# youngers2006/Dreamer

Hardware: AMD Instinct MI355X
Metric: imagined latent-steps/sec (B×H) at 64×64 CarRacing, 1/2/4/8 MI355X (higher is better)
Workload: dtype f32; 1 GPU; Dreamer.train_Agent() with AC_epochs=1 (replay sample + warm start S/2 + H-step imagination + actor-critic update), B=256/GPU S=64 H=15 64x64x3, precision=fp32 (north-star batch per GPU); global_batch=256, seq_len=64, horizon=15, parallelism=dp1, precision=fp32

## Files before the change

### dreamer_amd/_lib.py

```python
import ctypes as C
import os

import torch

_HERE = os.path.dirname(os.path.abspath(__file__))
LIB_PATH = os.path.join(_HERE, "libdreamer_hip.so")
if os.environ.get("DREAMER_LIB_VARIANT"):
    LIB_PATH = os.path.join(os.path.dirname(_HERE), "tools", "variants",
                            f"libdreamer_hip_{os.environ['DREAMER_LIB_VARIANT']}.so")

fp = C.c_void_p


class dr_linear(C.Structure):
    _fields_ = [("w", fp), ("b", fp)]


class dr_mlp3(C.Structure):
    _fields_ = [("l0", dr_linear), ("n1", dr_linear), ("l3", dr_linear), ("n4", dr_linear), ("l6", dr_linear)]


class dr_dims(C.Structure):
    _fields_ = [(n, C.c_int) for n in (
        "hidden", "rows", "cols", "action", "img_h", "img_w", "enc_f1", "enc_f2", "enc_hidden",
        "prior_h1", "prior_h2", "rew_h1", "rew_h2", "cont_h1", "cont_h2",
        "actor_h1", "actor_h2", "critic_h1", "critic_h2", "buckets", "dec_f1", "dec_f2", "dec_hidden", "precision", "obs_dim", "enc_depth",
        "launch_form")] + [("fault", fp), ("fault_host", fp)]

DR_MAX_DEPTH = 5


class dr_world_model(C.Structure):
    _fields_ = [("conv", dr_linear * DR_MAX_DEPTH), ("map0", dr_linear), ("map1", dr_linear), ("map3", dr_linear),
                ("w_ih", fp), ("w_hh", fp), ("b_ih", fp), ("b_hh", fp),
                ("prior", dr_mlp3), ("reward", dr_mlp3), ("cont", dr_mlp3), ("buckets_rew", fp)]


class dr_decoder(C.Structure):
    _fields_ = [("up0", dr_linear), ("up1", dr_linear), ("up3", dr_linear), ("convt", dr_linear * DR_MAX_DEPTH)]


class dr_wm_batch(C.Structure):
    _fields_ = [("actions", fp), ("act_sb", C.c_longlong), ("act_st", C.c_longlong), ("rewards", fp),
                ("continues", fp), ("rc_sb", C.c_longlong), ("rc_st", C.c_longlong)]


class dr_wm_loss_cfg(C.Structure):
    _fields_ = [("beta_pred", C.c_float), ("beta_dyn", C.c_float), ("beta_rep", C.c_float)]


class dr_actor(C.Structure):
    _fields_ = [("l0", dr_linear), ("n1", dr_linear), ("l3", dr_linear), ("n4", dr_linear),
                ("mu", dr_linear), ("ls", dr_linear)]


class dr_critic(C.Structure):
    _fields_ = [("net", dr_mlp3), ("buckets", fp)]


class dr_noise(C.Structure):
    _fields_ = [("q", fp), ("eps", fp), ("rng", fp), ("row0", C.c_int), ("stream", C.c_int)]


class dr_frames(C.Structure):
    _fields_ = [("ring", fp), ("ring_cap", C.c_longlong), ("starts", fp), ("obs", fp),
                ("stride_b", C.c_longlong), ("stride_t", C.c_longlong), ("raw255", C.c_int), ("t0", C.c_int)]


_P = C.POINTER
_sz = C.c_size_t
_i = C.c_int
_ll = C.c_longlong
_f = C.c_float
_d = C.c_double

_SIGS = {
    "dr_last_error": (C.c_char_p, []),
    "dr_version": (_i, []),
    "dr_encoder_workspace_bytes": (_sz, [_P(dr_dims), _i]),
    "dr_encoder_features": (_i, [_P(dr_dims), _P(dr_world_model), _P(dr_frames), _i, _i, fp, fp, _sz, fp]),
    "dr_observe_workspace_bytes": (_sz, [_P(dr_dims), _i]),
    "dr_observe_scan": (_i, [_P(dr_dims), _P(dr_world_model), _i, _i, fp, fp, _ll, _ll, fp, fp, dr_noise,
                             fp, fp, fp, fp, _sz, fp]),
    "dr_observe_trace_workspace_bytes": (_sz, [_P(dr_dims), _i, _i]),
    "dr_observe_trace": (_i, [_P(dr_dims), _P(dr_world_model), _i, _i, fp, fp, _ll, _ll, fp, fp, dr_noise,
                              fp, fp, fp, fp, fp, fp, fp, _sz, fp]),
    "dr_latent_stats": (_i, [_i, _i, _i, fp, fp, fp, fp, fp, fp, fp]),
    "dr_replay_returns": (_i, [_i, _i, fp, _ll, fp, _ll, _i, fp, _f, _f, fp, fp, fp, fp]),
    "dr_value_stats": (_i, [_i, _i, _i, _i, fp, _ll, fp, fp, fp, fp, fp, fp]),
    "dr_action_logprob": (_i, [_i, _i, _i, fp, fp, fp, _ll, _ll, fp, fp, fp, fp]),
    "dr_plan_sample": (_i, [_i, _i, _i, _i, _i, fp, fp, fp, dr_noise, fp, fp]),
    "dr_plan_update": (_i, [_i, _i, _i, _i, _i, fp, fp, fp, _f, _f, _f, _f, _f, fp, fp, fp, fp, fp, fp, fp, fp]),
    "dr_imagine_tape_bytes":(_sz, [_P(dr_dims), _i, _i]),
    "dr_imagine_workspace_bytes": (_sz, [_P(dr_dims), _i, _i]),
    "dr_imagine_fwd": (_i, [_P(dr_dims), _P(dr_world_model), _P(dr_actor), _i, _i, fp, fp, dr_noise, _i,
                            fp, fp, fp, fp, fp, fp, fp, fp, fp, _sz, fp]),
    "dr_imagine_actions_workspace_bytes": (_sz, [_P(dr_dims), _i, _i]),
    "dr_imagine_actions": (_i, [_P(dr_dims), _P(dr_world_model), _i, _i, fp, fp, fp, _ll, _ll, dr_noise,
                                fp, fp, fp, fp, fp, _sz, fp]),
    "dr_imagine_bwd": (_i, [_P(dr_dims), _P(dr_world_model), _P(dr_actor), _i, _i, fp, fp, fp, fp, fp,
                            fp, fp, fp, fp, _P(dr_actor), fp, _sz, fp]),
    "dr_imagine_bwd_prep": (_i, [_P(dr_dims), _P(dr_world_model), _P(dr_actor), _i, _i, fp, fp, fp, fp, _sz, fp]),
    "dr_imagine_bwd_main": (_i, [_P(dr_dims), _P(dr_world_model), _P(dr_actor), _i, _i, fp, fp, fp, fp, fp, _i,
                                 fp, _P(dr_actor), fp, _sz, fp]),
    "dr_step_workspace_bytes": (_sz, [_P(dr_dims), _i]),
    "dr_imagine_step": (_i, [_P(dr_dims), _P(dr_world_model), _i, fp, fp, fp, dr_noise, fp, fp, fp, fp,
                             fp, _sz, fp]),
    "dr_actor_act_workspace_bytes": (_sz, [_P(dr_dims), _i]),
    "dr_actor_act": (_i, [_P(dr_dims), _P(dr_actor), _i, fp, fp, dr_noise, _i, fp, fp, fp, fp, _sz, fp]),
    "dr_act_step_workspace_bytes": (_sz, [_P(dr_dims)]),
    "dr_act_step": (_i, [_P(dr_dims), _P(dr_world_model), _P(dr_actor), fp, _i, fp, fp, fp, dr_noise, _i,
                         fp, fp, fp, fp, fp, fp, fp, fp, _sz, fp]),
    "dr_act_batch_workspace_bytes": (_sz, [_P(dr_dims), _i]),
    "dr_act_batch": (_i, [_P(dr_dims), _P(dr_world_model), _P(dr_actor), _i, fp, fp, fp, fp, fp, dr_noise, _i,
                          fp, fp, fp, fp, fp, fp, fp, fp, _sz, fp]),
    "dr_act_vec_workspace_bytes": (_sz, [_P(dr_dims), _i]),
    "dr_act_vec": (_i, [_P(dr_dims), _P(dr_world_model), _P(dr_actor), _i, fp, fp, fp, fp, fp, dr_noise, _i,
                        fp, fp, fp, fp, fp, fp, fp, fp, _sz, fp]),
    "dr_gru_cell": (_i, [_P(dr_dims), _P(dr_world_model), _i, fp, fp, fp, fp, fp, _sz, fp]),
    "dr_categorical_sample": (_i, [_i, _i, _i, fp, dr_noise, fp, fp, fp, fp]),
    "dr_mlp3_fwd": (_i, [_P(dr_mlp3), _i, _i, fp, _ll, _i, fp, _ll, _i, _i, _i, fp, _ll, fp, _sz, fp]),
    "dr_bucket_value": (_i, [_i, _i, fp, fp, fp, fp]),
    "dr_critic_tape_bytes": (_sz, [_P(dr_dims), _i]),
    "dr_critic_workspace_bytes": (_sz, [_P(dr_dims), _i, _i]),
    "dr_critic_fwd": (_i, [_P(dr_dims), _P(dr_critic), _i, fp, _ll, fp, _ll, fp, fp, fp, fp, _sz, fp]),
    "dr_lambda_returns": (_i, [_i, _i, fp, fp, fp, _f, _f, fp, fp]),
    "dr_update_S": (_i, [_i, fp, fp, fp, fp, _sz, fp]),
    "dr_actor_loss_grad": (_i, [_i, _i, _i, fp, fp, fp, fp, fp, fp, _f, _f, fp, fp, fp, fp]),
    "dr_critic_loss_bwd": (_i, [_P(dr_dims), _P(dr_critic), _i, _i, fp, fp, fp, fp, _f, fp, _P(dr_critic),
                                fp, _sz, fp]),
    "dr_sqnorm": (_i, [_ll, fp, fp, fp]),
    "dr_sqnorm_multi": (_i, [_ll, fp, fp, fp, fp]),
    "dr_clip_stats": (_i, [_ll, fp, _ll, fp, _i, fp, fp, fp, fp, fp]),
    "dr_adamw": (_i, [_ll, fp, fp, fp, fp, fp, _f, _d, _d, _d, _d, _d, fp, fp, fp, fp]),
    "dr_ema": (_i, [_ll, fp, fp, _f, _f, fp, fp]),
    "dr_ac_optimiser_step": (_i, [_ll, fp, fp, fp, fp, fp, fp, _d, _d, _d, _d, _d,
                                  _ll, fp, fp, fp, fp, fp, fp, _d, _d, _d, _d, _d,
                                  _f, fp, _f, _f, _i, fp, fp, fp, fp, fp]),
    "dr_nonfinite": (_i, [_ll, fp, fp, fp]),
    "dr_replay_gather": (_i, [_ll, _i, _i, _i, _i, fp, fp, fp, fp, fp, fp, fp, fp, fp, fp]),
    "dr_rng_advance": (_i, [fp, C.c_ulonglong, fp]),
    "dr_persistent_kernels": (_i, [_P(dr_dims), _i, _i, _i]),
    "dr_stream_create_cumask": (_i, [_i, _P(C.c_uint), _P(fp)]),
    "dr_stream_destroy": (_i, [fp]),
    "dr_device_cus": (_i, [_P(_i)]),
    "dr_host_device_ptr": (_i, [fp, _P(fp)]),
    "dr_wm_train_workspace_bytes": (_sz, [_P(dr_dims), _i, _i]),
    "dr_decoder_workspace_bytes": (_sz, [_P(dr_dims), _i]),
    "dr_decoder_fwd": (_i, [_P(dr_dims), _P(dr_decoder), _i, fp, _ll, fp, _ll, fp, fp, _sz, fp]),
    "dr_frame_metrics": (_i, [_P(dr_dims), _i, _i, fp, _P(dr_frames), fp, fp, fp, fp]),
    "dr_frame_ssim": (_i, [_P(dr_dims), _i, _i, fp, _P(dr_frames), fp, fp, fp]),
    "dr_ensemble_metrics": (_i, [_P(dr_dims), _i, _i, _i, fp, _P(dr_frames), fp, fp, fp, fp, fp, fp]),
    "dr_wm_train_phase": (_i, [_P(dr_dims), _P(dr_world_model), _P(dr_decoder), _i, _i, _P(dr_frames),
                               _P(dr_wm_batch), dr_noise, dr_wm_loss_cfg, _i, fp, _i, fp, fp, _P(dr_world_model),
                               _P(dr_decoder), fp, fp, fp, fp, _sz, fp]),
    "dr_wm_train_grads": (_i, [_P(dr_dims), _P(dr_world_model), _P(dr_decoder), _i, _i, _P(dr_frames),
                               _P(dr_wm_batch), dr_noise, dr_wm_loss_cfg, fp, fp, _P(dr_world_model),
                               _P(dr_decoder), fp, fp, fp, fp, _sz, fp]),
}

EXPORTED = sorted(_SIGS)

_lib = None
_load_error = None


def load():
    global _lib, _load_error
    if _lib is not None:
        return _lib
    if not os.path.exists(LIB_PATH):
        _load_error = f"{LIB_PATH} not built (run: python -m dreamer_amd.build)"
        raise RuntimeError("dreamer_amd: HIP library missing: " + _load_error)
    lib = C.CDLL(LIB_PATH)
    for name, (res, args) in _SIGS.items():
        fn = getattr(lib, name)
        fn.restype = res
        fn.argtypes = args
    _lib = lib
    return lib


DR_E_INVALID, DR_E_HIP, DR_E_WORKSPACE, DR_E_UNSUPPORTED = 1001, 1002, 1003, 1004
DR_ACT_MAX_ENVS = 16
DR_ACT_VEC_MAX_OBS = 1023
DR_PLAN_MAX_CANDIDATES = 2048
DR_ENSEMBLE_MAX_SAMPLES = 64
DR_PLAN_MAX_ELEMS = 1024


class HipError(RuntimeError):

    def __init__(self, name, code, msg):
        super().__init__(f"{name} failed ({code}): {msg}")
        self.code = code


def call(name, *args):
    lib = load()
    rc = getattr(lib, name)(*args)
    if rc != 0:
        msg = lib.dr_last_error().decode(errors="replace")
        raise HipError(name, rc, msg)


def query(name, *args):
    return getattr(load(), name)(*args)


def ptr(t):
    if t is None:
        return None
    if not t.is_cuda:
        raise RuntimeError("dreamer_amd: tensors must live on the GPU (this framework is MI355X-only)")
    return t.data_ptr()


def stream_ptr(device=None):
    return torch.cuda.current_stream(device).cuda_stream


def require_gpu(t):
    if not (isinstance(t, torch.Tensor) and t.is_cuda):
        raise RuntimeError("dreamer_amd: hot-path ops run only on the GPU (MI355X); "
                           "move the model and tensors to 'cuda'")
```

### dreamer_amd/csrc/conv.h

```cpp
#pragma once
#include "common.h"

int op_conv_nhwc(int n, int cin, int ih, int iw, int cout, const float* in, const float* wr, const float* bias,
                 float* out, int out_nchw, hipStream_t s);
enum { CONV_EPI_FWD = 0, CONV_EPI_DSILU = 1 };
int op_conv_nhwc_ex(int n, int cin, int ih, int iw, int cout, const float* in, const float* wr, const float* bias,
                    float* out, int out_nchw, float* pre, int epi, hipStream_t s, float* csum = nullptr);
int op_frames_nhwc4(int n, int nb, int h, int w, const dr_frames* src, float* out, hipStream_t s, float pad = 0.0f);
int op_conv1_frames(int n, int nb, int ih, int iw, int cout, const dr_frames* src, const float* wr, const float* bias,
                    float* out, hipStream_t s);
int op_conv_repack_pad(int cout, int cin, int cin_pad, const float* w, float* wr, hipStream_t s);

int op_conv_repack_split3(int cout, int cin, const float* w, void* wr, hipStream_t s);
bool op_conv_split3_supported(int n, int cin, int ih, int iw, int cout);
int op_enc12_s1_bf16(int n, int nb, int h, int w, int c1, int c2, const dr_frames* src, const float* w1,
                     const float* b1, const float* w2, const float* b2, void* wr1, void* wr2, void* out,
                     hipStream_t s, int prepacked = 0);
int op_conv_s1_bf16(int n, int cin, int ih, int iw, int cout, const void* in, const void* wr, const float* bias,
                    void* out, int out_nchw, hipStream_t s);
bool op_conv_glds_bf16_supported(int n, int cin, int ih, int iw, int cout);
int op_conv_glds_s3(int n, int cin, int ih, int iw, int cout, const float* in, const void* wr, const float* bias,
                    float* out, int out_nchw, float* pre, int epi, hipStream_t s);
size_t op_gemm_nt_glds_part_floats(int M, int N, int K);
int op_gemm_nt_glds_bf16(int M, int N, int K, const void* X, int ldx, const void* W, int ldw, const float* bias,
                         float* Y, int ldy, float* part, size_t part_floats, hipStream_t s);
int op_conv_glds_bf16(int n, int cin, int ih, int iw, int cout, const void* in, const void* wr, const float* bias,
                      void* out, int out_nchw, hipStream_t s);
int op_conv_split3(int n, int cin, int ih, int iw, int cout, const float* in, const void* wr, const float* bias,
                   float* out, int out_nchw, hipStream_t s);
int op_conv_split3_ex(int n, int cin, int ih, int iw, int cout, const float* in, const void* wr, const float* bias,
                      float* out, int out_nchw, float* pre, int epi, hipStream_t s, int terms = 3);

size_t op_nt_split3_ws_bytes(int N, int K);
int op_nt_repack_split3(int N, int K, const float* W, int ldw, void* wr, hipStream_t s);
bool op_gemm_nt_split3_supported(int M, int N, int K, const float* A, int lda, const float* A2, int lda2, int ksA,
                                 int ldy);
int op_gemm_nt_split3(int M, int N, int K, const float* A, int lda, const float* A2, int lda2, int ksA, const void* wr,
                      const float* bias, int act, float* Y, int ldy, hipStream_t s);
size_t op_gemm_nt_split3_part_floats(int M, int N);
int op_gemm_nt_split3_sk(int M, int N, int K, const float* A, int lda, const float* A2, int lda2, int ksA,
                         const void* wr, const float* bias, int act, float* Y, int ldy, float* part,
                         size_t part_floats, hipStream_t s, int splits_fixed = 0);
int op_gemm_nt_split3_ex(int M, int N, int K, const float* A, int lda, const float* A2, int lda2, int ksA,
                         const void* wr, const float* bias, int act, float* Y, int ldy, int accumulate, float* Y2,
                         int ldy2, int nsplitY, float* part, size_t part_floats, hipStream_t s, int splits_fixed = 0);

int op_conv_repack_bf16(int cout, int cin, int cin_pad, const float* w, void* wr, hipStream_t s);
int op_to_bf16_2d(int rows, int cols, const float* x, long long ld, void* y, hipStream_t s);
int op_conv1_bf16(int n, int nb, int h, int w, int cout, const dr_frames* src, const void* wr, const float* bias,
                  void* out, hipStream_t s);
bool op_enc12_split3_ok(int n, int h, int w, int c1, int c2, const dr_frames* src);
int op_enc12_split3(int n, int nb, int h, int w, int c1, int c2, const dr_frames* src, const float* w1,
                    const float* b1, const float* w2, const float* b2, void* wr1, void* wr2, float* out,
                    hipStream_t s, int prepacked = 0);
int op_enc12_split3_ex(int n, int nb, int h, int w, int c1, int c2, const dr_frames* src, const float* w1,
                       const float* b1, const float* w2, const float* b2, void* wr1, void* wr2, float* out,
                       float* pre0, float* a0, float* pre1, hipStream_t s, int terms = 3, int prepacked = 0);
enum { RJ_CONV1 = 0, RJ_CONV = 1, RJ_NT = 2, RJ_BF16 = 3 };
struct RepackJob {
  int kind, a, b, c;
  const float* w;
  void* out;
  long long ld;
  long long total;
};
#define DR_RJ_MAX 6
RepackJob rj_conv1(int cout, const float* w, void* wr);
RepackJob rj_conv(int cout, int cin, const float* w, void* wr);
RepackJob rj_nt(int N, int K, const float* W, int ldw, void* wr);
RepackJob rj_bf16(int rows, int cols, const float* x, long long ld, void* y);
int op_repack_multi(const RepackJob* jobs, int n, hipStream_t s);
int op_enc12_bf16(int n, int nb, int h, int w, int c1, int c2, const dr_frames* src, const void* wr1, const float* b1,
                  const void* wr2, const float* b2, void* out, hipStream_t s);
int op_conv_bf16(int n, int cin, int ih, int iw, int cout, const void* in, const void* wr, const float* bias,
                 void* out, int out_nchw, hipStream_t s);
int op_gemm_nt_bf16(int M, int N, int K, const void* X, int ldx, const void* W, const float* bias, float* Y, int ldy,
                    hipStream_t s);

enum { CT_EPI_BIAS = 0, CT_EPI_DSILU = 1, CT_EPI_TANH_MSE = 2 };
struct ConvTArgs {
  int n, cin, h, w, cout;
  const float* in;
  int silu_in;
  const float* wq;
  const float* bias;
  float* out;
  float* out2;
  int silu_out;
  int ldc;
  const float* pre;
  const float* target;
  int tstride;
  const float* coef;
  float* part;
  float* bpart;
};
int op_convT_repack(int cin, int cout, const float* wt, float* wq, hipStream_t s);
int op_convT_nhwc(int epi, const ConvTArgs& a, hipStream_t s);
int op_convT_mse_parts(int h, int w);
int op_convT_out3_repack(int cin, const float* wt, float* wq, hipStream_t s);
int op_convT_out3(const ConvTArgs& a, hipStream_t s);
int op_convT_repack_split3(int cin, int cout, const float* wt, void* wr, hipStream_t s);
bool op_convT_split3_supported(int n, int cin, int h, int w, int cout, int terms = 3);
bool op_convT_cls_supported(int n, int cin, int h, int w, int cout);
int op_convT_split3(int epi, const ConvTArgs& a, const void* wr, hipStream_t s, int terms = 3);
bool op_convT_glds_s3_supported(const ConvTArgs& a, int epi);
int op_convT_glds_s3(int epi, const ConvTArgs& a, const void* wr, hipStream_t s);

size_t op_conv_wgrad_ws_floats(int n, int h, int w, int ca, int cb);
int op_wgrad_reduce(int ca, int cb, int cbo, int nsplit, const float* part, float* dw, float scale, int accumulate,
                    hipStream_t s);
bool op_wgrad_split3_supported(int n, int h, int w, int ca, int cb, int terms = 3);
size_t op_wgrad_split3_ws_floats(int n, int h, int w, int ca, int cb);
int op_wgrad_split3(int n, int h, int w, int ca, int cb, const float* lo, int lda, const float* hi, int ldb,
                    float* dw, int cbo, float scale, int accumulate, float* ws, size_t ws_floats, hipStream_t s,
                    int terms = 3);
int op_conv_wgrad(int n, int h, int w, int ca, int cb, const float* lo, int lda, int lo_silu, const float* hi, int ldb,
                  float* dw, int cbo, float scale, int accumulate, float* ws, size_t ws_floats, hipStream_t s,
                  float* bias_out = nullptr);
size_t op_chan_sum_ws_floats(long long rows, int C);
int op_chan_sum(long long rows, int C, const float* X, int ldx, float* out, int accumulate, float* ws, size_t ws_floats,
                hipStream_t s);
int op_chan_sum_final(int nb, int C, const float* part, float* out, int accumulate, hipStream_t s);

size_t op_gemm_tn_split3_ws_bytes(int M, int N, int K);
bool op_gemm_tn_split3_supported(int M, int N, int K);
int op_gemm_tn_split3(int M, int N, int K, const float* G, long long ldg, const float* X, long long ldx,
                      const float* X2, long long ldx2, int nsplitB, float* Y, long long ldy, int accumulate, void* ws,
                      size_t ws_bytes, hipStream_t s, int terms = 3);
struct TnProblem {
  int M, N, K;
  const float* G;
  long long ldg;
  const float* X;
  long long ldx;
  const float* X2;
  long long ldx2;
  int nsplitB;
  float* Y;
  long long ldy;
  int accumulate;
};
size_t op_gemm_tn_split3_multi_ws_bytes(const TnProblem* p, int n);
int op_gemm_tn_split3_multi(const TnProblem* p, int n, void* ws, size_t ws_bytes, hipStream_t s, int terms);
```

### dreamer_amd/csrc/conv_split.hip

```cpp
#include "conv.h"

#include <algorithm>
#include <climits>
#include <type_traits>

namespace {
typedef unsigned short u16;
typedef __bf16 bf16x8 __attribute__((ext_vector_type(8)));
typedef unsigned u32x4 __attribute__((ext_vector_type(4)));
typedef unsigned u32x2 __attribute__((ext_vector_type(2)));

__device__ __forceinline__ f32x4 mfma_b16(u32x4 a, u32x4 b, f32x4 c) {
  return __builtin_amdgcn_mfma_f32_16x16x32_bf16(__builtin_bit_cast(bf16x8, a), __builtin_bit_cast(bf16x8, b), c, 0, 0,
                                                  0);
}
__device__ __forceinline__ unsigned b16bits(__bf16 v) { return (unsigned)__builtin_bit_cast(u16, v); }
__device__ __forceinline__ void split3(float x, unsigned& h, unsigned& m, unsigned& l) {
  const __bf16 bh = (__bf16)x;
  const float r1 = x - (float)bh;
  const __bf16 bm = (__bf16)r1;
  const float r2 = r1 - (float)bm;
  h = b16bits(bh);
  m = b16bits(bm);
  l = b16bits((__bf16)r2);
// ... 1665 lines not shown
  for (int i = 0; i < APT; ++i) {
    const int m = min(m0 + prow + (NT / 8) * i, M - 1);
    oa[i] = (unsigned)(m * g.lda);
    oa2[i] = (unsigned)(m * g.lda2);
  }
  f32x4 ra0[APT], ra1[APT];
  u32x4 rb0[BPT], rb1[BPT];
  bool kv0 = true, kv1 = true;
  auto load = [&](int c, auto slot) __attribute__((always_inline)) {
    f32x4* ra = decltype(slot)::value == 0 ? ra0 : ra1;
    u32x4* rb = decltype(slot)::value == 0 ? rb0 : rb1;
    bool& kv = decltype(slot)::value == 0 ? kv0 : kv1;
    const int k = 32 * c + 4 * quad;
    kv = k < K;
    const int kk = kv ? k : 0;
    const bool s1 = kk < ksA;
    const float* base = s1 ? g.A : g.A2;
#pragma unroll
    for (int i = 0; i < APT; ++i) {
      const unsigned e = s1 ? oa[i] + (unsigned)kk : oa2[i] + (unsigned)(kk - ksA);
      ra[i] = *reinterpret_cast<const f32x4*>(base + e);
    }
#pragma unroll
    for (int j = 0; j < BPT; ++j) {
      const int e = tid + NT * j;
      if (BU % NT == 0 || e < BU) {
        const int pl = e / (BN * 4), rm = e - pl * BN * 4, row = rm >> 2, u = rm & 3;
        rb[j] = *reinterpret_cast<const u32x4*>(g.wr + (((long long)c * 3 + pl) * Np + n0 + row) * 32 + 8 * u);
      }
    }
  };
  auto store = [&](auto slot, int buf) __attribute__((always_inline)) {
    const f32x4* ra = decltype(slot)::value == 0 ? ra0 : ra1;
    const u32x4* rb = decltype(slot)::value == 0 ? rb0 : rb1;
    const bool kv = decltype(slot)::value == 0 ? kv0 : kv1;
#pragma unroll
    for (int i = 0; i < APT; ++i) {
      const int row = prow + (NT / 8) * i;
      const f32x4 v = kv ? ra[i] : (f32x4){0.f, 0.f, 0.f, 0.f};
      unsigned h0, m0_, l0, h1, m1, l1;
      split3_pair(v[0], v[1], h0, m0_, l0);
      split3_pair(v[2], v[3], h1, m1, l1);
      const int unit = (quad >> 1) ^ swz(row), half = quad & 1;
      reinterpret_cast<u32x2*>(&As[buf][0][row][unit])[half] = (u32x2){h0, h1};
      reinterpret_cast<u32x2*>(&As[buf][1][row][unit])[half] = (u32x2){m0_, m1};
      reinterpret_cast<u32x2*>(&As[buf][2][row][unit])[half] = (u32x2){l0, l1};
    }
#pragma unroll
    for (int j = 0; j < BPT; ++j) {
      const int e = tid + NT * j;
      if (BU % NT == 0 || e < BU) {
        const int pl = e / (BN * 4), rm = e - pl * BN * 4, row = rm >> 2, u = rm & 3;
        Bs[buf][pl][row][u ^ swz(row)] = rb[j];
      }
    }
  };
  const int wm0 = (wave >> 1) * 64, wn0 = (wave & 1) * WTN;
  const int fu = q ^ swz(r);
  f32x4 acc[FM][FN];
#pragma unroll
  for (int i = 0; i < FM; ++i)
#pragma unroll
    for (int j = 0; j < FN; ++j) acc[i][j] = (f32x4){0.f, 0.f, 0.f, 0.f};
  using S0 = std::integral_constant<int, 0>;
  using S1 = std::integral_constant<int, 1>;
  if (cb < NCH) {
  load(cb, S0{});
  load(min(cb + 1, NCH - 1), S1{});
  store(S0{}, 0);
  __syncthreads();
  auto step = [&](int c, auto slot) __attribute__((always_inline)) {
    constexpr int SL = decltype(slot)::value;
    using Next = std::integral_constant<int, 1 - SL>;
    const int buf = (c - cb) & 1;
    load(min(c + 2, NCH - 1), slot);
    u32x4 av[3][FM], bv[3][FN];
#pragma unroll
    for (int pl = 0; pl < 3; ++pl) {
#pragma unroll
      for (int i = 0; i < FM; ++i) av[pl][i] = As[buf][pl][wm0 + 16 * i + r][fu];
#pragma unroll
      for (int j = 0; j < FN; ++j) bv[pl][j] = Bs[buf][pl][wn0 + 16 * j + r][fu];
    }
#define DR_G3(PA, PB)                                                                                   \
  _Pragma("unroll") for (int i = 0; i < FM; ++i) _Pragma("unroll") for (int j = 0; j < FN; ++j) acc[i][j] = \
      mfma_b16(bv[PB][j], av[PA][i], acc[i][j]);
    DR_G3(2, 0)
    DR_G3(1, 1)
    DR_G3(0, 2)
    DR_G3(1, 0)
    DR_G3(0, 1)
    DR_G3(0, 0)
#undef DR_G3
    if (c + 1 < NCH) store(Next{}, buf ^ 1);
    dr_lds_barrier();
  };
  int c = cb;
  for (; c + 1 < NCH; c += 2) {
    step(c, S0{});
    step(c + 1, S1{});
  }
  if (c < NCH) step(c, S0{});
  }
#pragma unroll
  for (int i = 0; i < FM; ++i) {
    const int m = m0 + wm0 + 16 * i + r;
    if (m >= M) continue;
#pragma unroll
    for (int j = 0; j < FN; ++j) {
      const int n = n0 + wn0 + 16 * j + 4 * q;
      if (n >= N) continue;
      f32x4 v = acc[i][j];
      if (g.splits > 1) {
        *reinterpret_cast<f32x4*>(g.part + ((long long)blockIdx.y * M + m) * N + n) = v;
        continue;
      }
      if (g.bias) v += *reinterpret_cast<const f32x4*>(g.bias + n);
      if (g.act == 1) {
#pragma unroll
        for (int e = 0; e < 4; ++e) v[e] = v[e] / (1.0f + expf(-v[e]));
      }
      s3_store(g, m, n, v);
    }
  }
}

__global__ void k_s3_finish(GemmS3 g) {
  const long long i4 = (long long)blockIdx.x * 256 + threadIdx.x;
  const int N4 = g.N / 4;
  if (i4 >= (long long)g.M * N4) return;
  const int m = (int)(i4 / N4), n = 4 * (int)(i4 - (long long)m * N4);
  f32x4 v = (f32x4){0.f, 0.f, 0.f, 0.f};
  for (int sp = 0; sp < g.splits; ++sp) v += *reinterpret_cast<const f32x4*>(g.part + ((long long)sp * g.M + m) * g.N + n);
  if (g.bias) v += *reinterpret_cast<const f32x4*>(g.bias + n);
  if (g.act == 1) {
#pragma unroll
    for (int e = 0; e < 4; ++e) v[e] = v[e] / (1.0f + expf(-v[e]));
  }
  s3_store(g, m, n, v);
}

__device__ __forceinline__ void nt_repack_split3_elem(long long i, int N, int K, int Np, const float* __restrict__ W,
                                                      long long ldw, u16* __restrict__ wr) {
  const int KC = (K + 31) / 32;
  const int n = (int)(i / (KC * 32)), k = (int)(i - (long long)n * KC * 32);
  unsigned hh = 0, mm = 0, ll = 0;
  if (n < N && k < K) split3(W[(long long)n * ldw + k], hh, mm, ll);
  const long long plane = (long long)Np * 32;
  const long long base = ((long long)(k >> 5) * 3 * Np + n) * 32 + (k & 31);
  wr[base] = (u16)hh;
  wr[base + plane] = (u16)mm;
  wr[base + 2 * plane] = (u16)ll;
}
__global__ void k_nt_repack_split3(int N, int K, int Np, const float* __restrict__ W, int ldw, u16* __restrict__ wr) {
  const long long i = (long long)blockIdx.x * blockDim.x + threadIdx.x;
  if (i >= (long long)((K + 31) / 32) * 32 * Np) return;
  nt_repack_split3_elem(i, N, K, Np, W, ldw, wr);
}

struct RepackBatch {
  RepackJob j[DR_RJ_MAX];
  int blk0[DR_RJ_MAX + 1];
  int n;
};
__global__ __launch_bounds__(256) void k_repack_multi(RepackBatch b) {
  __shared__ __attribute__((aligned(16))) RepackJob J;
  int z = 0;
#pragma unroll
  for (int i = 1; i < DR_RJ_MAX; ++i)
    if ((int)blockIdx.x >= b.blk0[i]) z = i;
  dr_stage_args(b.j[z], J, threadIdx.x);
  const long long i = (long long)(blockIdx.x - b.blk0[z]) * 256 + threadIdx.x;
  if (i >= J.total) return;
  u16* out = static_cast<u16*>(J.out);
  switch (J.kind) {
    case RJ_CONV1: conv1_repack_split3_elem((int)i, J.a, J.w, out); break;
    case RJ_CONV: conv_repack_split3_elem((int)i, J.a, J.b, J.w, out); break;
    case RJ_NT: nt_repack_split3_elem(i, J.a, J.b, J.c, J.w, J.ld, out); break;
    default: {
      const int rr = (int)(i / J.b), cc = (int)(i - (long long)rr * J.b);
      out[i] = __builtin_bit_cast(u16, (__bf16)J.w[(long long)rr * J.ld + cc]);
    }
  }
}

RepackJob rj_conv1(int cout, const float* w, void* wr) { return {RJ_CONV1, cout, 0, 0, w, wr, 0, (long long)cout * 64}; }
RepackJob rj_conv(int cout, int cin, const float* w, void* wr) {
  return {RJ_CONV, cout, cin, 0, w, wr, 0, (long long)cout * 16 * cin};
}
RepackJob rj_nt(int N, int K, const float* W, int ldw, void* wr) {
  const int Np = (N + 127) / 128 * 128;
  return {RJ_NT, N, K, Np, W, wr, ldw, (long long)((K + 31) / 32) * 32 * Np};
}
RepackJob rj_bf16(int rows, int cols, const float* x, long long ld, void* y) {
  return {RJ_BF16, rows, cols, 0, x, y, ld, (long long)rows * cols};
}

int op_repack_multi(const RepackJob* jobs, int n, hipStream_t s) {
  if (n < 0 || n > DR_RJ_MAX) {
    dr_set_error("repack_multi: %d jobs (at most %d)", n, DR_RJ_MAX);
    return DR_E_INVALID;
  }
  if (n == 0) return DR_OK;
  RepackBatch b = {};
  int tot = 0;
  for (int i = 0; i < DR_RJ_MAX; ++i) {
    b.blk0[i] = tot;
    if (i < n) {
      b.j[i] = jobs[i];
      tot += (int)((jobs[i].total + 255) / 256);
    }
  }
  b.blk0[DR_RJ_MAX] = tot;
  b.n = n;
  hipLaunchKernelGGL(k_repack_multi, dim3((unsigned)tot), dim3(256), 0, s, b);
  return dr_check_launch("repack_multi");
}

static int s3_np(int N) { return (N + 127) / 128 * 128; }
size_t op_nt_split3_ws_bytes(int N, int K) {
  return (size_t)((K + 31) / 32) * 32 * 3 * s3_np(N) * sizeof(u16);
}
int op_nt_repack_split3(int N, int K, const float* W, int ldw, void* wr, hipStream_t s) {
  const int Np = s3_np(N);
  const long long total = (long long)((K + 31) / 32) * 32 * Np;
  hipLaunchKernelGGL(k_nt_repack_split3, dim3((unsigned)((total + 255) / 256)), dim3(256), 0, s, N, K, Np, W, ldw,
                     (u16*)wr);
  return dr_check_launch("nt_repack_split3");
}
bool op_gemm_nt_split3_supported(int M, int N, int K, const float* A, int lda, const float* A2, int lda2, int ksA,
                                 int ldy) {
  const bool seg = ksA < K;
  return M > 0 && N > 0 && N % 4 == 0 && ldy % 4 == 0 && K % 4 == 0 && lda % 4 == 0 && !((uintptr_t)A & 15) &&
         (!seg || (ksA % 4 == 0 && lda2 % 4 == 0 && A2 && !((uintptr_t)A2 & 15))) &&
         (long long)M * lda < (1LL << 31) && (!seg || (long long)M * lda2 < (1LL << 31));
}
size_t op_gemm_nt_split3_part_floats(int M, int N) { return (size_t)DR_S3_SPLITS * M * N; }

int op_gemm_nt_split3(int M, int N, int K, const float* A, int lda, const float* A2, int lda2, int ksA, const void* wr,
                      const float* bias, int act, float* Y, int ldy, hipStream_t s) {
  return op_gemm_nt_split3_sk(M, N, K, A, lda, A2, lda2, ksA, wr, bias, act, Y, ldy, nullptr, 0, s);
}

int op_gemm_nt_split3_sk(int M, int N, int K, const float* A, int lda, const float* A2, int lda2, int ksA,
                         const void* wr, const float* bias, int act, float* Y, int ldy, float* part,
                         size_t part_floats, hipStream_t s, int splits_fixed) {
  return op_gemm_nt_split3_ex(M, N, K, A, lda, A2, lda2, ksA, wr, bias, act, Y, ldy, 0, nullptr, 0, INT_MAX, part,
                              part_floats, s, splits_fixed);
}

int op_gemm_nt_split3_ex(int M, int N, int K, const float* A, int lda, const float* A2, int lda2, int ksA,
                         const void* wr, const float* bias, int act, float* Y, int ldy, int accumulate, float* Y2,
                         int ldy2, int nsplitY, float* part, size_t part_floats, hipStream_t s, int splits_fixed) {
  const bool y2 = nsplitY < N;
  if (!op_gemm_nt_split3_supported(M, N, K, A, lda, A2, lda2, ksA, ldy) || ((uintptr_t)Y & 15) ||
      (bias && ((uintptr_t)bias & 15)) || ((uintptr_t)part & 15) || splits_fixed < 0 ||
      splits_fixed > DR_S3_SPLITS || (splits_fixed > 1 && (!part || (size_t)splits_fixed * M * N > part_floats)) ||
      (y2 && (!Y2 || ((uintptr_t)Y2 & 15) || ldy2 % 4 || nsplitY % 4 || nsplitY < 0))) {
    dr_set_error("gemm_nt_split3: unsupported problem (M=%d N=%d K=%d)", M, N, K);
    return DR_E_INVALID;
  }
  GemmS3 g = {M, N, K, ksA < K ? ksA : K, lda, lda2, ldy, act, s3_np(N), A, A2, (const u16*)wr, bias, Y, 1, part,
              accumulate ? 1 : 0, ldy2, y2 ? nsplitY : INT_MAX, 0, Y2};
  auto tl = [&](int bm, int bn) { return ((M + bm - 1) / bm) * ((N + bn - 1) / bn); };
  auto waves = [&](int bm, int bn) { return (long long)tl(bm, bn) * (bm / 32); };
  const int nch = (K + 31) / 32;
  auto splits_for = [&](int bm, int bn) {
    if (splits_fixed > 0) return splits_fixed;
    int sp = 1;
    while (part && sp < DR_S3_SPLITS && waves(bm, bn) * sp < 2048 && nch / (2 * sp) >= 8 &&
           (size_t)(2 * sp) * M * N <= part_floats)
      sp *= 2;
    return sp;
  };
  const int shapes[5][2] = {{256, 128}, {256, 64}, {128, 128}, {128, 64}, {64, 64}};
  int pick = 4;
  for (int c = 0; c < 5; ++c) {
    if (waves(shapes[c][0], shapes[c][1]) * splits_for(shapes[c][0], shapes[c][1]) >= 2048) {
      pick = c;
      break;
    }
  }
  g.splits = splits_for(shapes[pick][0], shapes[pick][1]);
  const unsigned gy = (unsigned)g.splits;
  switch (pick) {
    case 0: hipLaunchKernelGGL((k_gemm_split3<256, 128>), dim3(dr_xcd_grid(tl(256, 128)), gy), dim3(512), 0, s, g); break;
    case 1: hipLaunchKernelGGL((k_gemm_split3<256, 64>), dim3(dr_xcd_grid(tl(256, 64)), gy), dim3(512), 0, s, g); break;
    case 2: hipLaunchKernelGGL((k_gemm_split3<128, 128>), dim3(dr_xcd_grid(tl(128, 128)), gy), dim3(256), 0, s, g); break;
    case 3: hipLaunchKernelGGL((k_gemm_split3<128, 64>), dim3(dr_xcd_grid(tl(128, 64)), gy), dim3(256), 0, s, g); break;
    default: hipLaunchKernelGGL((k_gemm_split3<64, 64>), dim3(dr_xcd_grid(tl(64, 64)), gy), dim3(128), 0, s, g); break;
  }
  DR_TRY(dr_check_launch("gemm_nt_split3"));
  if (g.splits > 1) {
    hipLaunchKernelGGL(k_s3_finish, dim3((unsigned)(((long long)M * (N / 4) + 255) / 256)), dim3(256), 0, s, g);
    DR_TRY(dr_check_launch("s3_finish"));
  }
  return DR_OK;
}

static int s3_pad(int n) { return (n + 127) / 128 * 128; }

struct KnRepack {
  int K, N, P, nsplit;
  const float* X;
  const float* X2;
  long long ldx, ldx2;
  u16* wr;
  long long pad_;
};

template <int TERMS>
__device__ __forceinline__ void kn_repack_body(int K, int N, int P, const float* __restrict__ X, long long ldx,
                                               const float* __restrict__ X2, long long ldx2, int nsplit,
                                               u16* __restrict__ wr) {
  const int n = blockIdx.x * 256 + threadIdx.x, kc = blockIdx.y;
  if (n >= P) return;
  const bool seg2 = n >= nsplit;
  const float* src = seg2 ? X2 : X;
  const long long ld = seg2 ? ldx2 : ldx;
  const int nn = seg2 ? n - nsplit : n;
  float v[32];
  const bool nok = n < N;
  const float* col = src + (nok ? nn : 0);
#pragma unroll
  for (int k = 0; k < 32; ++k) {
    const int kk = 32 * kc + k;
    const bool ok = nok && kk < K;
    const float t = col[ok ? (long long)kk * ld : 0LL];
    v[k] = ok ? t : 0.f;
  }
  u32x4* o = reinterpret_cast<u32x4*>(wr + (((long long)kc * 3) * P + n) * 32);
  if constexpr (TERMS == 1) {
#pragma unroll
    for (int u = 0; u < 4; ++u) {
      u32x4 h;
#pragma unroll
      for (int e = 0; e < 4; ++e) h[e] = pack_bf16x2(v[8 * u + 2 * e], v[8 * u + 2 * e + 1]);
      o[u] = h;
    }
    return;
  }
  u32x4 h[4], m[4], l[4];
#pragma unroll
  for (int u = 0; u < 4; ++u)
#pragma unroll
    for (int e = 0; e < 4; ++e) {
      unsigned hh, mm, ll;
      split3_pair(v[8 * u + 2 * e], v[8 * u + 2 * e + 1], hh, mm, ll);
      h[u][e] = hh;
      m[u][e] = mm;
      l[u][e] = ll;
    }
  const long long pl = (long long)P * 32 / 8;
#pragma unroll
  for (int u = 0; u < 4; ++u) {
    o[u] = h[u];
    o[pl + u] = m[u];
    o[2 * pl + u] = l[u];
  }
}

struct GemmPP {
  int M, N, K, Mp, Np, splits, accumulate, tiles;
  long long ldy;
  const u16* wa;
  const u16* wb;
  float* Y;
// ... 294 lines not shown
```

### dreamer_amd/csrc/engine.hip

```cpp
#include "engine_util.h"
#include "scan.h"
#include "dream.h"
#include "bptt.h"


static bool s3_first_layer(const dr_dims* d, int M, int N, const float* h, long long ldh, const float* z,
                           long long ldz) {
  return d->precision != DR_PREC_BF16 && M >= 1024 && ldh < INT_MAX && ldz < INT_MAX &&
         op_gemm_nt_split3_supported(M, N, d->hidden + latent(d), h, (int)ldh, z, (int)ldz, d->hidden, N);
}

struct EncWs {
  float *x0, *a[DR_MAX_DEPTH], *wr[DR_MAX_DEPTH], *sk;
  long long sk_n;
  void* wproj;
  void* s3proj;
  float* s3part;
  size_t s3part_n;
};

static void enc_carve(Carve& c, const dr_dims* d, int n, EncWs& w) {
  memset(&w, 0, sizeof(w));
  if (d->obs_dim > 0) {
    const int F = enc_feat_dim(d);
    w.x0 = c.f((long long)n * d->obs_dim);
    w.a[0] = c.f((long long)n * F);
    w.a[1] = c.f((long long)n * F);
    w.sk_n = splitk_floats(n, d->enc_hidden);
    w.sk = c.f(w.sk_n);
    return;
  }
  const bool bf = d->precision == DR_PREC_BF16;
  int e[DR_MAX_DEPTH + 1];
  const int N = enc_chans(d, e);
  const long long p0 = (long long)d->img_h * d->img_w;
  auto act = [&](long long elems) { return bf ? (float*)c.raw(elems * 2) : c.f(elems); };
  w.sk_n = bf ? 0 : splitk_floats(n, d->enc_hidden);
  w.sk = bf ? nullptr : c.f(w.sk_n);
  w.x0 = bf ? nullptr : c.f((long long)n * p0 * 4);
  for (int k = 0; k < N; ++k) w.a[k] = act((long long)n * (p0 >> (2 * (k + 1))) * e[k + 1]);
  w.wr[0] = (float*)c.raw((size_t)e[1] * 64 * 6);
  for (int k = 1; k < N; ++k) w.wr[k] = (float*)c.raw((long long)e[k + 1] * e[k] * 16 * 6);
  w.wproj = bf ? c.raw((size_t)d->enc_hidden * enc_feat_dim(d) * 2) : nullptr;
  w.s3proj = bf ? nullptr : c.raw(op_nt_split3_ws_bytes(d->enc_hidden, enc_feat_dim(d)));
  w.s3part_n = bf ? op_gemm_nt_glds_part_floats(n, d->enc_hidden, enc_feat_dim(d))
                  : op_gemm_nt_split3_part_floats(n, d->enc_hidden);
  w.s3part = w.s3part_n ? c.f((long long)w.s3part_n) : nullptr;
}

extern "C" size_t dr_encoder_workspace_bytes(const dr_dims* d, int n_frames) {
  Carve c(nullptr);
  EncWs w;
  enc_carve(c, d, n_frames, w);
  return c.off;
}

static int encoder_bf16(const dr_dims* d, const dr_world_model* wm, const dr_frames* src, int B, int n, float* feat,
                        const EncWs& w, hipStream_t s) {
  int e[DR_MAX_DEPTH + 1];
  const int N = enc_chans(d, e);
  const int h0 = d->img_h, w0 = d->img_w;
  const int F = enc_feat_dim(d);
  const bool e12 = N >= 2 && op_enc12_split3_ok(n, h0, w0, e[1], e[2], src) && !((uintptr_t)w.a[1] & 15);
  RepackJob rj[DR_RJ_MAX];
  int nj = 0;
  if (e12) {
    rj[nj++] = rj_conv1(e[1], wm->conv[0].w, w.wr[0]);
    rj[nj++] = rj_conv(e[2], e[1], wm->conv[1].w, w.wr[1]);
  }
  bool s3[DR_MAX_DEPTH + 1] = {};
  for (int k = 2; k < N; ++k) {
    s3[k] = op_conv_split3_supported(n, e[k], h0 >> k, w0 >> k, e[k + 1]) && nj < DR_RJ_MAX - 1;
    if (s3[k]) rj[nj++] = rj_conv(e[k + 1], e[k], wm->conv[k].w, w.wr[k]);
    else DR_TRY(op_conv_repack_bf16(e[k + 1], e[k], e[k], wm->conv[k].w, w.wr[k], s));
  }
  rj[nj++] = rj_bf16(d->enc_hidden, F, wm->map0.w, F + d->hidden, w.wproj);
  DR_TRY(op_repack_multi(rj, nj, s));
  const int rc_s1 = e12 ? op_enc12_s1_bf16(n, B, h0, w0, e[1], e[2], src, wm->conv[0].w, wm->conv[0].b, wm->conv[1].w,
                                           wm->conv[1].b, w.wr[0], w.wr[1], w.a[1], s, 1)
                        : DR_E_INVALID;
  if (rc_s1 != DR_OK) {
    if (rc_s1 != DR_E_INVALID) return rc_s1;
    DR_TRY(op_conv_repack_bf16(e[1], 3, 4, wm->conv[0].w, w.wr[0], s));
    DR_TRY(op_conv_repack_bf16(e[2], e[1], e[1], wm->conv[1].w, w.wr[1], s));
    const int rc_b = op_enc12_bf16(n, B, h0, w0, e[1], e[2], src, w.wr[0], wm->conv[0].b, w.wr[1], wm->conv[1].b,
                                   w.a[1], s);
    if (rc_b != DR_OK) {
      if (rc_b != DR_E_INVALID) return rc_b;
      DR_TRY(op_conv1_bf16(n, B, h0, w0, e[1], src, w.wr[0], wm->conv[0].b, w.a[0], s));
      DR_TRY(op_conv_bf16(n, e[1], h0 / 2, w0 / 2, e[2], w.a[0], w.wr[1], wm->conv[1].b, w.a[1], 0, s));
    }
  }
  for (int k = 2; k < N; ++k) {
    if (s3[k]) {
      DR_TRY(op_conv_s1_bf16(n, e[k], h0 >> k, w0 >> k, e[k + 1], w.a[k - 1], w.wr[k], wm->conv[k].b, w.a[k],
                             k == N - 1 ? 1 : 0, s));
    } else {
      DR_TRY(op_conv_bf16(n, e[k], h0 >> k, w0 >> k, e[k + 1], w.a[k - 1], w.wr[k], wm->conv[k].b, w.a[k],
                          k == N - 1 ? 1 : 0, s));
    }
  }
  const int rcp = op_gemm_nt_glds_bf16(n, d->enc_hidden, F, w.a[N - 1], F, w.wproj, F, wm->map0.b, feat, d->enc_hidden,
                                       w.s3part, w.s3part_n, s);
  if (rcp != DR_E_INVALID) return rcp;
  return op_gemm_nt_bf16(n, d->enc_hidden, F, w.a[N - 1], F, w.wproj, wm->map0.b, feat, d->enc_hidden, s);
}

extern "C" int dr_encoder_features(const dr_dims* d, const dr_world_model* wm, const dr_frames* src, int B, int T,
                                   float* feat, void* ws, size_t ws_bytes, hipStream_t s) {
  DR_REQUIRE(d && wm && src && feat && B > 0 && T > 0, "null argument or empty batch");
  DR_REQUIRE(vae_depth_ok(d), "enc_depth must be 0, 4 or 5");
  if (d->obs_dim > 0) {
    DR_REQUIRE(d->enc_f2 > 0 && d->obs_dim % 4 == 0, "vector observations: obs_dim % 4 == 0 required");
    const int n = B * T, F = enc_feat_dim(d), D = d->obs_dim;
    Carve c(ws);
    EncWs w;
    enc_carve(c, d, n, w);
    WS_CHECK(c, ws_bytes);
    DR_TRY(op_vec_gather(n, B, D, src, w.x0, s));
    GemmArgs g1 = lin(n, F, D, w.x0, D, wm->conv[0].w, D, wm->conv[0].b, w.a[0], F);
    g1.act = 1;
    DR_TRY(run(G_NT, AM_PLAIN, g1, s));
    GemmArgs g2 = lin(n, F, F, w.a[0], F, wm->conv[1].w, F, wm->conv[1].b, w.a[1], F);
    g2.act = 1;
    DR_TRY(run(G_NT, AM_PLAIN, g2, s));
    GemmArgs gp = lin(n, d->enc_hidden, F, w.a[1], F, wm->map0.w, F + d->hidden, wm->map0.b, feat, d->enc_hidden);
    float* sk = w.sk;
    long long skn = w.sk_n;
    give_splitk(gp, sk, skn);
    return run(G_NT, AM_PLAIN, gp, s);
  }
  int e[DR_MAX_DEPTH + 1];
  const int N = enc_chans(d, e);
  DR_REQUIRE(d->img_h % (1 << N) == 0 && d->img_w % (1 << N) == 0,
             "image size must be a multiple of 2^depth (16, or 32 for the 5-layer encoder)");
  DR_REQUIRE(d->enc_f1 % 4 == 0 && d->enc_f2 % 4 == 0, "encoder filter counts must be multiples of 4");
  DR_REQUIRE(d->precision == DR_PREC_FP32 || d->precision == DR_PREC_BF16, "precision must be DR_PREC_FP32/BF16");
  const int n = B * T;
  Carve c(ws);
  EncWs w;
  enc_carve(c, d, n, w);
  WS_CHECK(c, ws_bytes);
  if (d->precision == DR_PREC_BF16) return encoder_bf16(d, wm, src, B, n, feat, w, s);
  const int h0 = d->img_h, w0 = d->img_w;
  const int F = enc_feat_dim(d);
  const bool e12 = N >= 2 && op_enc12_split3_ok(n, h0, w0, e[1], e[2], src);
  const bool s3p = w.s3proj && n >= 1024 &&
                   op_gemm_nt_split3_supported(n, d->enc_hidden, F, w.a[N - 1], F, nullptr, 0, F, d->enc_hidden);
  RepackJob rj[DR_RJ_MAX];
  int nj = 0;
  if (e12) {
    rj[nj++] = rj_conv1(e[1], wm->conv[0].w, w.wr[0]);
    rj[nj++] = rj_conv(e[2], e[1], wm->conv[1].w, w.wr[1]);
  }
  bool s3[DR_MAX_DEPTH + 1] = {};
  for (int k = e12 ? 2 : 1; k < N; ++k) {
    s3[k] = op_conv_split3_supported(n, e[k], h0 >> k, w0 >> k, e[k + 1]) && nj < DR_RJ_MAX - 1;
    if (!s3[k]) continue;
    DR_TRY(conv_bias_aligned(__func__, "conv", k, wm->conv[k].b));
    rj[nj++] = rj_conv(e[k + 1], e[k], wm->conv[k].w, w.wr[k]);
  }
  if (s3p) rj[nj++] = rj_nt(d->enc_hidden, F, wm->map0.w, F + d->hidden, w.s3proj);
  DR_TRY(op_repack_multi(rj, nj, s));
  int k0 = 1;
  const int rc12 = e12 ? op_enc12_split3(n, B, h0, w0, e[1], e[2], src, wm->conv[0].w, wm->conv[0].b, wm->conv[1].w,
                                         wm->conv[1].b, w.wr[0], w.wr[1], w.a[1], s, 1)
                       : DR_E_INVALID;
  if (rc12 == DR_OK) {
    k0 = 2;
  } else {
    if (rc12 != DR_E_INVALID) return rc12;
    DR_TRY(op_conv_repack_pad(e[1], 3, 4, wm->conv[0].w, w.wr[0], s));
    if (op_conv1_frames(n, B, h0, w0, e[1], src, w.wr[0], wm->conv[0].b, w.a[0], s) != DR_OK) {
      DR_TRY(op_frames_nhwc4(n, B, h0, w0, src, w.x0, s));
      DR_TRY(op_conv_nhwc(n, 4, h0, w0, e[1], w.x0, w.wr[0], wm->conv[0].b, w.a[0], 0, s));
    }
  }
  for (int k = k0; k < N; ++k) {
    const int cin = e[k], cout = e[k + 1], hin = h0 >> k, win = w0 >> k, last = k == N - 1;
    const float* cw = wm->conv[k].w;
    const float* cb = wm->conv[k].b;
    if (s3[k]) {
      DR_TRY(op_conv_split3(n, cin, hin, win, cout, w.a[k - 1], w.wr[k], cb, w.a[k], last, s));
    } else {
      DR_TRY(op_conv_repack_pad(cout, cin, cin, cw, w.wr[k], s));
      DR_TRY(op_conv_nhwc(n, cin, hin, win, cout, w.a[k - 1], w.wr[k], cb, w.a[k], last, s));
    }
  }
  if (s3p) {
    const int ksplits = std::max(1, std::min(8, (F + 1023) / 1024));
    return op_gemm_nt_split3_sk(n, d->enc_hidden, F, w.a[N - 1], F, nullptr, 0, F, w.s3proj, wm->map0.b, 0, feat,
                                d->enc_hidden, w.s3part, w.s3part_n, s, ksplits);
  }
  GemmArgs gp = lin(n, d->enc_hidden, F, w.a[N - 1], F, wm->map0.w, F + d->hidden, wm->map0.b, feat, d->enc_hidden);
  float* sk = w.sk;
  long long skn = w.sk_n;
  give_splitk(gp, sk, skn);
  return run(G_NT, AM_PLAIN, gp, s);
}

struct ObsWs {
  float *gi, *gh, *pre1, *logits, *wt, *hb[2];
  unsigned short* hb16[2];
  int* idx;
  void *s3m0, *s3whh;
  void* ring;
};
static void obs_carve(Carve& c, const dr_dims* d, int B, ObsWs& w) {
  w.ring = c.raw(op_pscan_ring_bytes(B));
  w.s3m0 = c.raw(op_nt_split3_ws_bytes(d->enc_hidden, d->hidden));
  w.s3whh = c.raw(op_nt_split3_ws_bytes(3 * d->hidden, d->hidden));
  w.gi = c.f((long long)B * 3 * d->hidden);
  w.gh = c.f((long long)B * 3 * d->hidden);
  w.pre1 = c.f((long long)B * d->enc_hidden);
  w.logits = c.f((long long)B * latent(d));
  w.wt = c.f((long long)(latent(d) + d->action) * 3 * d->hidden);
  w.hb[0] = c.f((long long)B * d->hidden);
  w.hb[1] = c.f((long long)B * d->hidden);
  w.hb16[0] = (unsigned short*)c.raw(sizeof(unsigned short) * B * d->hidden);
  w.hb16[1] = (unsigned short*)c.raw(sizeof(unsigned short) * B * d->hidden);
  w.idx = c.i(2LL * B * d->rows);
}

extern "C" size_t dr_observe_workspace_bytes(const dr_dims* d, int B) {
  Carve c(nullptr);
  ObsWs w;
  obs_carve(c, d, B, w);
  return c.off;
}

struct ObsTrace {
  float *latents, *hiddens, *post_logits;
  float* z_last;
  int* idx_last;
};

static int observe_steps(const dr_dims* d, const dr_world_model* wm, int B, int T, const float* feat,
                         const float* actions, long long act_sb, long long act_st, const float* h_init,
                         const float* z_init, const dr_noise& noise, float* z_out, float* h_out, float* logits_out,
                         ObsWs& w, const ObsTrace* tr, hipStream_t s);

extern "C" int dr_observe_scan(const dr_dims* d, const dr_world_model* wm, int B, int T, const float* feat,
                               const float* actions, long long act_sb, long long act_st, const float* h_init,
                               const float* z_init, dr_noise noise, float* z_out, float* h_out, float* logits_out,
                               void* ws, size_t ws_bytes, hipStream_t s) {
  DR_REQUIRE(d && wm && feat && z_out && h_out && B > 0 && T > 0, "null argument or empty batch");
  GemmBf16Scope bf16_scope(d->precision == DR_PREC_BF16);
  DR_REQUIRE(T == 1 || (z_init == nullptr ? T > 1 : true), "bad T");
  DR_REQUIRE(actions || (z_init == nullptr && T == 1), "actions required");
  Carve c(ws);
  ObsWs w;
  obs_carve(c, d, B, w);
  WS_CHECK(c, ws_bytes);
  const int L = latent(d), Hd = d->hidden, eh = d->enc_hidden;
  const int F = enc_feat_dim(d);
  const bool any_gru = (z_init != nullptr) || T > 1;
  if (any_gru) {
    DR_REQUIRE(wm->w_ih && wm->w_hh && wm->b_ih && wm->b_hh, "GRU weights required");
    DR_TRY(op_transpose(3 * Hd, L + d->action, wm->w_ih, w.wt, s));
  }
  if (z_init == nullptr && h_init == nullptr && op_pscan_supported(d, B, T, d->action)) {
    const int rc = op_pscan(d, wm, B, T, d->action, feat, actions, act_sb, act_st, w.wt, wm->map0.w + F, F + Hd,
                            noise, 0, z_out, h_out, logits_out, w.ring, s);
    if (rc != DR_E_UNSUPPORTED) return rc;
  }
  return observe_steps(d, wm, B, T, feat, actions, act_sb, act_st, h_init, z_init, noise, z_out, h_out, logits_out, w,
                       nullptr, s);
}

static int observe_steps(const dr_dims* d, const dr_world_model* wm, int B, int T, const float* feat,
                         const float* actions, long long act_sb, long long act_st, const float* h_init,
                         const float* z_init, const dr_noise& noise, float* z_out, float* h_out, float* logits_out,
                         ObsWs& w, const ObsTrace* tr, hipStream_t s) {
  const int L = latent(d), Hd = d->hidden, eh = d->enc_hidden;
  const int F = enc_feat_dim(d);
  const long long ldL = (long long)T * L, ldH = (long long)T * Hd;
  const bool planes = B >= 128 && T > 1 && Hd % 8 == 0;
  if (planes) {
    DR_TRY(split_planes(eh, Hd, wm->map0.w + F, F + Hd, w.s3m0, s));
    DR_TRY(split_planes(3 * Hd, Hd, wm->w_hh, Hd, w.s3whh, s));
  }
  const float* h = h_init;
  const unsigned short* h16 = nullptr;
  const bool a16 = planes && d->precision == DR_PREC_BF16;
  int hb = 0;
  const bool split_gru = B >= 128;
  bool gh_pre = false;
  if (z_init) {
    if (z_init != z_out) DR_TRY(copy2d(z_out, L, z_init, L, L, B, s));
    DR_TRY(op_onehot_index(B, d->rows, d->cols, z_out, L, w.idx, onehot_vals(w.idx, B, d->rows), s));
    if (split_gru && planes && h_init) {
      GemmArgs gh = lin(B, 3 * Hd, Hd, h_init, Hd, wm->w_hh, Hd, wm->b_hh, w.gh, 3 * Hd);
      wplanes(gh, w.s3whh);
      DR_TRY(gemm_launch(G_NT, AM_PLAIN, &gh, 1, s));
      gh_pre = true;
    }
  }
  for (int t = 0; t < T; ++t) {
    const bool do_gru = (z_init != nullptr) || t > 0;
    if (do_gru) {
      const int ai = t - (z_init == nullptr ? 1 : 0);
      float* hn = w.hb[hb];
      unsigned short* hn16 = a16 ? w.hb16[hb] : nullptr;
      hb ^= 1;
      DR_TRY(gru_onehot(d, wm, B, w.idx, actions + ai * act_st, act_sb, h, Hd, hn, Hd, w.wt, nullptr,
                        nullptr, nullptr, nullptr, s, z_out, L, w.gh, gh_pre, hn16));
      h = hn;
      h16 = hn16;
    }
    GemmArgs g[2];
    g[0] = lin(B, eh, h ? Hd : 0, h, Hd, wm->map0.w + F, F + Hd, nullptr, w.pre1, eh);
    g[0].addend = feat + (long long)t * B * eh;
    g[0].ld_add = eh;
    const GemmArgs g_last = g[0];
    gh_pre = split_gru && h && t + 1 < T;
    if (gh_pre) {
      g[1] = lin(B, 3 * Hd, Hd, h, Hd, wm->w_hh, Hd, wm->b_hh, w.gh, 3 * Hd);
      if (planes) {
        wplanes(g[0], w.s3m0);
        wplanes(g[1], w.s3whh);
        g[0].A16 = g[1].A16 = h16;
      } else {
        g[0].bf16 = g[1].bf16 = 0;
      }
    }
    DR_TRY(gemm_launch(G_NT, AM_PLAIN, g, gh_pre ? 2 : 1, s));
    float* lg = (t == T - 1 && logits_out) ? logits_out : nullptr;
    long long ld_lg = L;
    const bool dual = tr && gh_pre && (planes || d->precision == DR_PREC_BF16);
    if (tr && tr->post_logits) {
      lg = tr->post_logits + (long long)t * L;
      ld_lg = ldL;
    }
    GemmArgs gp = lin_ln(B, L, eh, w.pre1, eh, wm->map1, wm->map3.w, wm->map3.b, dual ? nullptr : lg, ld_lg);
    with_sampler(gp, d, noise, t, z_out, L, w.idx, nullptr, 0);
    DR_TRY(run(G_NT, AM_LNSILU, gp, s));
    const float* zs = z_out;
    if (dual) {
      DR_TRY(gemm_launch(G_NT, AM_PLAIN, &g_last, 1, s));
      GemmArgs gq = lin_ln(B, L, eh, w.pre1, eh, wm->map1, wm->map3.w, wm->map3.b, lg, ld_lg);
      with_sampler(gq, d, noise, t, tr->z_last, L, tr->idx_last, nullptr, 0);
      DR_TRY(run(G_NT, AM_LNSILU, gq, s));
      zs = tr->z_last;
    }
    if (tr) {
      const float* hs = h;
      if (!hs) {
        DR_TRY(zero(w.hb[0], (long long)B * Hd, s));
        hs = w.hb[0];
      }
      const Copy2dJob cj[2] = {{tr->latents + (long long)t * L, ldL, zs, L, L, B},
                               {tr->hiddens + (long long)t * Hd, ldH, hs, Hd, Hd, B}};
      DR_TRY(op_copy2d_multi(cj, 2, s));
    }
  }
  if (!h_out) return DR_OK;
  if (h) DR_TRY(copy2d(h_out, Hd, h, Hd, Hd, B, s));
  else DR_TRY(zero(h_out, (long long)B * Hd, s));
  return DR_OK;
}

struct Tape {
  float *eps, *ls_raw;
  float *pre1a, *x1a, *pre2a, *x2a;
  float *r, *u, *n, *ghn;
  float *pre1p, *pre2p, *soft;
};
static void tape_carve(Carve& c, const dr_dims* d, int B, int H, Tape& t) {
  const long long BH = (long long)B * H;
  t.eps = c.f(BH * d->action);
  t.ls_raw = c.f(BH * d->action);
  t.pre1a = c.f(BH * d->actor_h1);
  t.x1a = c.f(BH * d->actor_h1);
  t.pre2a = c.f(BH * d->actor_h2);
  t.x2a = c.f(BH * d->actor_h2);
  t.r = c.f(BH * d->hidden);
  t.u = c.f(BH * d->hidden);
  t.n = c.f(BH * d->hidden);
  t.ghn = c.f(BH * d->hidden);
  t.pre1p = c.f(BH * d->prior_h1);
  t.pre2p = c.f(BH * d->prior_h2);
  t.soft = c.f(BH * latent(d));
}

extern "C" size_t dr_imagine_tape_bytes(const dr_dims* d, int B, int H) {
  Carve c(nullptr);
  Tape t;
  tape_carve(c, d, B, H, t);
  return c.off;
}

struct ImWs {
  float *gi, *gh, *plog, *p1r, *p1c, *p2r, *p2c, *rlog, *clog, *rval, *wt, *wst, *bst;
  unsigned short* hid16;
  float *tl0f, *hpart;
  void *s3r, *s3c;
  void *s3p0, *s3a0, *s3whh, *s3wt, *s3twhh, *s3tl0a;
  float* s3part;
  size_t s3part_n;
  int* idx[2];
  float *gH, *gZ, *gA, *glog, *gx2, *gp2, *gx1, *gp1, *ggi, *ggh, *gheads, *gx2a, *gpre2a, *gy2a, *xh2a, *gx1a,
      *gpre1a, *gy1a, *xh1a, *hcat, *zcat, *sk;
  unsigned short *ggi16, *ggh16, *gpre1a16;
  long long sk_n;
  float *tl6p, *tl3p, *tl0p, *twhh, *thead, *tl3a, *tl0a;
  void* tn;
  size_t tn_bytes;
  void* pd;
  void* pb;
};
static void imws_carve(Carve& c, const dr_dims* d, int B, int H, ImWs& w) {
  const long long Bl = B, BH = (long long)B * H, B1 = (long long)B * (H + 1);
  const int L = latent(d), Hd = d->hidden, A = d->action;
  w.gi = c.f(Bl * 3 * Hd);
  w.gh = c.f(Bl * 3 * Hd);
  w.plog = c.f(Bl * L);
  w.p1r = c.f(B1 * d->rew_h1);
  w.p1c = c.f(B1 * d->cont_h1);
  w.p2r = c.f(B1 * d->rew_h2);
  w.p2c = c.f(B1 * d->cont_h2);
  w.rlog = c.f(B1 * d->buckets);
  w.clog = c.f(B1);
  w.rval = c.f(B1);
  w.s3p0 = c.raw(op_nt_split3_ws_bytes(d->prior_h1, Hd));
  w.s3a0 = c.raw(op_nt_split3_ws_bytes(d->actor_h1, Hd));
  w.s3whh = c.raw(op_nt_split3_ws_bytes(3 * Hd, Hd));
  w.s3wt = c.raw(op_nt_split3_ws_bytes(L + A, 3 * Hd));
  w.s3twhh = c.raw(op_nt_split3_ws_bytes(Hd, 3 * Hd));
  w.s3tl0a = c.raw(op_nt_split3_ws_bytes(Hd + L, d->actor_h1));
  w.s3r = c.raw(op_nt_split3_ws_bytes(d->rew_h1, d->hidden + L));
  w.s3c = c.raw(op_nt_split3_ws_bytes(d->cont_h1, d->hidden + L));
  w.s3part_n = op_gemm_nt_split3_part_floats((int)B1, std::max(d->rew_h1, d->cont_h1));
  w.s3part = c.f((long long)w.s3part_n);
  w.wt = c.f((long long)(L + A) * 3 * Hd);
  w.hid16 = (unsigned short*)c.raw(sizeof(unsigned short) * Bl * (H + 1) * Hd);
  w.tl0f = c.f((long long)(Hd + L) * d->actor_h1);
  w.hpart = c.f(Bl * d->actor_h1);
  w.wst = c.f((long long)2 * A * d->actor_h2);
  w.bst = c.f((long long)2 * A);
  w.idx[0] = c.i(2 * Bl * d->rows);
  w.idx[1] = c.i(2 * Bl * d->rows);
  w.tl6p = c.f((long long)L * d->prior_h2);
  w.tl3p = c.f((long long)d->prior_h2 * d->prior_h1);
  w.tl0p = c.f((long long)d->prior_h1 * Hd);
  w.twhh = c.f((long long)3 * Hd * Hd);
  w.thead = c.f((long long)2 * A * d->actor_h2);
  w.tl3a = c.f((long long)d->actor_h2 * d->actor_h1);
  w.tl0a = c.f((long long)d->actor_h1 * (Hd + L));
  w.gH = c.f(B1 * Hd);
  w.gZ = c.f(B1 * L);
  w.gA = c.f(BH * A);
  w.glog = c.f(Bl * L);
  w.gx2 = c.f(Bl * d->prior_h2);
  w.gp2 = c.f(Bl * d->prior_h2);
  w.gx1 = c.f(Bl * d->prior_h1);
  w.gp1 = c.f(Bl * d->prior_h1);
  w.ggi = c.f(Bl * 3 * Hd);
  w.ggh = c.f(Bl * 3 * Hd);
  w.ggi16 = (unsigned short*)c.raw(sizeof(unsigned short) * Bl * 3 * Hd);
  w.ggh16 = (unsigned short*)c.raw(sizeof(unsigned short) * Bl * 3 * Hd);
  w.gheads = c.f(BH * 2 * A);
  w.gx2a = c.f(Bl * d->actor_h2);
  w.gpre2a = c.f(BH * d->actor_h2);
  w.gy2a = c.f(BH * d->actor_h2);
  w.xh2a = c.f(BH * d->actor_h2);
  w.gx1a = c.f(Bl * d->actor_h1);
  w.gpre1a = c.f(BH * d->actor_h1);
  w.gpre1a16 = (unsigned short*)c.raw(sizeof(unsigned short) * BH * d->actor_h1);
  w.gy1a = c.f(BH * d->actor_h1);
  w.xh1a = c.f(BH * d->actor_h1);
  w.hcat = c.f(BH * Hd);
  w.zcat = c.f(BH * L);
  w.sk_n = splitk_floats(d->actor_h1, Hd + L) + splitk_floats(d->actor_h2, d->actor_h1) +
           2 * splitk_floats(A, d->actor_h2);
  w.sk = c.f(w.sk_n);
  const int BHi = (int)BH;
  w.tn_bytes = op_gemm_tn_split3_ws_bytes(d->actor_h1, Hd + L, BHi) +
               op_gemm_tn_split3_ws_bytes(d->actor_h2, d->actor_h1, BHi) +
               2 * op_gemm_tn_split3_ws_bytes(A, d->actor_h2, BHi);
  w.tn = c.raw(w.tn_bytes);
  w.pd = c.raw(op_pdream_ws_bytes(d, B, H));
  w.pb = c.raw(op_pbptt_ws_bytes(d, B, H));
}

extern "C" size_t dr_imagine_workspace_bytes(const dr_dims* d, int B, int H) {
  Carve c(nullptr);
  ImWs w;
  imws_carve(c, d, B, H, w);
  return c.off;
}

static int imagine_heads(const dr_dims* d, const dr_world_model* wm, int B, int H, const float* latents,
                         const float* hiddens, float* rewards, float* continues, ImWs& w, hipStream_t s,
                         bool keep0 = false);

static int imagine_launch_form(const dr_dims* d, const dr_world_model* wm, const dr_actor* ac, int B, int H,
                               const dr_noise& noise, const dr_noise& nq, int deterministic, float* latents,
                               float* hiddens, float* actions, float* mus, float* sigmas, const Tape& tp, ImWs& w,
                               bool split_gru, bool zg, hipStream_t s) {
  const int L = latent(d), Hd = d->hidden, A = d->action, a1 = d->actor_h1, a2 = d->actor_h2;
  const long long ldH = (long long)(H + 1) * Hd, ldL = (long long)(H + 1) * L, ldA = (long long)H * A;
  const long long lda1 = (long long)H * a1, lda2 = (long long)H * a2;
  const bool planes = split_gru && H > 1 && Hd % 8 == 0;
  const bool a16 = planes && d->precision == DR_PREC_BF16;
  if (planes) {
    DR_TRY(split_planes(d->prior_h1, Hd, wm->prior.l0.w, Hd, w.s3p0, s));
    if (zg) DR_TRY(split_planes(a1, Hd, ac->l0.w, Hd + L, w.s3a0, s));
    DR_TRY(split_planes(3 * Hd, Hd, wm->w_hh, Hd, w.s3whh, s));
  }

  {
    DR_TRY(run(G_NT, AM_PLAIN, lin2(B, a1, hiddens, ldH, Hd, latents, ldL, L, ac->l0.w, ac->l0.b, tp.pre1a, lda1), s));
    GemmArgs g = lin_ln(B, a2, a1, tp.pre1a, lda1, ac->n1, ac->l3.w, ac->l3.b, tp.pre2a, lda2);
    g.a_out = tp.x1a; g.ld_aout = lda1;
    DR_TRY(run(G_NT, AM_LNSILU, g, s));
  }
  DR_TRY(stack_heads(ac, A, a2, w.wst, w.bst, s));
  {
    GemmArgs h = lin_ln(B, 2 * A, a2, tp.pre2a, lda2, ac->n4, w.wst, w.bst, nullptr, 0);
    h.a_out = tp.x2a; h.ld_aout = lda2;
    with_actor_head(h, A, noise, 0, deterministic, actions, ldA, mus, ldA, sigmas, ldA, tp.eps, tp.ls_raw, ldA);
    DR_TRY(run(G_NT, AM_LNSILU, h, s));
  }
  for (int t = 0; t < H; ++t) {
    const long long hb = (long long)Hd * B * t;
    float* h_t = hiddens + (long long)t * Hd;
    float* h_n = hiddens + (long long)(t + 1) * Hd;
    float* z_t = latents + (long long)t * L;
    float* z_n = latents + (long long)(t + 1) * L;
    unsigned short* h_n16 = a16 ? w.hid16 + (long long)(t + 1) * Hd : nullptr;
    DR_TRY(gru_onehot(d, wm, B, w.idx[t & 1], actions + (long long)t * A, ldA, h_t, ldH, h_n, ldH, w.wt,
                      tp.r + hb, tp.u + hb, tp.n + hb, tp.ghn + hb, s, z_t, ldL, w.gh, split_gru && t > 0, h_n16));
    float* p1 = tp.pre1p + (long long)t * B * d->prior_h1;
    float* p2 = tp.pre2p + (long long)t * B * d->prior_h2;
    {
      const bool more = t + 1 < H;
      GemmArgs p[3];
      int np = 0;
      p[np] = lin(B, d->prior_h1, Hd, h_n, ldH, wm->prior.l0.w, Hd, wm->prior.l0.b, p1, d->prior_h1);
      if (planes) wplanes(p[np], w.s3p0);
      ++np;
      if (more && zg) {
        p[np] = lin(B, a1, Hd, h_n, ldH, ac->l0.w, Hd + L, ac->l0.b, w.hpart, a1);
        if (planes) wplanes(p[np], w.s3a0);
        ++np;
      }
      if (more && split_gru) {
        p[np] = lin(B, 3 * Hd, Hd, h_n, ldH, wm->w_hh, Hd, wm->b_hh, w.gh, 3 * Hd);
        if (planes) wplanes(p[np], w.s3whh);
        ++np;
      }
      for (int i = 0; i < np; ++i) {
        if (!planes) p[i].bf16 = 0;
        p[i].A16 = h_n16;
      }
      DR_TRY(gemm_launch(G_NT, AM_PLAIN, p, np, s));
    }
    DR_TRY(run(G_NT, AM_LNSILU, lin_ln(B, d->prior_h2, d->prior_h1, p1, d->prior_h1, wm->prior.n1, wm->prior.l3.w,
                                       wm->prior.l3.b, p2, d->prior_h2), s));
    GemmArgs g = lin_ln(B, L, d->prior_h2, p2, d->prior_h2, wm->prior.n4, wm->prior.l6.w, wm->prior.l6.b, nullptr, 0);
    with_sampler(g, d, nq, t, z_n, ldL, w.idx[(t + 1) & 1], tp.soft + (long long)t * B * L, L);
    DR_TRY(run(G_NT, AM_LNSILU, g, s));
    if (t + 1 < H) {
      const long long o1 = (long long)(t + 1) * a1, o2 = (long long)(t + 1) * a2, o = (long long)(t + 1) * A;
      if (zg) {
        int* ix = w.idx[(t + 1) & 1];
        DR_TRY(op_zgather_add(B, a1, d->rows, d->cols, ix, onehot_vals(ix, B, d->rows), z_n, ldL,
                              w.tl0f + (long long)Hd * a1, a1, w.hpart, a1, tp.pre1a + o1, lda1, s));
      } else {
        DR_TRY(run(G_NT, AM_PLAIN, lin2(B, a1, h_n, ldH, Hd, z_n, ldL, L, ac->l0.w, ac->l0.b, tp.pre1a + o1, lda1), s));
      }
      GemmArgs g3 = lin_ln(B, a2, a1, tp.pre1a + o1, lda1, ac->n1, ac->l3.w, ac->l3.b, tp.pre2a + o2, lda2);
      g3.a_out = tp.x1a + o1;
      g3.ld_aout = lda1;
      DR_TRY(run(G_NT, AM_LNSILU, g3, s));
      GemmArgs hd = lin_ln(B, 2 * A, a2, tp.pre2a + o2, lda2, ac->n4, w.wst, w.bst, nullptr, 0);
      hd.a_out = tp.x2a + o2;
      hd.ld_aout = lda2;
      with_actor_head(hd, A, noise, t + 1, deterministic, actions + o, ldA, mus + o, ldA, sigmas + o, ldA,
                      tp.eps + (long long)(t + 1) * B * A, tp.ls_raw + o, ldA);
      DR_TRY(run(G_NT, AM_LNSILU, hd, s));
    }
  }
  return DR_OK;
}

extern "C" int dr_imagine_fwd(const dr_dims* d, const dr_world_model* wm, const dr_actor* ac, int B, int H,
                              const float* z0, const float* h0, dr_noise noise, int deterministic, float* latents,
                              float* hiddens, float* actions, float* rewards, float* continues, float* mus,
                              float* sigmas, void* tape, void* ws, size_t ws_bytes, hipStream_t s) {
  DR_REQUIRE(d && wm && ac && z0 && h0 && latents && hiddens && actions && rewards && continues && mus && sigmas &&
                 tape && B > 0 && H > 0,
             "null argument or empty batch");
  GemmBf16Scope bf16_scope(d->precision == DR_PREC_BF16);
  Carve c(ws);
  ImWs w;
  imws_carve(c, d, B, H, w);
  WS_CHECK(c, ws_bytes);
  Carve ct(tape);
  Tape tp;
  tape_carve(ct, d, B, H, tp);
  const int L = latent(d), Hd = d->hidden, A = d->action, a1 = d->actor_h1, a2 = d->actor_h2;
  const long long ldH = (long long)(H + 1) * Hd, ldL = (long long)(H + 1) * L, ldA = (long long)H * A;
  const long long lda1 = (long long)H * a1, lda2 = (long long)H * a2;
  {
    const Copy2dJob cj[2] = {{latents, ldL, z0, L, L, B}, {hiddens, ldH, h0, Hd, Hd, B}};
    DR_TRY(op_copy2d_multi(cj, 2, s));
  }
  dr_noise nq = noise;
  nq.stream += 65536;
  const bool split_gru = B >= 128;
  const bool zg = d->rows <= 32 && a1 % 4 == 0;
  {
    TransposeJob tj[2] = {{3 * Hd, L + A, 3 * Hd, wm->w_ih, w.wt}, {a1, Hd + L, a1, ac->l0.w, w.tl0f}};
    DR_TRY(op_transpose_multi(tj, zg ? 2 : 1, s));
  }
  DR_TRY(op_onehot_index(B, d->rows, d->cols, latents, ldL, w.idx[0], onehot_vals(w.idx[0], B, d->rows), s));

  bool unrolled = false;
  if (zg && op_pdream_supported(d, B, H, A)) {
    const PDreamTape pt = {tp.eps, tp.ls_raw, tp.pre1a, tp.x1a, tp.pre2a, tp.x2a, tp.r, tp.u, tp.n, tp.ghn,
                           tp.pre1p, tp.pre2p, tp.soft};
    const int rc = op_pdream(d, wm, ac, B, H, w.wt, w.tl0f + (long long)Hd * a1, w.idx[0], noise, nq, deterministic,
                             latents, hiddens, actions, mus, sigmas, pt, w.pd, s);
    if (rc != DR_E_UNSUPPORTED && rc != DR_OK) return rc;
    unrolled = rc == DR_OK;
  }
  if (!unrolled) DR_TRY(imagine_launch_form(d, wm, ac, B, H, noise, nq, deterministic, latents, hiddens, actions, mus,
                                            sigmas, tp, w, split_gru, zg, s));
  return imagine_heads(d, wm, B, H, latents, hiddens, rewards, continues, w, s);
}

static int imagine_heads(const dr_dims* d, const dr_world_model* wm, int B, int H, const float* latents,
                         const float* hiddens, float* rewards, float* continues, ImWs& w, hipStream_t s, bool keep0) {
  const int L = latent(d), Hd = d->hidden;
  {
    const int M1 = B * (H + 1);
    GemmArgs p[2];
    if (s3_first_layer(d, M1, d->rew_h1, hiddens, Hd, latents, L) &&
        s3_first_layer(d, M1, d->cont_h1, hiddens, Hd, latents, L)) {
      DR_TRY(op_nt_repack_split3(d->rew_h1, Hd + L, wm->reward.l0.w, Hd + L, w.s3r, s));
      DR_TRY(op_nt_repack_split3(d->cont_h1, Hd + L, wm->cont.l0.w, Hd + L, w.s3c, s));
      DR_TRY(op_gemm_nt_split3_sk(M1, d->rew_h1, Hd + L, hiddens, Hd, latents, L, Hd, w.s3r, wm->reward.l0.b, 0,
                                  w.p1r, d->rew_h1, w.s3part, w.s3part_n, s));
      DR_TRY(op_gemm_nt_split3_sk(M1, d->cont_h1, Hd + L, hiddens, Hd, latents, L, Hd, w.s3c, wm->cont.l0.b, 0,
                                  w.p1c, d->cont_h1, w.s3part, w.s3part_n, s));
    } else {
      p[0] = lin2(M1, d->rew_h1, hiddens, Hd, Hd, latents, L, L, wm->reward.l0.w, wm->reward.l0.b, w.p1r, d->rew_h1);
      p[1] = lin2(M1, d->cont_h1, hiddens, Hd, Hd, latents, L, L, wm->cont.l0.w, wm->cont.l0.b, w.p1c, d->cont_h1);
      DR_TRY(gemm_launch(G_NT, AM_PLAIN, p, 2, s));
    }
    p[0] = lin_ln(M1, d->buckets, d->rew_h2, w.p2r, d->rew_h2, wm->reward.n4, wm->reward.l6.w, wm->reward.l6.b, w.rlog,
                  d->buckets);
    p[1] = lin_ln(M1, 1, d->cont_h2, w.p2c, d->cont_h2, wm->cont.n4, wm->cont.l6.w, wm->cont.l6.b, w.clog, 1);
    p[1].act = 2;
    if (std::max(std::max(d->rew_h1, d->rew_h2), std::max(d->cont_h1, d->cont_h2)) <= 208) {
      Mlp2Args m2[2];
      const float* x1[2] = {w.p1r, w.p1c};
      const dr_mlp3* hm[2] = {&wm->reward, &wm->cont};
      const int k1[2] = {d->rew_h1, d->cont_h1}, k2[2] = {d->rew_h2, d->cont_h2};
      for (int i = 0; i < 2; ++i) {
        memset(&m2[i], 0, sizeof(Mlp2Args));
        m2[i].M = M1; m2[i].K1 = k1[i]; m2[i].K2 = k2[i];
        m2[i].X = x1[i]; m2[i].ldx = k1[i];
        m2[i].ln1_g = hm[i]->n1.w; m2[i].ln1_b = hm[i]->n1.b;
        m2[i].W3 = hm[i]->l3.w; m2[i].b3 = hm[i]->l3.b;
        m2[i].ln4_g = hm[i]->n4.w; m2[i].ln4_b = hm[i]->n4.b;
        m2[i].e = p[i];
        m2[i].e.A = nullptr;
      }
      DR_TRY(mlp2_launch(m2, 2, s));
    } else {
      GemmArgs q[2];
      q[0] = lin_ln(M1, d->rew_h2, d->rew_h1, w.p1r, d->rew_h1, wm->reward.n1, wm->reward.l3.w, wm->reward.l3.b, w.p2r,
                    d->rew_h2);
      q[1] = lin_ln(M1, d->cont_h2, d->cont_h1, w.p1c, d->cont_h1, wm->cont.n1, wm->cont.l3.w, wm->cont.l3.b, w.p2c,
                    d->cont_h2);
      DR_TRY(gemm_launch(G_NT, AM_LNSILU, q, 2, s));
      DR_TRY(gemm_launch(G_NT, AM_LNSILU, p, 2, s));
    }
    DR_TRY(op_bucket_value(M1, d->buckets, w.rlog, d->buckets, wm->buckets_rew, w.rval, 1, s));
    const int k0 = keep0 ? 0 : 1, Ho = H + 1 - k0;
    const Copy2dJob cj[2] = {{rewards, Ho, w.rval + k0, H + 1, Ho, B}, {continues, Ho, w.clog + k0, H + 1, Ho, B}};
    DR_TRY(op_copy2d_multi(cj, 2, s));
  }
  return DR_OK;
}

struct ImActWs {
  ImWs w;
  float *p1, *p2;
};
static void imact_carve(Carve& c, const dr_dims* d, int B, int H, ImActWs& a) {
  const long long Bl = B, B1 = (long long)B * (H + 1);
  const int L = latent(d), Hd = d->hidden, A = d->action;
  ImWs& w = a.w;
  memset(&w, 0, sizeof(w));
  w.gh = c.f(Bl * 3 * Hd);
  w.wt = c.f((long long)(L + A) * 3 * Hd);
  w.hid16 = (unsigned short*)c.raw(sizeof(unsigned short) * B1 * Hd);
  w.s3p0 = c.raw(op_nt_split3_ws_bytes(d->prior_h1, Hd));
  w.s3whh = c.raw(op_nt_split3_ws_bytes(3 * Hd, Hd));
  w.idx[0] = c.i(2 * Bl * d->rows);
  w.idx[1] = c.i(2 * Bl * d->rows);
  a.p1 = c.f(Bl * d->prior_h1);
  a.p2 = c.f(Bl * d->prior_h2);
  w.p1r = c.f(B1 * d->rew_h1);
  w.p1c = c.f(B1 * d->cont_h1);
  w.p2r = c.f(B1 * d->rew_h2);
  w.p2c = c.f(B1 * d->cont_h2);
  w.rlog = c.f(B1 * d->buckets);
  w.clog = c.f(B1);
  w.rval = c.f(B1);
  w.s3r = c.raw(op_nt_split3_ws_bytes(d->rew_h1, Hd + L));
  w.s3c = c.raw(op_nt_split3_ws_bytes(d->cont_h1, Hd + L));
  w.s3part_n = op_gemm_nt_split3_part_floats((int)B1, std::max(d->rew_h1, d->cont_h1));
  w.s3part = c.f((long long)w.s3part_n);
}

extern "C" size_t dr_imagine_actions_workspace_bytes(const dr_dims* d, int B, int H) {
  if (!d || B <= 0 || H <= 0) return 0;
  Carve c(nullptr);
  ImActWs a;
  imact_carve(c, d, B, H, a);
  return c.off;
}

extern "C" int dr_imagine_actions(const dr_dims* d, const dr_world_model* wm, int B, int H, const float* z0,
                                  const float* h0, const float* actions, long long act_sb, long long act_st,
                                  dr_noise noise, float* latents, float* hiddens, float* rewards, float* continues,
                                  void* ws, size_t ws_bytes, hipStream_t s) {
  DR_REQUIRE(d && wm && z0 && h0 && actions && latents && hiddens && rewards && continues && ws && B > 0 && H > 0,
             "null argument or empty batch");
  DR_REQUIRE(wm->w_ih && wm->w_hh && wm->b_ih && wm->b_hh, "GRU weights required");
  GemmBf16Scope bf16_scope(d->precision == DR_PREC_BF16);
  Carve c(ws);
  ImActWs a;
  imact_carve(c, d, B, H, a);
  WS_CHECK(c, ws_bytes);
  ImWs& w = a.w;
  const int L = latent(d), Hd = d->hidden, A = d->action;
  const long long ldH = (long long)(H + 1) * Hd, ldL = (long long)(H + 1) * L;
  {
    const Copy2dJob cj[2] = {{latents, ldL, z0, L, L, B}, {hiddens, ldH, h0, Hd, Hd, B}};
    DR_TRY(op_copy2d_multi(cj, 2, s));
  }
  const bool split_gru = B >= 128;
  const bool planes = split_gru && H > 1 && Hd % 8 == 0;
  const bool a16 = planes && d->precision == DR_PREC_BF16;
  DR_TRY(op_transpose(3 * Hd, L + A, wm->w_ih, w.wt, s));
  DR_TRY(op_onehot_index(B, d->rows, d->cols, latents, ldL, w.idx[0], onehot_vals(w.idx[0], B, d->rows), s));
  if (planes) {
    DR_TRY(split_planes(d->prior_h1, Hd, wm->prior.l0.w, Hd, w.s3p0, s));
    DR_TRY(split_planes(3 * Hd, Hd, wm->w_hh, Hd, w.s3whh, s));
  }
  for (int t = 0; t < H; ++t) {
    float* h_t = hiddens + (long long)t * Hd;
    float* h_n = hiddens + (long long)(t + 1) * Hd;
    float* z_t = latents + (long long)t * L;
    float* z_n = latents + (long long)(t + 1) * L;
    unsigned short* h_n16 = a16 ? w.hid16 + (long long)(t + 1) * Hd : nullptr;
    DR_TRY(gru_onehot(d, wm, B, w.idx[t & 1], actions + (long long)t * act_st, act_sb, h_t, ldH, h_n, ldH, w.wt,
                      nullptr, nullptr, nullptr, nullptr, s, z_t, ldL, w.gh, split_gru && t > 0, h_n16));
    {
      GemmArgs p[2];
      int np = 0;
      p[np] = lin(B, d->prior_h1, Hd, h_n, ldH, wm->prior.l0.w, Hd, wm->prior.l0.b, a.p1, d->prior_h1);
      if (planes) wplanes(p[np], w.s3p0);
      ++np;
      if (t + 1 < H && split_gru) {
        p[np] = lin(B, 3 * Hd, Hd, h_n, ldH, wm->w_hh, Hd, wm->b_hh, w.gh, 3 * Hd);
        if (planes) wplanes(p[np], w.s3whh);
        ++np;
      }
      for (int i = 0; i < np; ++i) {
        if (!planes) p[i].bf16 = 0;
        p[i].A16 = h_n16;
      }
      DR_TRY(gemm_launch(G_NT, AM_PLAIN, p, np, s));
    }
    DR_TRY(run(G_NT, AM_LNSILU, lin_ln(B, d->prior_h2, d->prior_h1, a.p1, d->prior_h1, wm->prior.n1, wm->prior.l3.w,
                                       wm->prior.l3.b, a.p2, d->prior_h2), s));
    GemmArgs g = lin_ln(B, L, d->prior_h2, a.p2, d->prior_h2, wm->prior.n4, wm->prior.l6.w, wm->prior.l6.b, nullptr, 0);
    with_sampler(g, d, noise, t, z_n, ldL, w.idx[(t + 1) & 1], nullptr, 0);
    DR_TRY(run(G_NT, AM_LNSILU, g, s));
  }
  return imagine_heads(d, wm, B, H, latents, hiddens, rewards, continues, w, s);
}

static int imagine_bwd_impl(const dr_dims* d, const dr_world_model* wm, const dr_actor* ac, int B, int H,
                            const float* latents, const float* hiddens, const float* actions,
                            const float* g_mus, const float* g_sigmas,
                            const float* g_actions, const float* g_latents, const float* g_hiddens,
                            const void* tape, const dr_actor* gr, void* ws, size_t ws_bytes, hipStream_t s,
                            bool do_prep, bool do_main);

extern "C" int dr_imagine_bwd(const dr_dims* d, const dr_world_model* wm, const dr_actor* ac, int B, int H,
                              const float* latents, const float* hiddens, const float* actions,
                              const float* g_mus, const float* g_sigmas,
                              const float* g_actions, const float* g_latents, const float* g_hiddens,
                              const void* tape, const dr_actor* gr, void* ws, size_t ws_bytes, hipStream_t s) {
  return imagine_bwd_impl(d, wm, ac, B, H, latents, hiddens, actions, g_mus, g_sigmas, g_actions, g_latents,
                          g_hiddens, tape, gr, ws, ws_bytes, s, true, true);
}

extern "C" int dr_imagine_bwd_prep(const dr_dims* d, const dr_world_model* wm, const dr_actor* ac, int B, int H,
                                   const float* g_actions, const float* g_latents, const float* g_hiddens, void* ws,
                                   size_t ws_bytes, hipStream_t s) {
  DR_REQUIRE(d && wm && ac && B > 0 && H > 0, "null argument or empty batch");
  return imagine_bwd_impl(d, wm, ac, B, H, nullptr, nullptr, nullptr, nullptr, nullptr, g_actions, g_latents,
                          g_hiddens, nullptr, nullptr, ws, ws_bytes, s, true, false);
}

extern "C" int dr_imagine_bwd_main(const dr_dims* d, const dr_world_model* wm, const dr_actor* ac, int B, int H,
                                   const float* latents, const float* hiddens, const float* actions,
                                   const float* g_mus, const float* g_sigmas, int upstream_state, const void* tape,
                                   const dr_actor* gr, void* ws, size_t ws_bytes, hipStream_t s) {
  const float* flag = upstream_state ? reinterpret_cast<const float*>(ws) : nullptr;
  return imagine_bwd_impl(d, wm, ac, B, H, latents, hiddens, actions, g_mus, g_sigmas, nullptr, flag, nullptr, tape,
                          gr, ws, ws_bytes, s, false, true);
}

static int imagine_bwd_impl(const dr_dims* d, const dr_world_model* wm, const dr_actor* ac, int B, int H,
                            const float* latents, const float* hiddens, const float* actions,
                            const float* g_mus, const float* g_sigmas,
                            const float* g_actions, const float* g_latents, const float* g_hiddens,
                            const void* tape, const dr_actor* gr, void* ws, size_t ws_bytes, hipStream_t s,
                            bool do_prep, bool do_main) {
  DR_REQUIRE(d && wm && ac && B > 0 && H > 0, "null argument or empty batch");
  GemmBf16Scope bf16_scope(d->precision == DR_PREC_BF16);
  DR_REQUIRE(!do_main || (latents && hiddens && actions && tape && gr), "null argument");
  Carve c(ws);
  ImWs w;
  imws_carve(c, d, B, H, w);
  WS_CHECK(c, ws_bytes);
  Carve ct((void*)tape);
  Tape tp;
  if (do_main) tape_carve(ct, d, B, H, tp);
  const int L = latent(d), Hd = d->hidden, A = d->action, a1 = d->actor_h1, a2 = d->actor_h2;
  const long long ldH = (long long)(H + 1) * Hd, ldL = (long long)(H + 1) * L, ldA = (long long)H * A;
  const long long lda1 = (long long)H * a1, lda2 = (long long)H * a2;
  const int BH = B * H;
  const bool upstream_state = g_latents || g_hiddens;
  if (do_prep) {
  if (!g_hiddens && !g_latents && !g_actions) {
    DR_TRY(zero(w.gH, (long long)((w.gA + (long long)BH * A) - w.gH), s));
  } else {
    if (g_hiddens) DR_TRY(copy2d(w.gH, Hd, g_hiddens, Hd, Hd, (long long)B * (H + 1), s));
    else DR_TRY(zero(w.gH, (long long)B * (H + 1) * Hd, s));
    if (g_latents) DR_TRY(copy2d(w.gZ, L, g_latents, L, L, (long long)B * (H + 1), s));
    else DR_TRY(zero(w.gZ, (long long)B * (H + 1) * L, s));
    if (g_actions) DR_TRY(copy2d(w.gA, A, g_actions, A, A, (long long)BH, s));
    else DR_TRY(zero(w.gA, (long long)BH * A, s));
  }
  {
    const int h1 = d->prior_h1, h2 = d->prior_h2;
    TransposeJob tj[9] = {
        {L, h2, L, wm->prior.l6.w, w.tl6p},
        {h2, h1, h2, wm->prior.l3.w, w.tl3p},
        {h1, Hd, h1, wm->prior.l0.w, w.tl0p},
        {3 * Hd, L + A, 3 * Hd, wm->w_ih, w.wt},
        {3 * Hd, Hd, 3 * Hd, wm->w_hh, w.twhh},
        {A, a2, 2 * A, ac->mu.w, w.thead},
        {A, a2, 2 * A, ac->ls.w, w.thead + A},
        {a2, a1, a2, ac->l3.w, w.tl3a},
        {a1, Hd + L, a1, ac->l0.w, w.tl0a},
    };
    DR_TRY(op_transpose_multi(tj, 9, s));
    if (B >= 128 && (3 * Hd) % 8 == 0) {
      DR_TRY(split_planes(L + A, 3 * Hd, w.wt, 3 * Hd, w.s3wt, s));
      DR_TRY(split_planes(Hd, 3 * Hd, w.twhh, 3 * Hd, w.s3twhh, s));
      if (d->actor_h1 % 8 == 0) DR_TRY(split_planes(Hd + L, d->actor_h1, w.tl0a, d->actor_h1, w.s3tl0a, s));
    }
  }
  }
  const bool planes = B >= 128 && (3 * Hd) % 8 == 0;
  if (!do_main) return DR_OK;

  bool looped = false;
  if (op_pbptt_supported(d, B, H, A)) {
    const PBpttIO io = {w.tl6p, w.tl3p, w.tl0p, w.wt, w.twhh, w.thead, w.tl3a, w.tl0a,
                        tp.soft, tp.pre2p, tp.pre1p, tp.r, tp.u, tp.n, tp.ghn, tp.pre2a, tp.pre1a, tp.ls_raw, tp.eps,
                        hiddens, actions, g_mus, g_sigmas, w.gH, w.gZ, w.gA,
                        w.gheads, w.gpre2a, w.gy2a, w.xh2a, w.gpre1a, w.gy1a, w.xh1a};
    const int rc = op_pbptt(d, wm, ac, B, H, io, w.pb, s);
    if (rc != DR_E_UNSUPPORTED && rc != DR_OK) return rc;
    looped = rc == DR_OK;
  }
  for (int t = H - 1; t >= 0 && !looped; --t) {
    const long long hb = (long long)Hd * B * t;
    float* gH_t = w.gH + (long long)t * Hd;
    float* gH_n = w.gH + (long long)(t + 1) * Hd;
    float* gZ_t = w.gZ + (long long)t * L;
    float* gZ_n = w.gZ + (long long)(t + 1) * L;
    const bool state_grad = upstream_state || t < H - 1;
    if (state_grad) {
      const int h1 = d->prior_h1, h2 = d->prior_h2;
      const int gl = d->cols / 4;
      GemmArgs gs = bwd_nt(B, h2, L, gZ_n, ldL, w.tl6p, w.gx2, h2, 0);
      if (L <= 1024 && d->cols % 4 == 0 && gl <= 64 && (gl & (gl - 1)) == 0 && gemm_bwd_rows16(&gs, 1)) {
        GemmArgs g = bwd_nt(B, h2, L, gZ_n, ldL, w.tl6p, w.gx2, h2, 0);
        g.pre = tp.soft + (long long)t * B * L;
        g.ld_pre = L;
        g.C = d->cols;
        DR_TRY(run(G_NT, AM_STEBWD, g, s));
      } else {
        DR_TRY(op_softmax_ste_bwd(B, d->rows, d->cols, gZ_n, ldL, tp.soft + (long long)t * B * L, L, w.glog, s));
        DR_TRY(run(G_NT, AM_PLAIN, bwd_nt(B, h2, L, w.glog, L, w.tl6p, w.gx2, h2, 0), s));
      }
      DR_TRY(lnbwd_nt(B, h1, h2, w.gx2, h2, tp.pre2p + (long long)t * B * h2, h2, wm->prior.n4, w.tl3p, w.gx1, h1, 0,
                      w.gp2, h2, nullptr, nullptr, nullptr, 0, INT_MAX, s));
      GruBwdEpi ge;
      memset(&ge, 0, sizeof(ge));
      ge.h = hiddens + (long long)t * Hd; ge.ldh = ldH;
      ge.r = tp.r + hb; ge.u = tp.u + hb; ge.n = tp.n + hb; ge.ghn = tp.ghn + hb;
      ge.gi = w.ggi; ge.gh = w.ggh; ge.ho = gH_t; ge.ldo = ldH; ge.Hd = Hd;
      const bool a16 = planes && d->precision == DR_PREC_BF16;
      if (a16) {
        ge.gi16 = w.ggi16;
        ge.gh16 = w.ggh16;
      }
      DR_TRY(lnbwd_nt(B, Hd, h1, w.gx1, h1, tp.pre1p + (long long)t * B * h1, h1, wm->prior.n1, w.tl0p, gH_n, ldH, 1,
                      w.gp1, h1, nullptr, nullptr, nullptr, 0, INT_MAX, s, &ge));
      if (t > 0) {
        GemmArgs p[2];
        p[0] = bwd_nt(B, L + A, 3 * Hd, w.ggi, 3 * Hd, w.wt, gZ_t, ldL, 1);
        p[0].Y2 = w.gA + (long long)t * A; p[0].ldy2 = ldA; p[0].nsplitY = L;
        p[1] = bwd_nt(B, Hd, 3 * Hd, w.ggh, 3 * Hd, w.twhh, gH_t, ldH, 1);
        if (planes) {
          wplanes(p[0], w.s3wt);
          wplanes(p[1], w.s3twhh);
        }
        if (a16) {
          p[0].A16 = w.ggi16;
          p[1].A16 = w.ggh16;
        }
        DR_TRY(gemm_launch(G_NT, AM_PLAIN, p, 2, s));
      } else {
        DR_TRY(run(G_NT, AM_PLAIN, bwd_nt(B, A, 3 * Hd, w.ggi, 3 * Hd, w.wt + (long long)L * 3 * Hd, w.gA, ldA, 1), s));
      }
    }
    const long long ot = (long long)t * A;
    float* gh_t = w.gheads + (long long)t * 2 * A;
    const long long o2 = (long long)t * a2, o1 = (long long)t * a1;
    DR_TRY(op_actor_head_bwd_x(B, A, a2, w.gA + ot, ldA, g_mus ? g_mus + ot : nullptr,
                               g_sigmas ? g_sigmas + ot : nullptr, ldA, actions + ot, ldA, tp.ls_raw + ot, ldA,
                               tp.eps + (long long)t * B * A, gh_t, (long long)H * 2 * A, w.thead, w.gx2a, a2, s));
    DR_TRY(lnbwd_nt(B, a1, a2, w.gx2a, a2, tp.pre2a + o2, lda2, ac->n4, w.tl3a, w.gx1a, a1, 0, w.gpre2a + o2, lda2,
                    w.gy2a + o2, w.xh2a + o2, nullptr, 0, INT_MAX, s));
    if (t > 0 && planes && a1 % 8 == 0) {
      const bool a16 = d->precision == DR_PREC_BF16 && lda1 % 8 == 0;
      DR_TRY(op_ln_silu_bwd(B, a1, w.gx1a, a1, tp.pre1a + o1, lda1, ac->n1.w, ac->n1.b, w.gpre1a + o1, lda1,
                            w.gy1a + o1, w.xh1a + o1, s, a16 ? w.gpre1a16 + o1 : nullptr));
      GemmArgs g = bwd_nt(B, Hd + L, a1, w.gpre1a + o1, lda1, w.tl0a, gH_t, ldH, 1);
      if (a16) g.A16 = w.gpre1a16 + o1;
      g.Y2 = gZ_t; g.ldy2 = ldL; g.nsplitY = Hd;
      wplanes(g, w.s3tl0a);
      DR_TRY(run(G_NT, AM_PLAIN, g, s));
    } else if (t > 0) {
      DR_TRY(lnbwd_nt(B, Hd + L, a1, w.gx1a, a1, tp.pre1a + o1, lda1, ac->n1, w.tl0a, gH_t, ldH, 1, w.gpre1a + o1,
                      lda1, w.gy1a + o1, w.xh1a + o1, gZ_t, ldL, Hd, s));
    } else {
      DR_TRY(op_ln_silu_bwd(B, a1, w.gx1a, a1, tp.pre1a + o1, lda1, ac->n1.w, ac->n1.b, w.gpre1a + o1, lda1,
                            w.gy1a + o1, w.xh1a + o1, s));
    }
  }
  {
    const Copy2dJob cj[2] = {{w.hcat, (long long)H * Hd, hiddens, ldH, (long long)H * Hd, B},
                             {w.zcat, (long long)H * L, latents, ldL, (long long)H * L, B}};
    DR_TRY(op_copy2d_multi(cj, 2, s));
  }
  {
    GemmArgs p[4];
    p[0] = bwd_w(a1, Hd + L, BH, w.gpre1a, a1, w.hcat, Hd, gr->l0.w);
    p[0].W2 = w.zcat; p[0].ldb2 = L; p[0].nsplitB = Hd;
    p[1] = bwd_w(a2, a1, BH, w.gpre2a, a2, tp.x1a, a1, gr->l3.w);
    p[2] = bwd_w(A, a2, BH, w.gheads, 2 * A, tp.x2a, a2, gr->mu.w);
    p[3] = bwd_w(A, a2, BH, w.gheads + A, 2 * A, tp.x2a, a2, gr->ls.w);
    float* sk = w.sk;
    long long skn = w.sk_n;
    for (int i = 0; i < 4; ++i) give_splitk(p[i], sk, skn);
    DR_TRY(tn_launch(p, 4, w.tn, w.tn_bytes, s, d->precision == DR_PREC_BF16 ? 1 : 3));
  }
  {
    ColsumJob cj[8] = {
        {a1, w.gpre1a, a1, nullptr, 0, gr->l0.b}, {a1, w.gy1a, a1, w.xh1a, a1, gr->n1.w},
        {a1, w.gy1a, a1, nullptr, 0, gr->n1.b},   {a2, w.gpre2a, a2, nullptr, 0, gr->l3.b},
        {a2, w.gy2a, a2, w.xh2a, a2, gr->n4.w},   {a2, w.gy2a, a2, nullptr, 0, gr->n4.b},
        {A, w.gheads, 2 * A, nullptr, 0, gr->mu.b}, {A, w.gheads + A, 2 * A, nullptr, 0, gr->ls.b},
    };
    DR_TRY(op_colsum_multi(BH, cj, 8, s));
  }
  return DR_OK;
}

struct CTape {
  float *pre1, *x1, *pre2, *x2, *logits;
};
static void ctape_carve(Carve& c, const dr_dims* d, int M, CTape& t) {
  t.pre1 = c.f((long long)M * d->critic_h1);
  t.x1 = c.f((long long)M * d->critic_h1);
  t.pre2 = c.f((long long)M * d->critic_h2);
  t.x2 = c.f((long long)M * d->critic_h2);
  t.logits = c.f((long long)M * d->buckets);
}

extern "C" size_t dr_critic_tape_bytes(const dr_dims* d, int M) {
  Carve c(nullptr);
  CTape t;
  ctape_carve(c, d, M, t);
  return c.off;
}

static size_t critic_ws_bytes(const dr_dims* d, int M) {
  Carve c(nullptr);
  CTape t;
  ctape_carve(c, d, M, t);
  c.f(splitk_floats(M, d->critic_h1));
  c.raw(op_nt_split3_ws_bytes(d->critic_h1, d->hidden + latent(d)));
  c.f((long long)op_gemm_nt_split3_part_floats(M, d->critic_h1));
  return c.off + 256;
}


extern "C" int dr_critic_fwd(const dr_dims* d, const dr_critic* cr, int M, const float* h, long long ldh,
                             const float* z, long long ldz, float* logits, float* values, void* tape, void* ws,
                             size_t ws_bytes, hipStream_t s) {
  DR_REQUIRE(d && cr && h && z && M > 0, "null argument or empty batch");
  GemmBf16Scope bf16_scope(d->precision == DR_PREC_BF16);
  CTape t;
  float* sk = nullptr;
  long long skn = 0;
  void* s3w = nullptr;
  float* s3part = nullptr;
  size_t s3part_n = 0;
  if (tape) {
    Carve c(tape);
    ctape_carve(c, d, M, t);
  }
  if (ws) {
    Carve c(ws);
    CTape tw;
    ctape_carve(c, d, M, tw);
    if (!tape) {
      t = tw;
      WS_CHECK(c, ws_bytes);
    }
    const long long want = splitk_floats(M, d->critic_h1);
    if (c.off + (size_t)want * sizeof(float) + 256 <= ws_bytes) {
      skn = want;
      sk = c.f(skn);
      const size_t pb = op_nt_split3_ws_bytes(d->critic_h1, d->hidden + latent(d));
      if (c.off + pb + 256 <= ws_bytes) s3w = c.raw(pb);
      const size_t pn = op_gemm_nt_split3_part_floats(M, d->critic_h1);
      if (s3w && c.off + pn * sizeof(float) + 256 <= ws_bytes) {
        s3part = c.f((long long)pn);
        s3part_n = pn;
      }
    }
  }
  DR_REQUIRE(tape || ws, "dr_critic_fwd needs a tape or a workspace");
  const int L = latent(d), Hd = d->hidden, c1 = d->critic_h1, c2 = d->critic_h2, nb = d->buckets;
  if (s3w && s3_first_layer(d, M, c1, h, ldh, z, ldz)) {
    DR_TRY(op_nt_repack_split3(c1, Hd + L, cr->net.l0.w, Hd + L, s3w, s));
    DR_TRY(op_gemm_nt_split3_sk(M, c1, Hd + L, h, (int)ldh, z, (int)ldz, Hd, s3w, cr->net.l0.b, 0, t.pre1, c1,
                                s3part, s3part_n, s));
  } else {
    GemmArgs g1 = lin2(M, c1, h, ldh, Hd, z, ldz, L, cr->net.l0.w, cr->net.l0.b, t.pre1, c1);
    give_splitk(g1, sk, skn);
    DR_TRY(run(G_NT, AM_PLAIN, g1, s));
  }
  GemmArgs g2 = lin_ln(M, c2, c1, t.pre1, c1, cr->net.n1, cr->net.l3.w, cr->net.l3.b, t.pre2, c2);
  g2.a_out = t.x1; g2.ld_aout = c1;
  DR_TRY(run(G_NT, AM_LNSILU, g2, s));
  float* lg = logits ? logits : t.logits;
  GemmArgs g3 = lin_ln(M, nb, c2, t.pre2, c2, cr->net.n4, cr->net.l6.w, cr->net.l6.b, lg, nb);
  g3.a_out = t.x2; g3.ld_aout = c2;
  DR_TRY(run(G_NT, AM_LNSILU, g3, s));
  if (tape && logits && logits != t.logits) DR_TRY(copy2d(t.logits, nb, logits, nb, nb, M, s));
  if (values) DR_TRY(op_bucket_value(M, nb, lg, nb, cr->buckets, values, 1, s));
  return DR_OK;
}

struct CBws {
  float *row_loss, *glog, *gx2, *gp2, *gy2, *xh2, *gx1, *gp1, *gy1, *xh1;
  float *tl6, *tl3;
  float* sk;
  long long sk_n;
  void* tn;
  size_t tn_bytes;
};
static void cbws_carve(Carve& c, const dr_dims* d, int B, int H, CBws& w) {
  const long long M = (long long)B * (H + 1);
  w.tn_bytes = op_gemm_tn_split3_ws_bytes(d->buckets, d->critic_h2, (int)M) +
               op_gemm_tn_split3_ws_bytes(d->critic_h2, d->critic_h1, (int)M) +
               op_gemm_tn_split3_ws_bytes(d->critic_h1, d->hidden + latent(d), (int)M);
  w.tn = c.raw(w.tn_bytes);
  w.row_loss = c.f((long long)B * H);
  w.sk_n = splitk_floats(d->buckets, d->critic_h2) + splitk_floats(d->critic_h2, d->critic_h1) +
           splitk_floats(d->critic_h1, d->hidden + latent(d));
  w.sk = c.f(w.sk_n);
  w.tl6 = c.f((long long)d->buckets * d->critic_h2);
  w.tl3 = c.f((long long)d->critic_h2 * d->critic_h1);
  w.glog = c.f(M * d->buckets);
  w.gx2 = c.f(M * d->critic_h2);
  w.gp2 = c.f(M * d->critic_h2);
  w.gy2 = c.f(M * d->critic_h2);
  w.xh2 = c.f(M * d->critic_h2);
  w.gx1 = c.f(M * d->critic_h1);
  w.gp1 = c.f(M * d->critic_h1);
  w.gy1 = c.f(M * d->critic_h1);
  w.xh1 = c.f(M * d->critic_h1);
}

extern "C" size_t dr_critic_workspace_bytes(const dr_dims* d, int B, int H) {
  Carve c(nullptr);
  CBws w;
  cbws_carve(c, d, B, H, w);
  const size_t a = c.off, b = critic_ws_bytes(d, B * (H + 1));
  return a > b ? a : b;
}

extern "C" int dr_critic_loss_bwd(const dr_dims* d, const dr_critic* cr, int B, int H, const float* hiddens,
                                  const float* latents, const float* R, const void* tape, float scale,
                                  float* loss_out, const dr_critic* gr, void* ws, size_t ws_bytes, hipStream_t s) {
  DR_REQUIRE(d && cr && hiddens && latents && R && tape && loss_out && gr && B > 0 && H > 0, "null argument");
  GemmBf16Scope bf16_scope(d->precision == DR_PREC_BF16);
  Carve c(ws);
  CBws w;
  cbws_carve(c, d, B, H, w);
  WS_CHECK(c, ws_bytes);
  const int M = B * (H + 1);
  Carve ct((void*)tape);
  CTape t;
  ctape_carve(ct, d, M, t);
  const int L = latent(d), Hd = d->hidden, c1 = d->critic_h1, c2 = d->critic_h2, nb = d->buckets;
  DR_TRY(op_critic_ce(B, H, nb, t.logits, R, cr->buckets, scale, w.row_loss, w.glog, s));
  DR_TRY(op_mean(B * H, w.row_loss, loss_out, s));
  {
    TransposeJob tj[2] = {{nb, c2, nb, cr->net.l6.w, w.tl6}, {c2, c1, c2, cr->net.l3.w, w.tl3}};
    DR_TRY(op_transpose_multi(tj, 2, s));
  }
  DR_TRY(run(G_NT, AM_PLAIN, bwd_nt(M, c2, nb, w.glog, nb, w.tl6, w.gx2, c2, 0), s));
  DR_TRY(lnbwd_nt(M, c1, c2, w.gx2, c2, t.pre2, c2, cr->net.n4, w.tl3, w.gx1, c1, 0, w.gp2, c2, w.gy2, w.xh2, nullptr,
                  0, INT_MAX, s));
  DR_TRY(op_ln_silu_bwd(M, c1, w.gx1, c1, t.pre1, c1, cr->net.n1.w, cr->net.n1.b, w.gp1, c1, w.gy1, w.xh1, s));
  {
    GemmArgs p[3];
    p[0] = bwd_w(nb, c2, M, w.glog, nb, t.x2, c2, gr->net.l6.w);
    p[1] = bwd_w(c2, c1, M, w.gp2, c2, t.x1, c1, gr->net.l3.w);
    p[2] = bwd_w(c1, Hd + L, M, w.gp1, c1, hiddens, Hd, gr->net.l0.w);
    p[2].W2 = latents; p[2].ldb2 = L; p[2].nsplitB = Hd;
    float* sk = w.sk;
    long long skn = w.sk_n;
    for (int i = 0; i < 3; ++i) give_splitk(p[i], sk, skn);
    DR_TRY(tn_launch(p, 3, w.tn, w.tn_bytes, s, d->precision == DR_PREC_BF16 ? 1 : 3));
  }
  {
    ColsumJob cj[7] = {
        {nb, w.glog, nb, nullptr, 0, gr->net.l6.b}, {c2, w.gp2, c2, nullptr, 0, gr->net.l3.b},
        {c2, w.gy2, c2, w.xh2, c2, gr->net.n4.w},   {c2, w.gy2, c2, nullptr, 0, gr->net.n4.b},
        {c1, w.gp1, c1, nullptr, 0, gr->net.l0.b},  {c1, w.gy1, c1, w.xh1, c1, gr->net.n1.w},
        {c1, w.gy1, c1, nullptr, 0, gr->net.n1.b},
    };
    DR_TRY(op_colsum_multi(M, cj, 7, s));
  }
  return DR_OK;
}

static size_t step_ws(const dr_dims* d, int B) {
  Carve c(nullptr);
  c.f((long long)B * 3 * d->hidden);
  c.f((long long)B * 3 * d->hidden);
  c.f((long long)B * latent(d));
  const int mx = d->prior_h1 > d->rew_h1 ? d->prior_h1 : d->rew_h1;
  c.f((long long)B * (mx > d->actor_h1 ? mx : d->actor_h1) * 2);
  c.f((long long)B * (d->buckets + 8) * 2);
  return c.off;
}

extern "C" size_t dr_step_workspace_bytes(const dr_dims* d, int B) { return step_ws(d, B) + 4096; }

static int mlp3(const dr_mlp3& m, int M, int in_h, const float* h, long long ldh, int in_z, const float* z,
                long long ldz, int h1, int h2, int n_out, float* out, long long ldo, float* p1, float* p2,
                hipStream_t s) {
  GemmArgs g = in_z ? lin2(M, h1, h, ldh, in_h, z, ldz, in_z, m.l0.w, m.l0.b, p1, h1)
                    : lin(M, h1, in_h, h, ldh, m.l0.w, in_h, m.l0.b, p1, h1);
  DR_TRY(run(G_NT, AM_PLAIN, g, s));
  DR_TRY(run(G_NT, AM_LNSILU, lin_ln(M, h2, h1, p1, h1, m.n1, m.l3.w, m.l3.b, p2, h2), s));
  return run(G_NT, AM_LNSILU, lin_ln(M, n_out, h2, p2, h2, m.n4, m.l6.w, m.l6.b, out, ldo), s);
}

extern "C" int dr_mlp3_fwd(const dr_mlp3* m, int M, int in_h, const float* h, long long ldh, int in_z,
                           const float* z, long long ldz, int h1, int h2, int n_out, float* out, long long ldo,
                           void* ws, size_t ws_bytes, hipStream_t s) {
  DR_REQUIRE(m && h && out && M > 0 && h1 > 0 && h2 > 0 && n_out > 0, "null argument or bad widths");
  Carve c(ws);
  float* p1 = c.f((long long)M * h1);
  float* p2 = c.f((long long)M * h2);
  WS_CHECK(c, ws_bytes);
  return mlp3(*m, M, in_h, h, ldh, in_z, z, ldz, h1, h2, n_out, out, ldo, p1, p2, s);
}

struct TraceWs {
  ObsWs o;
  float *zc, *zl;
  int* idxl;
  float *p1, *p2;
  ImWs w;
};
static void trace_carve(Carve& c, const dr_dims* d, int B, int T, TraceWs& a) {
  const long long BT = (long long)B * T;
  const int L = latent(d), Hd = d->hidden;
  obs_carve(c, d, B, a.o);
  a.zc = c.f((long long)B * L);
  a.zl = c.f((long long)B * L);
  a.idxl = c.i(2LL * B * d->rows);
  a.p1 = c.f(BT * d->prior_h1);
  a.p2 = c.f(BT * d->prior_h2);
  ImWs& w = a.w;
  memset(&w, 0, sizeof(w));
  w.p1r = c.f(BT * d->rew_h1);
  w.p1c = c.f(BT * d->cont_h1);
  w.p2r = c.f(BT * d->rew_h2);
  w.p2c = c.f(BT * d->cont_h2);
  w.rlog = c.f(BT * d->buckets);
  w.clog = c.f(BT);
  w.rval = c.f(BT);
  w.s3r = c.raw(op_nt_split3_ws_bytes(d->rew_h1, Hd + L));
  w.s3c = c.raw(op_nt_split3_ws_bytes(d->cont_h1, Hd + L));
  w.s3part_n = op_gemm_nt_split3_part_floats((int)BT, std::max(d->rew_h1, d->cont_h1));
  w.s3part = c.f((long long)w.s3part_n);
}

extern "C" size_t dr_observe_trace_workspace_bytes(const dr_dims* d, int B, int T) {
  if (!d || B <= 0 || T <= 0 || (long long)B * T > 0x7fffffffLL) return 0;
  Carve c(nullptr);
  TraceWs a;
  trace_carve(c, d, B, T, a);
  return c.off;
}

extern "C" int dr_observe_trace(const dr_dims* d, const dr_world_model* wm, int B, int T, const float* feat,
                                const float* actions, long long act_sb, long long act_st, const float* h_init,
                                const float* z_init, dr_noise noise, float* latents, float* hiddens,
                                float* post_logits, float* prior_logits, float* rewards, float* continues, void* ws,
                                size_t ws_bytes, hipStream_t s) {
  DR_REQUIRE(d && wm && feat && latents && hiddens && ws && B > 0 && T > 0, "null argument or empty batch");
  DR_REQUIRE((long long)B * T <= 0x7fffffffLL, "too many states");
  DR_REQUIRE((rewards == nullptr) == (continues == nullptr), "rewards and continues: both or neither");
  DR_REQUIRE(actions || (z_init == nullptr && T == 1), "actions required");
  GemmBf16Scope bf16_scope(d->precision == DR_PREC_BF16);
  Carve c(ws);
  TraceWs a;
  trace_carve(c, d, B, T, a);
  WS_CHECK(c, ws_bytes);
  const int L = latent(d), Hd = d->hidden;
  if (z_init != nullptr || T > 1) {
    DR_REQUIRE(wm->w_ih && wm->w_hh && wm->b_ih && wm->b_hh, "GRU weights required");
    DR_TRY(op_transpose(3 * Hd, L + d->action, wm->w_ih, a.o.wt, s));
  }
  const ObsTrace tr = {latents, hiddens, post_logits, a.zl, a.idxl};
  DR_TRY(observe_steps(d, wm, B, T, feat, actions, act_sb, act_st, h_init, z_init, noise, a.zc, nullptr, nullptr, a.o,
                       &tr, s));
  const int M = B * T;
  if (prior_logits)
    DR_TRY(mlp3(wm->prior, M, Hd, hiddens, Hd, 0, nullptr, 0, d->prior_h1, d->prior_h2, L, prior_logits, L, a.p1, a.p2,
                s));
  if (rewards) DR_TRY(imagine_heads(d, wm, B, T - 1, latents, hiddens, rewards, continues, a.w, s, true));
  return DR_OK;
}

extern "C" int dr_gru_cell(const dr_dims* d, const dr_world_model* wm, int B, const float* z, const float* h,
                           const float* a, float* h_out, void* ws, size_t ws_bytes, hipStream_t s) {
  DR_REQUIRE(d && wm && z && a && h_out && B > 0, "null argument");
  Carve c(ws);
  float* gi = c.f((long long)B * 3 * d->hidden);
  float* gh = c.f((long long)B * 3 * d->hidden);
  WS_CHECK(c, ws_bytes);
  return gru_step(d, wm, B, z, latent(d), a, d->action, h, d->hidden, h_out, d->hidden, gi, gh, nullptr, nullptr,
                  nullptr, nullptr, s);
}

extern "C" int dr_imagine_step(const dr_dims* d, const dr_world_model* wm, int B, const float* h, const float* z,
                               const float* a, dr_noise noise, float* h_out, float* z_out, float* r_out,
                               float* c_out, void* ws, size_t ws_bytes, hipStream_t s) {
  DR_REQUIRE(d && wm && z && a && h_out && z_out && B > 0, "null argument");
  const int L = latent(d), Hd = d->hidden;
  Carve c(ws);
  float* gi = c.f((long long)B * 3 * Hd);
  float* gh = c.f((long long)B * 3 * Hd);
  float* lg = c.f((long long)B * L);
// ... 65 lines not shown
```

### dreamer_amd/engine.py

```python
import contextlib
import gc

import numpy as np

import torch

from . import _lib as L
from . import hip

WARM_STREAM = 1 << 24
DREAM_STREAM = 2 << 24
_CU_STREAMS = {}


@contextlib.contextmanager
def _no_gc():
    enabled = gc.isenabled()
    gc.collect()
    gc.disable()
    try:
        yield
    finally:
        if enabled:
            gc.enable()


def cu_mask_words(n_cus, fraction):
    keep = max(1, min(n_cus, int(round(n_cus * fraction))))
    words = [0] * ((n_cus + 31) // 32)
    for i in range(keep):
        words[i // 32] |= 1 << (i % 32)
    return words


class ImaginationEngine:
    def __init__(self, dreamer, B=None, world=None, use_graph=True):
        self.dr = dreamer
        self.dev = dreamer.device
        self.B = int(B or dreamer.batch_size)
        self.S = int(dreamer.sequence_length)
        self.H = int(dreamer.horizon)
        self.T = self.S // 2
        self.world = world
        self.rank = world[0] if world else 0
        self.wsize = world[1] if world else 1
        self.dp = world is not None
        self.use_graph = use_graph
        self.graph = None
        self.graph_key = None
        self.side = torch.cuda.Stream(self.dev)
        self.chunks = [(0, self.T)]
        self._alloc()
    @staticmethod
    def warm_chunks(T, size=8):
        return [(t0, min(T, t0 + size)) for t0 in range(0, T, size)]

    def dims(self):
        return self.dr.world_model.dims(self.dr.agent)

    def _alloc(self):
        d = self.dims()
        self.d = d
        B, H, T = self.B, self.H, self.T
        L_ = d.rows * d.cols
        dev = self.dev
        f = lambda *s: torch.zeros(*s, device=dev)
        self.starts = torch.zeros(B, dtype=torch.int64, device=dev)
        self.starts_host = [torch.zeros(B, dtype=torch.int64).pin_memory() for _ in range(2)]
        self.copy_ev = [None, None]
        self.epochs = 0
        self.act_win = f(B, self.S, d.action)
        self.feat = f(T * B, d.enc_hidden)
        self.z0, self.h0 = f(B, L_), f(B, d.hidden)
        self.latents, self.hiddens = f(B, H + 1, L_), f(B, H + 1, d.hidden)
        self.actions, self.mus, self.sigmas = f(B, H, d.action), f(B, H, d.action), f(B, H, d.action)
        self.rewards, self.continues = f(B, H), f(B, H)
        self.V_t, self.V_c = f(B, H + 1), f(B, H + 1)
        self.R = f(B, H)
        self.R_all = f(self.wsize * B, H) if self.dp else self.R
        self.norm = f(1)
        self.loss_a = f(1 + B * H)
        self.g_mu, self.g_sig = f(B, H, d.action), f(B, H, d.action)
        self.sq = f(2)
        self.skip = torch.zeros(1, dtype=torch.int32, device=dev)
        M = B * (H + 1)
        self.ws_enc = hip.workspace(dev).get("e_enc", L.query("dr_encoder_workspace_bytes", d, T * B))
        self.ws_obs = hip.workspace(dev).get("e_obs", L.query("dr_observe_workspace_bytes", d, B))
        self.tape = torch.zeros(L.query("dr_imagine_tape_bytes", d, B, H), dtype=torch.uint8, device=dev)
        self.ws_im = hip.workspace(dev).get("e_im", L.query("dr_imagine_workspace_bytes", d, B, H))
        self.ctape = torch.zeros(L.query("dr_critic_tape_bytes", d, M), dtype=torch.uint8, device=dev)
        self.ws_cr = hip.workspace(dev).get("e_cr", L.query("dr_critic_workspace_bytes", d, B, H))
        self.ws_cr2 = hip.workspace(dev).get("e_cr2", L.query("dr_critic_workspace_bytes", d, B, H))
        self.rng = hip.rng(dev)

    def encode_and_warm(self, frames, noise_q=None):
        d, st = self.d, hip.stream()
        wm = self.dr.world_model.packed()
        L.call("dr_encoder_features", d, wm, frames, self.B, self.T, L.ptr(self.feat), L.ptr(self.ws_enc),
               self.ws_enc.numel(), st)
        if noise_q is not None:
            nz = hip.explicit_noise(q=noise_q, device=self.dev)
        else:
            nz = L.dr_noise(None, None, self.rng.state.data_ptr(), self.rank * self.B, WARM_STREAM)
        A = d.action
        L.call("dr_observe_scan", d, wm, self.B, self.T, L.ptr(self.feat), L.ptr(self.act_win), self.S * A, A, None,
               None, nz, L.ptr(self.z0), L.ptr(self.h0), None, L.ptr(self.ws_obs), self.ws_obs.numel(), st)

    def imagine(self, eps=None, q=None, deterministic=False, z0=None, h0=None, d=None):
        d = self.d if d is None else d
        z0 = self.z0 if z0 is None else z0
        h0 = self.h0 if h0 is None else h0
        if eps is not None or q is not None:
            nz = hip.explicit_noise(q=q, eps=eps, device=self.dev)
        else:
            nz = L.dr_noise(None, None, self.rng.state.data_ptr(), self.rank * self.B, DREAM_STREAM)
        L.call("dr_imagine_fwd", d, self.dr.world_model.packed(), self.dr.agent.actor_struct(), self.B, self.H,
               L.ptr(z0), L.ptr(h0), nz, int(deterministic), L.ptr(self.latents), L.ptr(self.hiddens),
               L.ptr(self.actions), L.ptr(self.rewards), L.ptr(self.continues), L.ptr(self.mus),
               L.ptr(self.sigmas), L.ptr(self.tape), L.ptr(self.ws_im), self.ws_im.numel(), hip.stream())

    def returns(self):
        ag, d, st = self.dr.agent, self.d, hip.stream()
        M = self.B * (self.H + 1)
        L_ = d.rows * d.cols
        L.call("dr_critic_fwd", d, ag.critic_struct(target=True), M, L.ptr(self.hiddens), d.hidden,
               L.ptr(self.latents), L_, None, L.ptr(self.V_t), None, L.ptr(self.ws_cr), self.ws_cr.numel(), st)
        L.call("dr_lambda_returns", self.B, self.H, L.ptr(self.rewards), L.ptr(self.continues), L.ptr(self.V_t),
               ag.gamma, ag.lambda_, L.ptr(self.R), st)

    def losses_and_grads(self, fork=True):
        ag, d = self.dr.agent, self.d
        main = torch.cuda.current_stream(self.dev)
        st = main.cuda_stream
        B, H = self.B, self.H
        M = B * (H + 1)
        L_ = d.rows * d.cols
        scale = 1.0 / float(B * self.wsize * H)
        L.call("dr_critic_fwd", d, ag.critic_struct(), M, L.ptr(self.hiddens), d.hidden, L.ptr(self.latents), L_,
               None, L.ptr(self.V_c), L.ptr(self.ctape), L.ptr(self.ws_cr), self.ws_cr.numel(), st)
        critic_args = (d, ag.critic_struct(), B, H, L.ptr(self.hiddens), L.ptr(self.latents), L.ptr(self.R),
                       L.ptr(self.ctape), scale, L.ptr(ag.loss_slot(1)), ag.critic_struct(grad=True),
                       L.ptr(self.ws_cr), self.ws_cr.numel())
        if fork:
            self.side.wait_stream(main)
            L.call("dr_critic_loss_bwd", *critic_args, self.side.cuda_stream)
        L.call("dr_update_S", self.R_all.numel(), L.ptr(self.R_all), L.ptr(ag.S_dev), L.ptr(self.norm), None, 0, st)
        L.call("dr_actor_loss_grad", B, H, d.action, L.ptr(self.mus), L.ptr(self.sigmas), L.ptr(self.actions),
               L.ptr(self.R), L.ptr(self.V_c), L.ptr(self.norm), ag.nu, scale, L.ptr(self.loss_a), L.ptr(self.g_mu),
               L.ptr(self.g_sig), st)
        if not fork:
            L.call("dr_critic_loss_bwd", *critic_args, st)
        L.call("dr_imagine_bwd", d, self.dr.world_model.packed(), ag.actor_struct(), B, H, L.ptr(self.latents),
               L.ptr(self.hiddens), L.ptr(self.actions), L.ptr(self.g_mu), L.ptr(self.g_sig), None, None, None,
               L.ptr(self.tape), ag.actor_struct(grad=True), L.ptr(self.ws_im), self.ws_im.numel(), st)
        ag.loss_slot(0).copy_(self.loss_a[0:1])
        if fork:
            main.wait_stream(self.side)

    def _x_critic_fwd_and_prep(self):
        ag, d, st = self.dr.agent, self.d, hip.stream()
        M = self.B * (self.H + 1)
        L.call("dr_critic_fwd", d, ag.critic_struct(), M, L.ptr(self.hiddens), d.hidden, L.ptr(self.latents),
               d.rows * d.cols, None, L.ptr(self.V_c), L.ptr(self.ctape), L.ptr(self.ws_cr2), self.ws_cr2.numel(),
               st)
        L.call("dr_imagine_bwd_prep", d, self.dr.world_model.packed(), ag.actor_struct(), self.B, self.H, None,
               None, None, L.ptr(self.ws_im), self.ws_im.numel(), st)

    def _actor_loss(self):
        ag, d, st = self.dr.agent, self.d, hip.stream()
        B, H = self.B, self.H
        scale = 1.0 / float(B * self.wsize * H)
        L.call("dr_update_S", self.R_all.numel(), L.ptr(self.R_all), L.ptr(ag.S_dev), L.ptr(self.norm), None, 0, st)
        L.call("dr_actor_loss_grad", B, H, d.action, L.ptr(self.mus), L.ptr(self.sigmas), L.ptr(self.actions),
               L.ptr(self.R), L.ptr(self.V_c), L.ptr(self.norm), ag.nu, scale, L.ptr(self.loss_a), L.ptr(self.g_mu),
               L.ptr(self.g_sig), st)

    def _x_critic_bwd(self):
        ag, d = self.dr.agent, self.d
        B, H = self.B, self.H
        scale = 1.0 / float(B * self.wsize * H)
        L.call("dr_critic_loss_bwd", d, ag.critic_struct(), B, H, L.ptr(self.hiddens), L.ptr(self.latents),
               L.ptr(self.R), L.ptr(self.ctape), scale, L.ptr(ag.loss_slot(1)), ag.critic_struct(grad=True),
               L.ptr(self.ws_cr2), self.ws_cr2.numel(), hip.stream())

    def _bptt(self, d=None):
        ag, d = self.dr.agent, (self.d if d is None else d)
        L.call("dr_imagine_bwd_main", d, self.dr.world_model.packed(), ag.actor_struct(), self.B, self.H,
               L.ptr(self.latents), L.ptr(self.hiddens), L.ptr(self.actions), L.ptr(self.g_mu), L.ptr(self.g_sig),
               0, L.ptr(self.tape), ag.actor_struct(grad=True), L.ptr(self.ws_im), self.ws_im.numel(), hip.stream())
        ag.loss_slot(0).copy_(self.loss_a[0:1])

    def optimise(self):
        self.dr.agent.fused_optimiser_step(self.sq, self.skip)

    def _encode_chunk(self, t0, t1, stream_ptr):
        d = self.d
        fr = self.dr.buffer.frames_struct(self.starts)
        fr.t0 = t0
        off = t0 * self.B * d.enc_hidden * 4
        L.call("dr_encoder_features", d, self.dr.world_model.packed(), fr, self.B, t1 - t0,
               L.ptr(self.feat) + off, L.ptr(self.ws_enc), self.ws_enc.numel(), stream_ptr)

    def _scan_chunk(self, t0, t1, stream_ptr):
        d, A = self.d, self.d.action
        nz = L.dr_noise(None, None, self.rng.state.data_ptr(), self.rank * self.B, WARM_STREAM + t0)
        feat = L.ptr(self.feat) + t0 * self.B * d.enc_hidden * 4
        if t0 == 0:
            acts, zi, hi = L.ptr(self.act_win), None, None
        else:
            acts, zi, hi = L.ptr(self.act_win) + (t0 - 1) * A * 4, L.ptr(self.z0), L.ptr(self.h0)
        L.call("dr_observe_scan", d, self.dr.world_model.packed(), self.B, t1 - t0, feat, acts, self.S * A, A,
               hi, zi, nz, L.ptr(self.z0), L.ptr(self.h0), None, L.ptr(self.ws_obs), self.ws_obs.numel(),
               stream_ptr)

    def _ph_encwarm(self):
        main = torch.cuda.current_stream(self.dev)
        self.dr.buffer.gather_actions(self.starts, self.act_win)
        self.side.wait_stream(main)
        done = []
        with torch.cuda.stream(self.side):
            for t0, t1 in self.chunks:
                self._encode_chunk(t0, t1, self.side.cuda_stream)
                ev = torch.cuda.Event()
                ev.record(self.side)
                done.append(ev)
        for (t0, t1), ev in zip(self.chunks, done):
            main.wait_event(ev)
            self._scan_chunk(t0, t1, main.cuda_stream)

    def time_encoder(self, reps=5):
        st = torch.cuda.current_stream(self.dev)
        for t0, t1 in self.chunks:
            self._encode_chunk(t0, t1, st.cuda_stream)
        a, b = torch.cuda.Event(enable_timing=True), torch.cuda.Event(enable_timing=True)
        a.record(st)
        for _ in range(reps):
            for t0, t1 in self.chunks:
                self._encode_chunk(t0, t1, st.cuda_stream)
        b.record(st)
        b.synchronize()
        return a.elapsed_time(b) / reps

    def _ph_update(self):
        self.losses_and_grads(fork=False)

    def _ph_optim(self):
        self.optimise()
        L.call("dr_rng_advance", self.rng.state.data_ptr(), 1, hip.stream())

    def phases(self):
        ph = [("encwarm", self._ph_encwarm, None), ("imagine", self.imagine, None),
              ("returns", self.returns, self._allgather_R if self.dp else None),
              ("update", self._ph_update, self._allreduce_grads if self.dp else None),
              ("optim", self._ph_optim, None)]
        if self.dp and not self.persistent_bptt():
            ph[3:4] = [("critic", self._ph_critic, self._allreduce_critic_async),
                       ("actor", self._ph_actor, self._allreduce_actor)]
        return ph

    def persistent_chain(self):
        return bool(L.query("dr_persistent_kernels", self.d, self.B, self.T, self.H) & 2)

    def persistent_bptt(self):
        return bool(L.query("dr_persistent_kernels", self.d, self.B, self.T, self.H) & 4)

    def check_faults(self, wait=True):
        h, _ = self.dr.agent.fault_host()
        if wait:
            torch.cuda.current_stream(self.dev).synchronize()
        if int(h[0]) != 0:
            self._on_fault()

    def _on_fault(self):
        ag = self.dr.agent
        torch.cuda.synchronize(self.dev)
        ag.fault_slot().zero_()
        ag.fault_host()[0][0] = 0
        ag.persistent_ok = False
        self.d = self.dims()
        self.graph, self.graph_key, self._pipe = None, None, None
        raise RuntimeError("dreamer_amd: a persistent kernel (posterior scan / imagination unroll / BPTT) timed out "
                           "waiting on another workgroup (not every workgroup was resident, e.g. other work held "
                           "CUs); its outputs were NaN and that epoch's actor-critic update was skipped. Every "
                           "later epoch runs the launch form.")

    def _ph_critic(self):
        ag, d, st = self.dr.agent, self.d, hip.stream()
        B, H = self.B, self.H
        M = B * (H + 1)
        scale = 1.0 / float(B * self.wsize * H)
        L.call("dr_critic_fwd", d, ag.critic_struct(), M, L.ptr(self.hiddens), d.hidden, L.ptr(self.latents),
               d.rows * d.cols, None, L.ptr(self.V_c), L.ptr(self.ctape), L.ptr(self.ws_cr), self.ws_cr.numel(), st)
        self._actor_loss()
        L.call("dr_critic_loss_bwd", d, ag.critic_struct(), B, H, L.ptr(self.hiddens), L.ptr(self.latents),
               L.ptr(self.R), L.ptr(self.ctape), scale, L.ptr(ag.loss_slot(1)), ag.critic_struct(grad=True),
               L.ptr(self.ws_cr), self.ws_cr.numel(), st)
        ag.loss_slot(0).copy_(self.loss_a[0:1])

    def _ph_actor(self):
        ag, d = self.dr.agent, self.d
        L.call("dr_imagine_bwd", d, self.dr.world_model.packed(), ag.actor_struct(), self.B, self.H,
               L.ptr(self.latents), L.ptr(self.hiddens), L.ptr(self.actions), L.ptr(self.g_mu), L.ptr(self.g_sig),
               None, None, None, L.ptr(self.tape), ag.actor_struct(grad=True), L.ptr(self.ws_im), self.ws_im.numel(),
               hip.stream())

    def epoch_body(self):
        for _, body, coll in self.phases():
            body()
            if coll is not None:
                coll()

    def _allgather_R(self):
        import torch.distributed as dist
        parts = list(self.R_all.view(self.wsize, self.B, self.H).unbind(0))
        dist.all_gather(parts, self.R, group=self.world[2])

    def _allreduce_grads(self):
        import torch.distributed as dist
        ag = self.dr.agent
        dist.all_reduce(ag.grad_buffer, op=dist.ReduceOp.SUM, group=self.world[2])
        ag.loss_buffer.div_(self.wsize)

    def _allreduce_critic_async(self):
        import torch.distributed as dist
        ag = self.dr.agent
        na = ag.fa.grad.numel()
        self._critic_work = dist.all_reduce(ag.grad_buffer[na:], op=dist.ReduceOp.SUM, group=self.world[2],
                                            async_op=True)

    def _allreduce_actor(self):
        import torch.distributed as dist
        ag = self.dr.agent
        na = ag.fa.grad.numel()
        dist.all_reduce(ag.grad_buffer[:na], op=dist.ReduceOp.SUM, group=self.world[2])
        self._critic_work.wait()
        self._critic_work = None
        ag.loss_buffer.div_(self.wsize)

    def run(self, starts_np, timing=False):
        self.check_faults(wait=False)
        i = self.epochs & 1
        if self.copy_ev[i] is not None:
            self.copy_ev[i].synchronize()
        self.starts_host[i].copy_(torch.from_numpy(np.asarray(starts_np, dtype=np.int64)))
        self.starts.copy_(self.starts_host[i], non_blocking=True)
        self.copy_ev[i] = torch.cuda.Event()
        self.copy_ev[i].record()
        self.epochs += 1
        ag = self.dr.agent
        key = (ag.params_key(), self.dr.world_model.params_key(), self.dr.buffer.device_key())
        if self.use_graph and (self.graph is None or self.graph_key != key):
            self._capture(key)
        evs = [torch.cuda.Event(enable_timing=True)] if timing else None
        if evs:
            evs[0].record()
        for k, (name, body, coll) in enumerate(self.phases()):
            if self.use_graph:
                self.graph[k].replay()
            else:
                body()
            if coll is not None:
                coll()
            if evs:
                e = torch.cuda.Event(enable_timing=True)
                e.record()
                evs.append(e)
        self.last_events = evs
        return ag.loss_slot(0), ag.loss_slot(1)

    def phase_ms(self):
        names = [p[0] for p in self.phases()]
        ev = self.last_events
        return {n: ev[k].elapsed_time(ev[k + 1]) for k, n in enumerate(names)}

    def warm_stream(self, cu_fraction=None):
        import ctypes
        import os
        if cu_fraction is None:
            cu_fraction = float(os.environ.get("DREAMER_WARM_CUS", "0.875"))
        if not 0.0 < cu_fraction < 1.0:
            return torch.cuda.Stream(self.dev)
        n = ctypes.c_int(0)
        with torch.cuda.device(self.dev):
            L.call("dr_device_cus", ctypes.byref(n))
            words = cu_mask_words(n.value, cu_fraction)
            ck = (torch.device(self.dev).index, tuple(words))
            h = _CU_STREAMS.get(ck)
            if h is None:
                mask = (ctypes.c_uint * len(words))(*words)
                h = ctypes.c_void_p()
                L.call("dr_stream_create_cumask", len(words), mask, ctypes.byref(h))
                _CU_STREAMS[ck] = h
        return torch.cuda.ExternalStream(h.value, device=self.dev)

    def _pipe_capture(self, key):
        dev, B, H = self.dev, self.B, self.H
        if getattr(self, "_pipe", None) is None:
            self._pipe = dict(
                stream=self.warm_stream(), side=torch.cuda.Stream(dev),
                rng=torch.zeros(2, dtype=torch.int64, device=dev),
                z0=[self.z0, torch.zeros_like(self.z0)],
                h0=[self.h0, torch.zeros_like(self.h0)],
                key=None)
        P = self._pipe
        if P["key"] == key:
            return P
        d, A = self.d, self.d.action
        dw = L.dr_dims.from_buffer_copy(d)
        dw.launch_form = 1

        def warm(s):
            st = torch.cuda.current_stream(dev).cuda_stream
            self.dr.buffer.gather_actions(self.starts, self.act_win)
            self._encode_chunk(0, self.T, st)
            nz = L.dr_noise(None, None, P["rng"].data_ptr(), self.rank * B, WARM_STREAM)
            L.call("dr_observe_scan", dw, self.dr.world_model.packed(), B, self.T, L.ptr(self.feat),
                   L.ptr(self.act_win), self.S * A, A, None, None, nz, L.ptr(P["z0"][s]), L.ptr(P["h0"][s]), None,
                   L.ptr(self.ws_obs), self.ws_obs.numel(), st)
            L.call("dr_rng_advance", P["rng"].data_ptr(), 1, st)

        cs = torch.cuda.Stream(dev)
        cs.wait_stream(torch.cuda.current_stream(dev))
        graphs = {}
        with _no_gc(), torch.cuda.stream(cs):
            for s in (0, 1):
                for name, body in (("warm", lambda s=s: warm(s)),
                                   ("imagine", lambda s=s: self.imagine(z0=P["z0"][s], h0=P["h0"][s], d=dw))):
                    g = torch.cuda.CUDAGraph()
                    with torch.cuda.graph(g, stream=cs):
                        body()
                    graphs[(name, s)] = g
            for name, body in (("returns", self.returns), ("xfwd", self._x_critic_fwd_and_prep),
                               ("actor_loss", self._actor_loss), ("xbwd", self._x_critic_bwd),
                               ("bptt", lambda: self._bptt(d=dw)), ("optim", self._ph_optim)):
                g = torch.cuda.CUDAGraph()
                with torch.cuda.graph(g, stream=cs):
                    body()
                graphs[name] = g
        torch.cuda.current_stream(dev).wait_stream(cs)
        P["graphs"], P["key"] = graphs, key
        return P

    def run_many(self, starts_list):
        self.check_faults(wait=False)
        ag = self.dr.agent
        key = (ag.params_key(), self.dr.world_model.params_key(), self.dr.buffer.device_key())
        P = self._pipe_capture(key)
        G = P["graphs"]
        outer = torch.cuda.current_stream(self.dev)
        import os
        fenced = 0.0 < float(os.environ.get("DREAMER_WARM_CUS", "0.875")) < 1.0
        prio = int(os.environ.get("DREAMER_CHAIN_PRIORITY", "-1" if fenced else "0"))
        if prio != 0:
            if P.get("chain") is None or P.get("chain_prio") != prio:
                P["chain"], P["chain_prio"] = torch.cuda.Stream(self.dev, priority=prio), prio
            P["chain"].wait_stream(outer)
            with torch.cuda.stream(P["chain"]):
                losses = self._run_many(P, G, starts_list, P["chain"])
            outer.wait_stream(P["chain"])
        else:
            losses = self._run_many(P, G, starts_list, outer)
        return losses

    def _run_many(self, P, G, starts_list, main):
        import os
        K = len(starts_list)
        ag = self.dr.agent
        ws = P["stream"]
        host = torch.from_numpy(np.stack([np.asarray(x, dtype=np.int64) for x in starts_list])).pin_memory()
        losses = torch.empty(K, 2, device=self.dev)
        ws.wait_stream(main)
        with torch.cuda.stream(ws):
            dst = host.to(self.dev, non_blocking=True)
            P["rng"].copy_(self.rng.state)
        ev_w, ev_i = [None] * K, [None] * K
        warm0_main = os.environ.get("DREAMER_WARM0_MAIN", "1") == "1"

        def issue_warm(e):
            s = main if (e == 0 and warm0_main) else ws
            if s is main:
                main.wait_stream(ws)
            elif e == 1 and warm0_main:
                ws.wait_event(ev_w[0])
            with torch.cuda.stream(s):
                if e >= 2:
                    s.wait_event(ev_i[e - 2])
                self.starts.copy_(dst[e])
                G[("warm", e & 1)].replay()
                ev_w[e] = torch.cuda.Event()
                ev_w[e].record(s)

        xs = P["side"]
        import os
        side = os.environ.get("DREAMER_SIDE", "none")

        def record(stream):
            ev = torch.cuda.Event()
            ev.record(stream)
            return ev

        issue_warm(0)
        for e in range(K):
            if e + 1 < K:
                issue_warm(e + 1)
            main.wait_event(ev_w[e])
            G[("imagine", e & 1)].replay()
            ev_i[e] = record(main)
            s1 = xs if side in ("both", "fwd") else main
            s2 = xs if side in ("both", "bwd") else main
            if s1 is xs:
                xs.wait_event(ev_i[e])
            with torch.cuda.stream(s1):
                G["xfwd"].replay()
            ev_x1 = record(s1)
            G["returns"].replay()
            if self.dp:
                self._allgather_R()
            ev_r = record(main)
            main.wait_event(ev_x1)
            G["actor_loss"].replay()
            if s2 is xs:
                xs.wait_event(record(main) if s1 is main else ev_r)
            with torch.cuda.stream(s2):
                G["xbwd"].replay()
            ev_x2 = record(s2)
            G["bptt"].replay()
            main.wait_event(ev_x2)
            if self.dp:
                self._allreduce_grads()
            G["optim"].replay()
            losses[e].copy_(ag.loss_buffer[0:2])
        main.wait_stream(ws)
        main.wait_stream(xs)
        self.epochs += K
        self._pipe_host = host
        return losses

    def _capture(self, key):
        s = torch.cuda.Stream(self.dev)
        s.wait_stream(torch.cuda.current_stream(self.dev))
        graphs = []
        with _no_gc(), torch.cuda.stream(s):
            for _, body, _ in self.phases():
                g = torch.cuda.CUDAGraph()
                with torch.cuda.graph(g, stream=s):
                    body()
                graphs.append(g)
        torch.cuda.current_stream(self.dev).wait_stream(s)
        self.graph, self.graph_key = graphs, key
```

### include/dreamer_hip.h

```cpp
#ifndef DREAMER_HIP_H
#define DREAMER_HIP_H

#include <hip/hip_runtime.h>
#include <stddef.h>

#ifdef __cplusplus
extern "C" {
#endif

#define DR_OK 0
#define DR_E_INVALID 1001
#define DR_E_HIP 1002
#define DR_E_WORKSPACE 1003
#define DR_E_UNSUPPORTED 1004

typedef struct { float* w; float* b; } dr_linear;

typedef struct { dr_linear l0, n1, l3, n4, l6; } dr_mlp3;

typedef struct {
  int hidden;
  int rows, cols;
  int action;
  int img_h, img_w;
  int enc_f1, enc_f2;
  int enc_hidden;
  int prior_h1, prior_h2, rew_h1, rew_h2, cont_h1, cont_h2;
  int actor_h1, actor_h2, critic_h1, critic_h2;
  int buckets;
  int dec_f1, dec_f2;
  int dec_hidden;
  int precision;
  int obs_dim;
  int enc_depth;
  int launch_form;
  float* fault;
  unsigned* fault_host;
} dr_dims;
#define DR_MAX_DEPTH 5
#define DR_PREC_FP32 0
#define DR_PREC_BF16 1

typedef struct {
  dr_linear conv[DR_MAX_DEPTH];
  dr_linear map0, map1, map3;
  float *w_ih, *w_hh, *b_ih, *b_hh;
  dr_mlp3 prior;
  dr_mlp3 reward;
  dr_mlp3 cont;
  float* buckets_rew;
} dr_world_model;

typedef struct {
  dr_linear up0, up1, up3;
  dr_linear convt[DR_MAX_DEPTH];
} dr_decoder;

typedef struct { dr_linear l0, n1, l3, n4, mu, ls; } dr_actor;

typedef struct { dr_mlp3 net; float* buckets; } dr_critic;

typedef struct {
  const float* q;
  const float* eps;
  const unsigned long long* rng;
  int row0;
  int stream;
} dr_noise;

typedef struct {
  const unsigned char* ring;
  long long ring_cap;
  const long long* starts;
  const float* obs;
  long long stride_b, stride_t;
  int raw255;
  int t0;
} dr_frames;

const char* dr_last_error(void);
int dr_version(void);

int dr_stream_create_cumask(int n_words, const unsigned* mask, hipStream_t* out);
int dr_stream_destroy(hipStream_t s);
int dr_device_cus(int* out);
int dr_host_device_ptr(void* host, void** dev);

size_t dr_encoder_workspace_bytes(const dr_dims* d, int n_frames);
int dr_encoder_features(const dr_dims* d, const dr_world_model* wm, const dr_frames* src, int B, int T,
                        float* feat, void* ws, size_t ws_bytes, hipStream_t stream);

size_t dr_observe_workspace_bytes(const dr_dims* d, int B);
int dr_observe_scan(const dr_dims* d, const dr_world_model* wm, int B, int T, const float* feat,
                    const float* actions, long long act_sb, long long act_st, const float* h_init,
                    const float* z_init, dr_noise noise, float* z_out, float* h_out, float* logits_out,
                    void* ws, size_t ws_bytes, hipStream_t stream);

size_t dr_observe_trace_workspace_bytes(const dr_dims* d, int B, int T);
int dr_observe_trace(const dr_dims* d, const dr_world_model* wm, int B, int T, const float* feat,
                     const float* actions, long long act_sb, long long act_st, const float* h_init,
                     const float* z_init, dr_noise noise, float* latents, float* hiddens, float* post_logits,
                     float* prior_logits, float* rewards, float* continues, void* ws, size_t ws_bytes,
                     hipStream_t stream);

size_t dr_imagine_tape_bytes(const dr_dims* d, int B, int H);
size_t dr_imagine_workspace_bytes(const dr_dims* d, int B, int H);
int dr_imagine_fwd(const dr_dims* d, const dr_world_model* wm, const dr_actor* actor, int B, int H,
                   const float* z0, const float* h0, dr_noise noise, int deterministic, float* latents,
                   float* hiddens, float* actions, float* rewards, float* continues, float* mus,
                   float* sigmas, void* tape, void* ws, size_t ws_bytes, hipStream_t stream);

size_t dr_imagine_actions_workspace_bytes(const dr_dims* d, int B, int H);
int dr_imagine_actions(const dr_dims* d, const dr_world_model* wm, int B, int H, const float* z0, const float* h0,
                       const float* actions, long long act_sb, long long act_st, dr_noise noise, float* latents,
                       float* hiddens, float* rewards, float* continues, void* ws, size_t ws_bytes,
                       hipStream_t stream);

int dr_imagine_bwd(const dr_dims* d, const dr_world_model* wm, const dr_actor* actor, int B, int H,
                   const float* latents, const float* hiddens, const float* actions, const float* g_mus,
                   const float* g_sigmas,
                   const float* g_actions, const float* g_latents, const float* g_hiddens,
                   const void* tape, const dr_actor* grad, void* ws, size_t ws_bytes, hipStream_t stream);
int dr_imagine_bwd_prep(const dr_dims* d, const dr_world_model* wm, const dr_actor* actor, int B, int H,
                        const float* g_actions, const float* g_latents, const float* g_hiddens, void* ws,
                        size_t ws_bytes, hipStream_t stream);
int dr_imagine_bwd_main(const dr_dims* d, const dr_world_model* wm, const dr_actor* actor, int B, int H,
                        const float* latents, const float* hiddens, const float* actions, const float* g_mus,
                        const float* g_sigmas, int upstream_state, const void* tape, const dr_actor* grad, void* ws,
                        size_t ws_bytes, hipStream_t stream);

int dr_imagine_step(const dr_dims* d, const dr_world_model* wm, int B, const float* h, const float* z,
                    const float* a, dr_noise noise, float* h_out, float* z_out, float* r_out, float* c_out,
                    void* ws, size_t ws_bytes, hipStream_t stream);
size_t dr_actor_act_workspace_bytes(const dr_dims* d, int B);
int dr_actor_act(const dr_dims* d, const dr_actor* actor, int B, const float* h, const float* z,
                 dr_noise noise, int deterministic, float* a_out, float* mu_out, float* sigma_out, void* ws,
                 size_t ws_bytes, hipStream_t stream);
size_t dr_act_step_workspace_bytes(const dr_dims* d);
int dr_act_step(const dr_dims* d, const dr_world_model* wm, const dr_actor* actor, const unsigned char* frame,
                int has_prev, const float* z_prev, const float* h, const float* a_prev, dr_noise noise,
                int deterministic, float* z_out, float* h_out, float* a_out, float* mu_out, float* sigma_out,
                float* logits_out, int* status, void* ws, size_t ws_bytes, hipStream_t stream);
#define DR_ACT_MAX_ENVS 16
size_t dr_act_batch_workspace_bytes(const dr_dims* d, int n_env);
int dr_act_batch(const dr_dims* d, const dr_world_model* wm, const dr_actor* actor, int n_env,
                 const unsigned char* frames, const unsigned char* first, const float* z_prev, const float* h,
                 const float* a_prev, dr_noise noise, int deterministic, float* z_out, float* h_out, float* a_out,
                 float* mu_out, float* sigma_out, float* logits_out, int* status, void* ws, size_t ws_bytes,
                 hipStream_t stream);
#define DR_ACT_VEC_MAX_OBS 1023
size_t dr_act_vec_workspace_bytes(const dr_dims* d, int n_env);
int dr_act_vec(const dr_dims* d, const dr_world_model* wm, const dr_actor* actor, int n_env, const float* obs,
               const unsigned char* first, const float* z_prev, const float* h, const float* a_prev, dr_noise noise,
               int deterministic, float* z_out, float* h_out, float* a_out, float* mu_out, float* sigma_out,
               float* logits_out, int* status, void* ws, size_t ws_bytes, hipStream_t stream);

int dr_gru_cell(const dr_dims* d, const dr_world_model* wm, int B, const float* z, const float* h,
                const float* a, float* h_out, void* ws, size_t ws_bytes, hipStream_t stream);
int dr_categorical_sample(int M, int R, int C, const float* logits, dr_noise noise, float* z_out,
                          int* idx_out, float* soft_out, hipStream_t stream);
int dr_mlp3_fwd(const dr_mlp3* m, int M, int in_h, const float* h, long long ldh, int in_z, const float* z,
                long long ldz, int h1, int h2, int n_out, float* out, long long ldo, void* ws, size_t ws_bytes,
                hipStream_t stream);
size_t dr_step_workspace_bytes(const dr_dims* d, int B);
int dr_bucket_value(int M, int nb, const float* logits, const float* buckets, float* out, hipStream_t stream);

size_t dr_critic_tape_bytes(const dr_dims* d, int M);
size_t dr_critic_workspace_bytes(const dr_dims* d, int B, int H);
int dr_critic_fwd(const dr_dims* d, const dr_critic* c, int M, const float* h, long long ldh, const float* z,
                  long long ldz, float* logits, float* values, void* tape, void* ws, size_t ws_bytes,
                  hipStream_t stream);
int dr_lambda_returns(int B, int H, const float* r, const float* c, const float* V, float gamma, float lam,
                      float* R, hipStream_t stream);
int dr_update_S(int n, const float* R, float* S, float* norm_out, void* ws, size_t ws_bytes,
                hipStream_t stream);
int dr_actor_loss_grad(int B, int H, int A, const float* mus, const float* sigmas, const float* actions,
                       const float* R, const float* V, const float* norm, float nu, float scale,
                       float* loss_out, float* g_mus, float* g_sigmas, hipStream_t stream);
int dr_critic_loss_bwd(const dr_dims* d, const dr_critic* c, int B, int H, const float* hiddens,
                       const float* latents, const float* R, const void* tape, float scale, float* loss_out,
                       const dr_critic* grad, void* ws, size_t ws_bytes, hipStream_t stream);

int dr_sqnorm(long long n, const float* g, float* acc, hipStream_t stream);
int dr_sqnorm_multi(long long n, const float* g, float* acc, float* scratch, hipStream_t stream);
#define DR_CLIP_SCRATCH_FLOATS 1024
int dr_clip_stats(long long na, const float* ga, long long nb, const float* gb, int nloss, const float* loss,
                  float* sq, int* skip, void* scratch, hipStream_t stream);
int dr_adamw(long long n, float* p, float* g, float* m, float* v, const float* sqnorm, float max_norm,
             double lr, double b1, double b2, double eps, double wd, int* step, float* hyper, const int* skip,
             hipStream_t stream);
int dr_ema(long long n, float* target, const float* src, float keep, float tau, const int* skip,
           hipStream_t stream);
int dr_ac_optimiser_step(long long na, float* pa, float* ga, float* ma, float* va, int* step_a, float* hyper_a,
                         double lr_a, double b1_a, double b2_a, double eps_a, double wd_a, long long nc, float* pc,
                         float* gc, float* mc, float* vc, int* step_c, float* hyper_c, double lr_c, double b1_c,
                         double b2_c, double eps_c, double wd_c, float max_norm, float* target, float ema_keep,
                         float tau, int nloss, const float* loss, float* sq, int* skip, void* scratch,
                         hipStream_t stream);
int dr_nonfinite(long long n, const float* x, int* flag, hipStream_t stream);

typedef struct {
  const float* actions; long long act_sb, act_st;
  const float* rewards; const float* continues; long long rc_sb, rc_st;
} dr_wm_batch;
typedef struct { float beta_pred, beta_dyn, beta_rep; } dr_wm_loss_cfg;
size_t dr_wm_train_workspace_bytes(const dr_dims* d, int B, int T);
#define DR_WM_PREP 1
#define DR_WM_FWD 2
#define DR_WM_BWD 4
#define DR_WM_BWD_HEADS 8
#define DR_WM_BWD_SCAN 16
#define DR_WM_BWD_ENC 32
int dr_wm_train_phase(const dr_dims* d, const dr_world_model* wm, const dr_decoder* dec, int B, int T,
                      const dr_frames* src, const dr_wm_batch* batch, dr_noise noise, dr_wm_loss_cfg cfg, int phases,
                      float* stats, int rows_global, float* losses, int* skip, const dr_world_model* g_wm,
                      const dr_decoder* g_dec, float* hiddens_out, float* latents_out, float* post_logits_out,
                      void* ws, size_t ws_bytes, hipStream_t stream);
int dr_wm_train_grads(const dr_dims* d, const dr_world_model* wm, const dr_decoder* dec, int B, int T,
                      const dr_frames* src, const dr_wm_batch* batch, dr_noise noise, dr_wm_loss_cfg cfg,
                      float* losses, int* skip, const dr_world_model* g_wm, const dr_decoder* g_dec,
                      float* hiddens_out, float* latents_out, float* post_logits_out, void* ws, size_t ws_bytes,
                      hipStream_t stream);

size_t dr_decoder_workspace_bytes(const dr_dims* d, int M);
int dr_decoder_fwd(const dr_dims* d, const dr_decoder* dec, int M, const float* h, long long ldh, const float* z,
                   long long ldz, float* mu, void* ws, size_t ws_bytes, hipStream_t stream);

int dr_frame_metrics(const dr_dims* d, int B, int T, const float* mu, const dr_frames* truth, float* sqerr,
                     unsigned char* pred_u8, unsigned char* true_u8, hipStream_t stream);

int dr_frame_ssim(const dr_dims* d, int B, int T, const float* mu, const dr_frames* truth, float* ssim,
                  float* ssim_ch, hipStream_t stream);

int dr_ensemble_metrics(const dr_dims* d, int B, int M, int T, const float* mu, const dr_frames* truth,
                        float* sqerr_mean, float* spread, unsigned char* mean_u8, unsigned char* std_u8,
                        float* mean_f32, hipStream_t stream);

int dr_latent_stats(int M, int R, int C, const float* post_logits, const float* prior_logits, float* kl,
                    float* post_entropy, float* prior_entropy, float* kl_groups, hipStream_t stream);
// ... 33 lines not shown
```

Before: 613,000 imagined latent-steps/s.

## Prepare repacked and transposed weights once per update in a shared block

Adds a prepared-weights block that dr_prepare_weights fills once per epoch, and again after the optimizer step for actor and critic. It holds the split3-packed and transposed copies of the encoder, GRU, prior, head, actor and critic weights. Kernels that used to repack or transpose weights on every call now read from this block, which removes many small repack launches. The multi-repack kernel also gains tiled transpose, transposed-split3 and copy job kinds plus a vectorized split3 packer. The cost is extra device memory, validation bookkeeping on each call, and a repack that still runs once per update.

```diff
diff --git a/dreamer_amd/_lib.py b/dreamer_amd/_lib.py
--- a/dreamer_amd/_lib.py
+++ b/dreamer_amd/_lib.py
@@ -25,7 +25,7 @@
         "hidden", "rows", "cols", "action", "img_h", "img_w", "enc_f1", "enc_f2", "enc_hidden",
         "prior_h1", "prior_h2", "rew_h1", "rew_h2", "cont_h1", "cont_h2",
         "actor_h1", "actor_h2", "critic_h1", "critic_h2", "buckets", "dec_f1", "dec_f2", "dec_hidden", "precision", "obs_dim", "enc_depth",
-        "launch_form")] + [("fault", fp), ("fault_host", fp)]
+        "launch_form")] + [("fault", fp), ("fault_host", fp), ("prepared", fp), ("prepared_bytes", C.c_size_t)]
 
 DR_MAX_DEPTH = 5
 
@@ -77,6 +77,9 @@
 _SIGS = {
     "dr_last_error": (C.c_char_p, []),
     "dr_version": (_i, []),
+    "dr_prepared_bytes": (_sz, [_P(dr_dims), _i, _i, _i]),
+    "dr_prepare_weights": (_i, [_P(dr_dims), _P(dr_world_model), _P(dr_actor), _P(dr_critic), _P(dr_critic),
+                                _i, _i, _i, fp, _sz, fp]),
     "dr_encoder_workspace_bytes": (_sz, [_P(dr_dims), _i]),
     "dr_encoder_features": (_i, [_P(dr_dims), _P(dr_world_model), _P(dr_frames), _i, _i, fp, fp, _sz, fp]),
     "dr_observe_workspace_bytes": (_sz, [_P(dr_dims), _i]),
diff --git a/dreamer_amd/csrc/conv.h b/dreamer_amd/csrc/conv.h
--- a/dreamer_amd/csrc/conv.h
+++ b/dreamer_amd/csrc/conv.h
@@ -56,7 +56,7 @@
 int op_enc12_split3_ex(int n, int nb, int h, int w, int c1, int c2, const dr_frames* src, const float* w1,
                        const float* b1, const float* w2, const float* b2, void* wr1, void* wr2, float* out,
                        float* pre0, float* a0, float* pre1, hipStream_t s, int terms = 3, int prepacked = 0);
-enum { RJ_CONV1 = 0, RJ_CONV = 1, RJ_NT = 2, RJ_BF16 = 3 };
+enum { RJ_CONV1 = 0, RJ_CONV = 1, RJ_NT = 2, RJ_BF16 = 3, RJ_T = 4, RJ_TNT = 5, RJ_COPY = 6 };
 struct RepackJob {
   int kind, a, b, c;
   const float* w;
@@ -64,11 +64,14 @@
   long long ld;
   long long total;
 };
-#define DR_RJ_MAX 6
+#define DR_RJ_MAX 36
 RepackJob rj_conv1(int cout, const float* w, void* wr);
 RepackJob rj_conv(int cout, int cin, const float* w, void* wr);
 RepackJob rj_nt(int N, int K, const float* W, int ldw, void* wr);
 RepackJob rj_bf16(int rows, int cols, const float* x, long long ld, void* y);
+RepackJob rj_t(int rows, int cols, const float* in, float* out, int ldo);
+RepackJob rj_tnt(int N, int K, const float* in, long long ld, void* wr);
+RepackJob rj_copy(int rows, int cols, const float* in, long long ld, float* out, int ldo);
 int op_repack_multi(const RepackJob* jobs, int n, hipStream_t s);
 int op_enc12_bf16(int n, int nb, int h, int w, int c1, int c2, const dr_frames* src, const void* wr1, const float* b1,
                   const void* wr2, const float* b2, void* out, hipStream_t s);
diff --git a/dreamer_amd/csrc/conv_split.hip b/dreamer_amd/csrc/conv_split.hip
--- a/dreamer_amd/csrc/conv_split.hip
+++ b/dreamer_amd/csrc/conv_split.hip
@@ -1841,6 +1841,22 @@
   wr[base + plane] = (u16)mm;
   wr[base + 2 * plane] = (u16)ll;
 }
+__device__ __forceinline__ void nt_repack_split3_quad(long long i, int N, int K, int Np, const float* __restrict__ W,
+                                                      long long ldw, u16* __restrict__ wr) {
+  const int KQ = (K + 31) / 32 * 8;
+  const int n = (int)(i / KQ), k = 4 * (int)(i - (long long)n * KQ);
+  unsigned h[4], m[4], l[4];
+#pragma unroll
+  for (int j = 0; j < 4; ++j) {
+    h[j] = m[j] = l[j] = 0;
+    if (n < N && k + j < K) split3(W[(long long)n * ldw + k + j], h[j], m[j], l[j]);
+  }
+  const long long plane = (long long)Np * 32;
+  const long long base = ((long long)(k >> 5) * 3 * Np + n) * 32 + (k & 31);
+  *reinterpret_cast<uint2*>(wr + base) = make_uint2(h[0] | (h[1] << 16), h[2] | (h[3] << 16));
+  *reinterpret_cast<uint2*>(wr + base + plane) = make_uint2(m[0] | (m[1] << 16), m[2] | (m[3] << 16));
+  *reinterpret_cast<uint2*>(wr + base + 2 * plane) = make_uint2(l[0] | (l[1] << 16), l[2] | (l[3] << 16));
+}
 __global__ void k_nt_repack_split3(int N, int K, int Np, const float* __restrict__ W, int ldw, u16* __restrict__ wr) {
   const long long i = (long long)blockIdx.x * blockDim.x + threadIdx.x;
   if (i >= (long long)((K + 31) / 32) * 32 * Np) return;
@@ -1854,18 +1870,66 @@
 };
 __global__ __launch_bounds__(256) void k_repack_multi(RepackBatch b) {
   __shared__ __attribute__((aligned(16))) RepackJob J;
+  __shared__ float tile[32][33];
   int z = 0;
 #pragma unroll
   for (int i = 1; i < DR_RJ_MAX; ++i)
     if ((int)blockIdx.x >= b.blk0[i]) z = i;
   dr_stage_args(b.j[z], J, threadIdx.x);
-  const long long i = (long long)(blockIdx.x - b.blk0[z]) * 256 + threadIdx.x;
+  const int blk = (int)blockIdx.x - b.blk0[z];
+  if (J.kind == RJ_T || J.kind == RJ_TNT) {
+    const int tx = threadIdx.x & 31, ty = threadIdx.x >> 5;
+    if (J.kind == RJ_T) {
+      const int tcx = (J.b + 31) / 32;
+      const int bx = (blk % tcx) * 32, by = (blk / tcx) * 32;
+      for (int k = ty; k < 32; k += 8) {
+        const int r = by + k, c = bx + tx;
+        tile[k][tx] = (r < J.a && c < J.b) ? J.w[(long long)r * J.b + c] : 0.f;
+      }
+      __syncthreads();
+      float* out = static_cast<float*>(J.out);
+      for (int k = ty; k < 32; k += 8) {
+        const int c = bx + k, r = by + tx;
+        if (c < J.b && r < J.a) out[(long long)c * J.c + r] = tile[tx][k];
+      }
+      return;
+    }
+    const int N = J.a, K = J.b, Np = J.c;
+    const int tn = Np / 32;
+    const int kc = blk / tn, n0 = (blk - kc * tn) * 32;
+    for (int kk = ty; kk < 32; kk += 8) {
+      const int k = kc * 32 + kk, n = n0 + tx;
+      tile[kk][tx] = (n < N && k < K) ? J.w[(long long)k * J.ld + n] : 0.f;
+    }
+    __syncthreads();
+    u16* wr = static_cast<u16*>(J.out);
+    const long long plane = (long long)Np * 32;
+    const int nn = threadIdx.x >> 3, kq = 4 * (threadIdx.x & 7);
+    const int n = n0 + nn;
+    unsigned h[4], m[4], l[4];
+#pragma unroll
+    for (int j = 0; j < 4; ++j) {
+      h[j] = m[j] = l[j] = 0;
+      if (n < N && kc * 32 + kq + j < K) split3(tile[kq + j][nn], h[j], m[j], l[j]);
+    }
+    const long long base = ((long long)kc * 3 * Np + n) * 32 + kq;
+    *reinterpret_cast<uint2*>(wr + base) = make_uint2(h[0] | (h[1] << 16), h[2] | (h[3] << 16));
+    *reinterpret_cast<uint2*>(wr + base + plane) = make_uint2(m[0] | (m[1] << 16), m[2] | (m[3] << 16));
+    *reinterpret_cast<uint2*>(wr + base + 2 * plane) = make_uint2(l[0] | (l[1] << 16), l[2] | (l[3] << 16));
+    return;
+  }
+  const long long i = (long long)blk * 256 + threadIdx.x;
   if (i >= J.total) return;
   u16* out = static_cast<u16*>(J.out);
   switch (J.kind) {
     case RJ_CONV1: conv1_repack_split3_elem((int)i, J.a, J.w, out); break;
     case RJ_CONV: conv_repack_split3_elem((int)i, J.a, J.b, J.w, out); break;
-    case RJ_NT: nt_repack_split3_elem(i, J.a, J.b, J.c, J.w, J.ld, out); break;
+    case RJ_NT: nt_repack_split3_quad(i, J.a, J.b, J.c, J.w, J.ld, out); break;
+    case RJ_COPY: {
+      const int rr = (int)(i / J.b), cc = (int)(i - (long long)rr * J.b);
+      static_cast<float*>(J.out)[(long long)rr * J.c + cc] = J.w[(long long)rr * J.ld + cc];
+      break;
+    }
     default: {
       const int rr = (int)(i / J.b), cc = (int)(i - (long long)rr * J.b);
       out[i] = __builtin_bit_cast(u16, (__bf16)J.w[(long long)rr * J.ld + cc]);
@@ -1879,10 +1943,20 @@
 }
 RepackJob rj_nt(int N, int K, const float* W, int ldw, void* wr) {
   const int Np = (N + 127) / 128 * 128;
-  return {RJ_NT, N, K, Np, W, wr, ldw, (long long)((K + 31) / 32) * 32 * Np};
+  return {RJ_NT, N, K, Np, W, wr, ldw, (long long)((K + 31) / 32) * 8 * Np};
 }
 RepackJob rj_bf16(int rows, int cols, const float* x, long long ld, void* y) {
   return {RJ_BF16, rows, cols, 0, x, y, ld, (long long)rows * cols};
+}
+RepackJob rj_t(int rows, int cols, const float* in, float* out, int ldo) {
+  return {RJ_T, rows, cols, ldo, in, out, 0, 256LL * ((rows + 31) / 32) * ((cols + 31) / 32)};
+}
+RepackJob rj_tnt(int N, int K, const float* in, long long ld, void* wr) {
+  const int Np = (N + 127) / 128 * 128;
+  return {RJ_TNT, N, K, Np, in, wr, ld, 256LL * ((K + 31) / 32) * (Np / 32)};
+}
+RepackJob rj_copy(int rows, int cols, const float* in, long long ld, float* out, int ldo) {
+  return {RJ_COPY, rows, cols, ldo, in, out, ld, (long long)rows * cols};
 }
 
 int op_repack_multi(const RepackJob* jobs, int n, hipStream_t s) {
@@ -1892,16 +1966,21 @@
   }
   if (n == 0) return DR_OK;
   RepackBatch b = {};
-  int tot = 0;
+  long long tot = 0;
   for (int i = 0; i < DR_RJ_MAX; ++i) {
-    b.blk0[i] = tot;
+    b.blk0[i] = (int)tot;
     if (i < n) {
       b.j[i] = jobs[i];
-      tot += (int)((jobs[i].total + 255) / 256);
-    }
-  }
-  b.blk0[DR_RJ_MAX] = tot;
+      tot += (jobs[i].total + 255) / 256;
+    }
+    if (tot > INT_MAX) {
+      dr_set_error("repack_multi: too many elements");
+      return DR_E_INVALID;
+    }
+  }
+  b.blk0[DR_RJ_MAX] = (int)tot;
   b.n = n;
+  if (tot == 0) return DR_OK;
   hipLaunchKernelGGL(k_repack_multi, dim3((unsigned)tot), dim3(256), 0, s, b);
   return dr_check_launch("repack_multi");
 }
diff --git a/dreamer_amd/csrc/engine.hip b/dreamer_amd/csrc/engine.hip
--- a/dreamer_amd/csrc/engine.hip
+++ b/dreamer_amd/csrc/engine.hip
@@ -3,11 +3,336 @@
 #include "dream.h"
 #include "bptt.h"
 
+#include <cstddef>
+#include <mutex>
+
 
 static bool s3_first_layer(const dr_dims* d, int M, int N, const float* h, long long ldh, const float* z,
                            long long ldz) {
   return d->precision != DR_PREC_BF16 && M >= 1024 && ldh < INT_MAX && ldz < INT_MAX &&
          op_gemm_nt_split3_supported(M, N, d->hidden + latent(d), h, (int)ldh, z, (int)ldz, d->hidden, N);
+}
+
+static bool chain_planes(const dr_dims* d, int B, int steps) { return B >= 128 && steps > 1 && d->hidden % 8 == 0; }
+static bool bwd_planes(const dr_dims* d, int B) { return B >= 128 && (3 * d->hidden) % 8 == 0; }
+static bool actor_zgather(const dr_dims* d) { return d->rows <= 32 && d->actor_h1 % 4 == 0; }
+
+struct PrepPlan {
+  bool enc_c1, enc_s3[DR_MAX_DEPTH], enc_proj;
+  bool obs_planes, im_planes, heads_s3, bwd_pl, zg, a0_planes, tl0a_planes, critic_s3;
+};
+struct Prep {
+  void* enc_wr[DR_MAX_DEPTH];
+  void* enc_proj;
+  float* wt;
+  void *s3m0, *s3whh, *s3p0, *s3r, *s3c;
+  float *tl6p, *tl3p, *tl0p, *twhh;
+  void *s3wt, *s3twhh;
+  float *tl0, *wst, *bst, *thead, *tl3a;
+  void *s3a0, *s3tl0a;
+  void* s3v[2];
+  float *tl6, *tl3;
+};
+
+static const float* prep_dummy() { return reinterpret_cast<const float*>((uintptr_t)256); }
+
+static void prep_plan(const dr_dims* d, int B, int T, int H, PrepPlan& p) {
+  memset(&p, 0, sizeof(p));
+  const int L = latent(d), Hd = d->hidden;
+  if (d->obs_dim == 0 && vae_depth_ok(d)) {
+    const bool bf = d->precision == DR_PREC_BF16;
+    int e[DR_MAX_DEPTH + 1];
+    const int N = enc_chans(d, e);
+    const int n = B * T;
+    dr_frames ring;
+    memset(&ring, 0, sizeof(ring));
+    ring.ring = (decltype(ring.ring))prep_dummy();
+    ring.starts = (decltype(ring.starts))prep_dummy();
+    ring.ring_cap = 1;
+    p.enc_c1 = N >= 2 && op_enc12_split3_ok(n, d->img_h, d->img_w, e[1], e[2], &ring);
+    for (int k = 1; k < N; ++k) {
+      const bool s3 = op_conv_split3_supported(n, e[k], d->img_h >> k, d->img_w >> k, e[k + 1]);
+      p.enc_s3[k] = k == 1 ? (p.enc_c1 || (!bf && s3)) : s3;
+    }
+    const int F = enc_feat_dim(d);
+    p.enc_proj = bf || (n >= 1024 && op_gemm_nt_split3_supported(n, d->enc_hidden, F, prep_dummy(), F, nullptr, 0, F,
+                                                                  d->enc_hidden));
+  }
+  p.obs_planes = chain_planes(d, B, T);
+  p.im_planes = chain_planes(d, B, H);
+  const int M1 = B * (H + 1);
+  p.heads_s3 = s3_first_layer(d, M1, d->rew_h1, prep_dummy(), Hd, prep_dummy(), L) &&
+               s3_first_layer(d, M1, d->cont_h1, prep_dummy(), Hd, prep_dummy(), L);
+  p.bwd_pl = bwd_planes(d, B);
+  p.zg = actor_zgather(d);
+  p.a0_planes = p.im_planes && p.zg;
+  p.tl0a_planes = p.bwd_pl && d->actor_h1 % 8 == 0;
+  p.critic_s3 = s3_first_layer(d, M1, d->critic_h1, prep_dummy(), Hd, prep_dummy(), L);
+}
+
+static void prep_carve(Carve& c, const dr_dims* d, const PrepPlan& p, Prep& w) {
+  memset(&w, 0, sizeof(w));
+  const int L = latent(d), Hd = d->hidden, A = d->action, a1 = d->actor_h1, a2 = d->actor_h2;
+  if (d->obs_dim == 0 && vae_depth_ok(d)) {
+    int e[DR_MAX_DEPTH + 1];
+    const int N = enc_chans(d, e);
+    const int F = enc_feat_dim(d);
+    if (p.enc_c1) w.enc_wr[0] = c.raw((size_t)e[1] * 64 * 6);
+    for (int k = 1; k < N; ++k)
+      if (p.enc_s3[k]) w.enc_wr[k] = c.raw((size_t)e[k + 1] * e[k] * 16 * 6);
+    if (p.enc_proj)
+      w.enc_proj = d->precision == DR_PREC_BF16 ? c.raw((size_t)d->enc_hidden * F * 2)
+                                                : c.raw(op_nt_split3_ws_bytes(d->enc_hidden, F));
+  }
+  w.wt = c.f((long long)(L + A) * 3 * Hd);
+  if (p.obs_planes) w.s3m0 = c.raw(op_nt_split3_ws_bytes(d->enc_hidden, Hd));
+  if (p.obs_planes || p.im_planes) w.s3whh = c.raw(op_nt_split3_ws_bytes(3 * Hd, Hd));
+  if (p.im_planes) w.s3p0 = c.raw(op_nt_split3_ws_bytes(d->prior_h1, Hd));
+  if (p.heads_s3) {
+    w.s3r = c.raw(op_nt_split3_ws_bytes(d->rew_h1, Hd + L));
+    w.s3c = c.raw(op_nt_split3_ws_bytes(d->cont_h1, Hd + L));
+  }
+  w.tl6p = c.f((long long)L * d->prior_h2);
+  w.tl3p = c.f((long long)d->prior_h2 * d->prior_h1);
+  w.tl0p = c.f((long long)d->prior_h1 * Hd);
+  w.twhh = c.f((long long)3 * Hd * Hd);
+  if (p.bwd_pl) {
+    w.s3wt = c.raw(op_nt_split3_ws_bytes(L + A, 3 * Hd));
+    w.s3twhh = c.raw(op_nt_split3_ws_bytes(Hd, 3 * Hd));
+  }
+  w.tl0 = c.f((long long)a1 * (Hd + L));
+  w.wst = c.f((long long)2 * A * a2);
+  w.bst = c.f((long long)2 * A);
+  w.thead = c.f((long long)2 * A * a2);
+  w.tl3a = c.f((long long)a2 * a1);
+  if (p.a0_planes) w.s3a0 = c.raw(op_nt_split3_ws_bytes(a1, Hd));
+  if (p.tl0a_planes) w.s3tl0a = c.raw(op_nt_split3_ws_bytes(Hd + L, a1));
+  if (p.critic_s3) {
+    w.s3v[0] = c.raw(op_nt_split3_ws_bytes(d->critic_h1, Hd + L));
+    w.s3v[1] = c.raw(op_nt_split3_ws_bytes(d->critic_h1, Hd + L));
+  }
+  w.tl6 = c.f((long long)d->buckets * d->critic_h2);
+  w.tl3 = c.f((long long)d->critic_h2 * d->critic_h1);
+}
+
+struct PrepNote {
+  void* block;
+  size_t bytes;
+  dr_dims d;
+  int B, T, H;
+  const void *wm, *ac, *cr, *tc;
+  unsigned long long age;
+};
+#define DR_PREP_NOTES 64
+static std::mutex g_prep_mu;
+static PrepNote g_prep[DR_PREP_NOTES];
+static unsigned long long g_prep_age = 0;
+
+static bool prep_same_dims(const dr_dims& a, const dr_dims& b) { return memcmp(&a, &b, offsetof(dr_dims, launch_form)) == 0; }
+
+static int prep_get(const dr_dims* d, const char* fn, int B, int T, int H, const dr_world_model* wm,
+                    const dr_actor* ac, Prep& P, PrepNote* note = nullptr) {
+  PrepNote n;
+  bool found = false;
+  {
+    std::lock_guard<std::mutex> g(g_prep_mu);
+    for (int i = 0; i < DR_PREP_NOTES && !found; ++i)
+      if (g_prep[i].block == d->prepared) {
+        n = g_prep[i];
+        found = true;
+      }
+  }
+  const char* why = nullptr;
+  if (!found) why = "dr_dims.prepared is no block dr_prepare_weights filled";
+  else if (!prep_same_dims(n.d, *d)) why = "the block was prepared for other dims";
+  else if ((B >= 0 && B != n.B) || (T >= 0 && T != n.T) || (H >= 0 && H != n.H))
+    why = "the block was prepared for another shape (B, T, H)";
+  else if (d->prepared_bytes < n.bytes) why = "dr_dims.prepared_bytes is smaller than the block";
+  else if (wm && n.wm != (const void*)wm->map0.w) why = "the block's world-model part was not prepared from these weights";
+  else if (ac && n.ac != (const void*)ac->l0.w) why = "the block's actor part was not prepared from these weights";
+  if (why) {
+    dr_set_error("%s: %s", fn, why);
+    return DR_E_INVALID;
+  }
+  PrepPlan pl;
+  prep_plan(d, n.B, n.T, n.H, pl);
+  Carve c(d->prepared);
+  prep_carve(c, d, pl, P);
+  if (note) *note = n;
+  return DR_OK;
+}
+#define PREP_NEED(p)                                                                  \
+  do {                                                                                \
+    if (!(p)) {                                                                       \
+      dr_set_error("%s: the prepared block holds no %s for this call", __func__, #p); \
+      return DR_E_INVALID;                                                            \
+    }                                                                                 \
+  } while (0)
+
+extern "C" size_t dr_prepared_bytes(const dr_dims* d, int B, int T, int H) {
+  if (!d || B <= 0 || T <= 0 || H <= 0) return 0;
+  PrepPlan pl;
+  prep_plan(d, B, T, H, pl);
+  Carve c(nullptr);
+  Prep w;
+  prep_carve(c, d, pl, w);
+  return c.off;
+}
+
+extern "C" int dr_prepare_weights(const dr_dims* d, const dr_world_model* wm, const dr_actor* ac, const dr_critic* critic,
+                                  const dr_critic* target_critic, int B, int T, int H, void* out, size_t bytes,
+                                  hipStream_t s) {
+  DR_REQUIRE(d && out && B > 0 && T > 0 && H > 0, "null argument or empty shape");
+  DR_REQUIRE((long long)B * T < INT_MAX && (long long)B * (H + 1) < INT_MAX, "too many rows");
+  PrepPlan pl;
+  prep_plan(d, B, T, H, pl);
+  Carve c(out);
+  Prep w;
+  prep_carve(c, d, pl, w);
+  WS_CHECK(c, bytes);
+  const int L = latent(d), Hd = d->hidden, A = d->action, a1 = d->actor_h1, a2 = d->actor_h2;
+  RepackJob rj[DR_RJ_MAX];
+  int nj = 0;
+  if (wm) {
+    if (d->obs_dim == 0 && vae_depth_ok(d) && wm->conv[0].w) {
+      int e[DR_MAX_DEPTH + 1];
+      const int N = enc_chans(d, e);
+      const int F = enc_feat_dim(d);
+      if (pl.enc_c1) rj[nj++] = rj_conv1(e[1], wm->conv[0].w, w.enc_wr[0]);
+      for (int k = 1; k < N; ++k)
+        if (pl.enc_s3[k]) rj[nj++] = rj_conv(e[k + 1], e[k], wm->conv[k].w, w.enc_wr[k]);
+      if (pl.enc_proj)
+        rj[nj++] = d->precision == DR_PREC_BF16 ? rj_bf16(d->enc_hidden, F, wm->map0.w, F + Hd, w.enc_proj)
+                                                : rj_nt(d->enc_hidden, F, wm->map0.w, F + Hd, w.enc_proj);
+    }
+    DR_REQUIRE(wm->w_ih && wm->w_hh && wm->map0.w, "GRU weights required");
+    const int F = enc_feat_dim(d);
+    rj[nj++] = rj_t(3 * Hd, L + A, wm->w_ih, w.wt, 3 * Hd);
+    if (pl.obs_planes) rj[nj++] = rj_nt(d->enc_hidden, Hd, wm->map0.w + F, F + Hd, w.s3m0);
+    if (w.s3whh) rj[nj++] = rj_nt(3 * Hd, Hd, wm->w_hh, Hd, w.s3whh);
+    if (pl.im_planes) rj[nj++] = rj_nt(d->prior_h1, Hd, wm->prior.l0.w, Hd, w.s3p0);
+    if (pl.heads_s3) {
+      rj[nj++] = rj_nt(d->rew_h1, Hd + L, wm->reward.l0.w, Hd + L, w.s3r);
+      rj[nj++] = rj_nt(d->cont_h1, Hd + L, wm->cont.l0.w, Hd + L, w.s3c);
+    }
+    rj[nj++] = rj_t(L, d->prior_h2, wm->prior.l6.w, w.tl6p, L);
+    rj[nj++] = rj_t(d->prior_h2, d->prior_h1, wm->prior.l3.w, w.tl3p, d->prior_h2);
+    rj[nj++] = rj_t(d->prior_h1, Hd, wm->prior.l0.w, w.tl0p, d->prior_h1);
+    rj[nj++] = rj_t(3 * Hd, Hd, wm->w_hh, w.twhh, 3 * Hd);
+    if (pl.bwd_pl) {
+      rj[nj++] = rj_tnt(L + A, 3 * Hd, wm->w_ih, L + A, w.s3wt);
+      rj[nj++] = rj_tnt(Hd, 3 * Hd, wm->w_hh, Hd, w.s3twhh);
+    }
+  }
+  if (ac) {
+    rj[nj++] = rj_t(a1, Hd + L, ac->l0.w, w.tl0, a1);
+    rj[nj++] = rj_copy(A, a2, ac->mu.w, a2, w.wst, a2);
+    rj[nj++] = rj_copy(A, a2, ac->ls.w, a2, w.wst + (long long)A * a2, a2);
+    rj[nj++] = rj_copy(1, A, ac->mu.b, A, w.bst, A);
+    rj[nj++] = rj_copy(1, A, ac->ls.b, A, w.bst + A, A);
+    rj[nj++] = rj_t(A, a2, ac->mu.w, w.thead, 2 * A);
+    rj[nj++] = rj_t(A, a2, ac->ls.w, w.thead + A, 2 * A);
+    rj[nj++] = rj_t(a2, a1, ac->l3.w, w.tl3a, a2);
+    if (pl.a0_planes) rj[nj++] = rj_nt(a1, Hd, ac->l0.w, Hd + L, w.s3a0);
+    if (pl.tl0a_planes) rj[nj++] = rj_tnt(Hd + L, a1, ac->l0.w, Hd + L, w.s3tl0a);
+  }
+  const dr_critic* crs[2] = {critic, target_critic};
+  for (int i = 0; i < 2; ++i)
+    if (crs[i] && pl.critic_s3) rj[nj++] = rj_nt(d->critic_h1, Hd + L, crs[i]->net.l0.w, Hd + L, w.s3v[i]);
+  if (critic) {
+    rj[nj++] = rj_t(d->buckets, d->critic_h2, critic->net.l6.w, w.tl6, d->buckets);
+    rj[nj++] = rj_t(d->critic_h2, d->critic_h1, critic->net.l3.w, w.tl3, d->critic_h2);
+  }
+  {
+    std::lock_guard<std::mutex> g(g_prep_mu);
+    int slot = 0;
+    bool same = false;
+    for (int i = 0; i < DR_PREP_NOTES; ++i) {
+      if (g_prep[i].block == out) {
+        slot = i;
+        same = g_prep[i].B == B && g_prep[i].T == T && g_prep[i].H == H && prep_same_dims(g_prep[i].d, *d);
+        break;
+      }
+      if (g_prep[i].age < g_prep[slot].age) slot = i;
+    }
+    PrepNote& n = g_prep[slot];
+    if (!same) memset(&n, 0, sizeof(n));
+    n.block = out;
+    n.bytes = c.off;
+    n.d = *d;
+    n.B = B; n.T = T; n.H = H;
+    if (wm) n.wm = wm->map0.w;
+    if (ac) n.ac = ac->l0.w;
+    if (critic) n.cr = critic->net.l0.w;
+    if (target_critic) n.tc = target_critic->net.l0.w;
+    n.age = ++g_prep_age;
+  }
+  return op_repack_multi(rj, nj, s);
+}
+
+extern "C" int dr_internal_prepare_reference(const dr_dims* d, const dr_world_model* wm, const dr_actor* ac,
+                                             const dr_critic* critic, const dr_critic* target_critic, int B, int T,
+                                             int H, void* out, size_t bytes, hipStream_t s) {
+  DR_REQUIRE(d && out && B > 0 && T > 0 && H > 0, "null argument or empty shape");
+  PrepPlan pl;
+  prep_plan(d, B, T, H, pl);
+  Carve c(out);
+  Prep w;
+  prep_carve(c, d, pl, w);
+  WS_CHECK(c, bytes);
+  const int L = latent(d), Hd = d->hidden, A = d->action, a1 = d->actor_h1, a2 = d->actor_h2;
+  if (wm) {
+    const int F = enc_feat_dim(d);
+    if (d->obs_dim == 0 && vae_depth_ok(d) && wm->conv[0].w) {
+      int e[DR_MAX_DEPTH + 1];
+      const int N = enc_chans(d, e);
+      RepackJob rj[DR_MAX_DEPTH + 1];
+      int nj = 0;
+      if (pl.enc_c1) rj[nj++] = rj_conv1(e[1], wm->conv[0].w, w.enc_wr[0]);
+      for (int k = 1; k < N; ++k)
+        if (pl.enc_s3[k]) rj[nj++] = rj_conv(e[k + 1], e[k], wm->conv[k].w, w.enc_wr[k]);
+      if (pl.enc_proj && d->precision == DR_PREC_BF16)
+        rj[nj++] = rj_bf16(d->enc_hidden, F, wm->map0.w, F + Hd, w.enc_proj);
+      else if (pl.enc_proj)
+        DR_TRY(op_nt_repack_split3(d->enc_hidden, F, wm->map0.w, F + Hd, w.enc_proj, s));
+      DR_TRY(op_repack_multi(rj, nj, s));
+    }
+    DR_TRY(op_transpose(3 * Hd, L + A, wm->w_ih, w.wt, s));
+    DR_TRY(split_planes(d->enc_hidden, Hd, wm->map0.w + F, F + Hd, w.s3m0, s));
+    DR_TRY(split_planes(3 * Hd, Hd, wm->w_hh, Hd, w.s3whh, s));
+    DR_TRY(split_planes(d->prior_h1, Hd, wm->prior.l0.w, Hd, w.s3p0, s));
+    if (pl.heads_s3) {
+      DR_TRY(op_nt_repack_split3(d->rew_h1, Hd + L, wm->reward.l0.w, Hd + L, w.s3r, s));
+      DR_TRY(op_nt_repack_split3(d->cont_h1, Hd + L, wm->cont.l0.w, Hd + L, w.s3c, s));
+    }
+    const int h1 = d->prior_h1, h2 = d->prior_h2;
+    TransposeJob tj[4] = {{L, h2, L, wm->prior.l6.w, w.tl6p},
+                          {h2, h1, h2, wm->prior.l3.w, w.tl3p},
+                          {h1, Hd, h1, wm->prior.l0.w, w.tl0p},
+                          {3 * Hd, Hd, 3 * Hd, wm->w_hh, w.twhh}};
+    DR_TRY(op_transpose_multi(tj, 4, s));
+    DR_TRY(split_planes(L + A, 3 * Hd, w.wt, 3 * Hd, w.s3wt, s));
+    DR_TRY(split_planes(Hd, 3 * Hd, w.twhh, 3 * Hd, w.s3twhh, s));
+  }
+  if (ac) {
+    TransposeJob tj[4] = {{a1, Hd + L, a1, ac->l0.w, w.tl0},
+                          {A, a2, 2 * A, ac->mu.w, w.thead},
+                          {A, a2, 2 * A, ac->ls.w, w.thead + A},
+                          {a2, a1, a2, ac->l3.w, w.tl3a}};
+    DR_TRY(op_transpose_multi(tj, 4, s));
+    DR_TRY(stack_heads(ac, A, a2, w.wst, w.bst, s));
+    DR_TRY(split_planes(a1, Hd, ac->l0.w, Hd + L, w.s3a0, s));
+    DR_TRY(split_planes(Hd + L, a1, w.tl0, a1, w.s3tl0a, s));
+  }
+  const dr_critic* crs[2] = {critic, target_critic};
+  for (int i = 0; i < 2; ++i)
+    if (crs[i] && pl.critic_s3) DR_TRY(op_nt_repack_split3(d->critic_h1, Hd + L, crs[i]->net.l0.w, Hd + L, w.s3v[i], s));
+  if (critic) {
+    const int nb = d->buckets, c1 = d->critic_h1, c2 = d->critic_h2;
+    TransposeJob tj[2] = {{nb, c2, nb, critic->net.l6.w, w.tl6}, {c2, c1, c2, critic->net.l3.w, w.tl3}};
+    DR_TRY(op_transpose_multi(tj, 2, s));
+  }
+  return DR_OK;
 }
 
 struct EncWs {
@@ -56,28 +381,47 @@
 }
 
 static int encoder_bf16(const dr_dims* d, const dr_world_model* wm, const dr_frames* src, int B, int n, float* feat,
-                        const EncWs& w, hipStream_t s) {
+                        const EncWs& w, const Prep* P, hipStream_t s) {
   int e[DR_MAX_DEPTH + 1];
   const int N = enc_chans(d, e);
   const int h0 = d->img_h, w0 = d->img_w;
   const int F = enc_feat_dim(d);
   const bool e12 = N >= 2 && op_enc12_split3_ok(n, h0, w0, e[1], e[2], src) && !((uintptr_t)w.a[1] & 15);
+  void* wr[DR_MAX_DEPTH];
+  for (int k = 0; k < N; ++k) wr[k] = w.wr[k];
+  void* wproj = w.wproj;
   RepackJob rj[DR_RJ_MAX];
   int nj = 0;
   if (e12) {
-    rj[nj++] = rj_conv1(e[1], wm->conv[0].w, w.wr[0]);
-    rj[nj++] = rj_conv(e[2], e[1], wm->conv[1].w, w.wr[1]);
+    if (P) {
+      PREP_NEED(P->enc_wr[0] && P->enc_wr[1]);
+      wr[0] = P->enc_wr[0];
+      wr[1] = P->enc_wr[1];
+    }
+    rj[nj++] = rj_conv1(e[1], wm->conv[0].w, wr[0]);
+    rj[nj++] = rj_conv(e[2], e[1], wm->conv[1].w, wr[1]);
   }
   bool s3[DR_MAX_DEPTH + 1] = {};
   for (int k = 2; k < N; ++k) {
     s3[k] = op_conv_split3_supported(n, e[k], h0 >> k, w0 >> k, e[k + 1]) && nj < DR_RJ_MAX - 1;
-    if (s3[k]) rj[nj++] = rj_conv(e[k + 1], e[k], wm->conv[k].w, w.wr[k]);
-    else DR_TRY(op_conv_repack_bf16(e[k + 1], e[k], e[k], wm->conv[k].w, w.wr[k], s));
-  }
-  rj[nj++] = rj_bf16(d->enc_hidden, F, wm->map0.w, F + d->hidden, w.wproj);
-  DR_TRY(op_repack_multi(rj, nj, s));
+    if (s3[k]) {
+      if (P) {
+        PREP_NEED(P->enc_wr[k]);
+        wr[k] = P->enc_wr[k];
+      }
+      rj[nj++] = rj_conv(e[k + 1], e[k], wm->conv[k].w, wr[k]);
+    } else {
+      DR_TRY(op_conv_repack_bf16(e[k + 1], e[k], e[k], wm->conv[k].w, wr[k], s));
+    }
+  }
+  if (P) {
+    PREP_NEED(P->enc_proj);
+    wproj = P->enc_proj;
+  }
+  rj[nj++] = rj_bf16(d->enc_hidden, F, wm->map0.w, F + d->hidden, wproj);
+  if (!P) DR_TRY(op_repack_multi(rj, nj, s));
   const int rc_s1 = e12 ? op_enc12_s1_bf16(n, B, h0, w0, e[1], e[2], src, wm->conv[0].w, wm->conv[0].b, wm->conv[1].w,
-                                           wm->conv[1].b, w.wr[0], w.wr[1], w.a[1], s, 1)
+                                           wm->conv[1].b, wr[0], wr[1], w.a[1], s, 1)
                         : DR_E_INVALID;
   if (rc_s1 != DR_OK) {
     if (rc_s1 != DR_E_INVALID) return rc_s1;
@@ -93,17 +437,17 @@
   }
   for (int k = 2; k < N; ++k) {
     if (s3[k]) {
-      DR_TRY(op_conv_s1_bf16(n, e[k], h0 >> k, w0 >> k, e[k + 1], w.a[k - 1], w.wr[k], wm->conv[k].b, w.a[k],
+      DR_TRY(op_conv_s1_bf16(n, e[k], h0 >> k, w0 >> k, e[k + 1], w.a[k - 1], wr[k], wm->conv[k].b, w.a[k],
                              k == N - 1 ? 1 : 0, s));
     } else {
-      DR_TRY(op_conv_bf16(n, e[k], h0 >> k, w0 >> k, e[k + 1], w.a[k - 1], w.wr[k], wm->conv[k].b, w.a[k],
+      DR_TRY(op_conv_bf16(n, e[k], h0 >> k, w0 >> k, e[k + 1], w.a[k - 1], wr[k], wm->conv[k].b, w.a[k],
                           k == N - 1 ? 1 : 0, s));
     }
   }
-  const int rcp = op_gemm_nt_glds_bf16(n, d->enc_hidden, F, w.a[N - 1], F, w.wproj, F, wm->map0.b, feat, d->enc_hidden,
+  const int rcp = op_gemm_nt_glds_bf16(n, d->enc_hidden, F, w.a[N - 1], F, wproj, F, wm->map0.b, feat, d->enc_hidden,
                                        w.s3part, w.s3part_n, s);
   if (rcp != DR_E_INVALID) return rcp;
-  return op_gemm_nt_bf16(n, d->enc_hidden, F, w.a[N - 1], F, w.wproj, wm->map0.b, feat, d->enc_hidden, s);
+  return op_gemm_nt_bf16(n, d->enc_hidden, F, w.a[N - 1], F, wproj, wm->map0.b, feat, d->enc_hidden, s);
 }
 
 extern "C" int dr_encoder_features(const dr_dims* d, const dr_world_model* wm, const dr_frames* src, int B, int T,
@@ -141,30 +485,54 @@
   EncWs w;
   enc_carve(c, d, n, w);
   WS_CHECK(c, ws_bytes);
-  if (d->precision == DR_PREC_BF16) return encoder_bf16(d, wm, src, B, n, feat, w, s);
+  Prep Pb;
+  const Prep* P = nullptr;
+  if (d->prepared) {
+    DR_TRY(prep_get(d, __func__, B, T, -1, wm, nullptr, Pb));
+    P = &Pb;
+  }
+  if (d->precision == DR_PREC_BF16) return encoder_bf16(d, wm, src, B, n, feat, w, P, s);
   const int h0 = d->img_h, w0 = d->img_w;
   const int F = enc_feat_dim(d);
   const bool e12 = N >= 2 && op_enc12_split3_ok(n, h0, w0, e[1], e[2], src);
   const bool s3p = w.s3proj && n >= 1024 &&
                    op_gemm_nt_split3_supported(n, d->enc_hidden, F, w.a[N - 1], F, nullptr, 0, F, d->enc_hidden);
+  void* wr[DR_MAX_DEPTH];
+  for (int k = 0; k < N; ++k) wr[k] = w.wr[k];
+  void* s3proj = w.s3proj;
   RepackJob rj[DR_RJ_MAX];
   int nj = 0;
   if (e12) {
-    rj[nj++] = rj_conv1(e[1], wm->conv[0].w, w.wr[0]);
-    rj[nj++] = rj_conv(e[2], e[1], wm->conv[1].w, w.wr[1]);
+    if (P) {
+      PREP_NEED(P->enc_wr[0] && P->enc_wr[1]);
+      wr[0] = P->enc_wr[0];
+      wr[1] = P->enc_wr[1];
+    }
+    rj[nj++] = rj_conv1(e[1], wm->conv[0].w, wr[0]);
+    rj[nj++] = rj_conv(e[2], e[1], wm->conv[1].w, wr[1]);
   }
   bool s3[DR_MAX_DEPTH + 1] = {};
   for (int k = e12 ? 2 : 1; k < N; ++k) {
     s3[k] = op_conv_split3_supported(n, e[k], h0 >> k, w0 >> k, e[k + 1]) && nj < DR_RJ_MAX - 1;
     if (!s3[k]) continue;
     DR_TRY(conv_bias_aligned(__func__, "conv", k, wm->conv[k].b));
-    rj[nj++] = rj_conv(e[k + 1], e[k], wm->conv[k].w, w.wr[k]);
-  }
-  if (s3p) rj[nj++] = rj_nt(d->enc_hidden, F, wm->map0.w, F + d->hidden, w.s3proj);
-  DR_TRY(op_repack_multi(rj, nj, s));
+    if (P) {
+      PREP_NEED(P->enc_wr[k]);
+      wr[k] = P->enc_wr[k];
+    }
+    rj[nj++] = rj_conv(e[k + 1], e[k], wm->conv[k].w, wr[k]);
+  }
+  if (s3p) {
+    if (P) {
+      PREP_NEED(P->enc_proj);
+      s3proj = P->enc_proj;
+    }
+    rj[nj++] = rj_nt(d->enc_hidden, F, wm->map0.w, F + d->hidden, s3proj);
+  }
+  if (!P) DR_TRY(op_repack_multi(rj, nj, s));
   int k0 = 1;
   const int rc12 = e12 ? op_enc12_split3(n, B, h0, w0, e[1], e[2], src, wm->conv[0].w, wm->conv[0].b, wm->conv[1].w,
-                                         wm->conv[1].b, w.wr[0], w.wr[1], w.a[1], s, 1)
+                                         wm->conv[1].b, wr[0], wr[1], w.a[1], s, 1)
                        : DR_E_INVALID;
   if (rc12 == DR_OK) {
     k0 = 2;
@@ -181,7 +549,7 @@
     const float* cw = wm->conv[k].w;
     const float* cb = wm->conv[k].b;
     if (s3[k]) {
-      DR_TRY(op_conv_split3(n, cin, hin, win, cout, w.a[k - 1], w.wr[k], cb, w.a[k], last, s));
+      DR_TRY(op_conv_split3(n, cin, hin, win, cout, w.a[k - 1], wr[k], cb, w.a[k], last, s));
     } else {
       DR_TRY(op_conv_repack_pad(cout, cin, cin, cw, w.wr[k], s));
       DR_TRY(op_conv_nhwc(n, cin, hin, win, cout, w.a[k - 1], w.wr[k], cb, w.a[k], last, s));
@@ -189,7 +557,7 @@
   }
   if (s3p) {
     const int ksplits = std::max(1, std::min(8, (F + 1023) / 1024));
-    return op_gemm_nt_split3_sk(n, d->enc_hidden, F, w.a[N - 1], F, nullptr, 0, F, w.s3proj, wm->map0.b, 0, feat,
+    return op_gemm_nt_split3_sk(n, d->enc_hidden, F, w.a[N - 1], F, nullptr, 0, F, s3proj, wm->map0.b, 0, feat,
                                 d->enc_hidden, w.s3part, w.s3part_n, s, ksplits);
   }
   GemmArgs gp = lin(n, d->enc_hidden, F, w.a[N - 1], F, wm->map0.w, F + d->hidden, wm->map0.b, feat, d->enc_hidden);
@@ -238,7 +606,7 @@
 static int observe_steps(const dr_dims* d, const dr_world_model* wm, int B, int T, const float* feat,
                          const float* actions, long long act_sb, long long act_st, const float* h_init,
                          const float* z_init, const dr_noise& noise, float* z_out, float* h_out, float* logits_out,
-                         ObsWs& w, const ObsTrace* tr, hipStream_t s);
+                         ObsWs& w, const ObsTrace* tr, hipStream_t s, bool prepared = false);
 
 extern "C" int dr_observe_scan(const dr_dims* d, const dr_world_model* wm, int B, int T, const float* feat,
                                const float* actions, long long act_sb, long long act_st, const float* h_init,
@@ -255,9 +623,20 @@
   const int L = latent(d), Hd = d->hidden, eh = d->enc_hidden;
   const int F = enc_feat_dim(d);
   const bool any_gru = (z_init != nullptr) || T > 1;
+  const bool prepared = d->prepared != nullptr;
+  if (prepared) {
+    Prep P;
+    DR_TRY(prep_get(d, __func__, B, T, -1, wm, nullptr, P));
+    w.wt = P.wt;
+    if (chain_planes(d, B, T)) {
+      PREP_NEED(P.s3m0 && P.s3whh);
+      w.s3m0 = P.s3m0;
+      w.s3whh = P.s3whh;
+    }
+  }
   if (any_gru) {
     DR_REQUIRE(wm->w_ih && wm->w_hh && wm->b_ih && wm->b_hh, "GRU weights required");
-    DR_TRY(op_transpose(3 * Hd, L + d->action, wm->w_ih, w.wt, s));
+    if (!prepared) DR_TRY(op_transpose(3 * Hd, L + d->action, wm->w_ih, w.wt, s));
   }
   if (z_init == nullptr && h_init == nullptr && op_pscan_supported(d, B, T, d->action)) {
     const int rc = op_pscan(d, wm, B, T, d->action, feat, actions, act_sb, act_st, w.wt, wm->map0.w + F, F + Hd,
@@ -265,18 +644,18 @@
     if (rc != DR_E_UNSUPPORTED) return rc;
   }
   return observe_steps(d, wm, B, T, feat, actions, act_sb, act_st, h_init, z_init, noise, z_out, h_out, logits_out, w,
-                       nullptr, s);
+                       nullptr, s, prepared);
 }
 
 static int observe_steps(const dr_dims* d, const dr_world_model* wm, int B, int T, const float* feat,
                          const float* actions, long long act_sb, long long act_st, const float* h_init,
                          const float* z_init, const dr_noise& noise, float* z_out, float* h_out, float* logits_out,
-                         ObsWs& w, const ObsTrace* tr, hipStream_t s) {
+                         ObsWs& w, const ObsTrace* tr, hipStream_t s, bool prepared) {
   const int L = latent(d), Hd = d->hidden, eh = d->enc_hidden;
   const int F = enc_feat_dim(d);
   const long long ldL = (long long)T * L, ldH = (long long)T * Hd;
-  const bool planes = B >= 128 && T > 1 && Hd % 8 == 0;
-  if (planes) {
+  const bool planes = chain_planes(d, B, T);
+  if (planes && !prepared) {
     DR_TRY(split_planes(eh, Hd, wm->map0.w + F, F + Hd, w.s3m0, s));
     DR_TRY(split_planes(3 * Hd, Hd, wm->w_hh, Hd, w.s3whh, s));
   }
@@ -492,18 +871,18 @@
 
 static int imagine_heads(const dr_dims* d, const dr_world_model* wm, int B, int H, const float* latents,
                          const float* hiddens, float* rewards, float* continues, ImWs& w, hipStream_t s,
-                         bool keep0 = false);
+                         bool keep0 = false, bool prepared = false);
 
 static int imagine_launch_form(const dr_dims* d, const dr_world_model* wm, const dr_actor* ac, int B, int H,
                                const dr_noise& noise, const dr_noise& nq, int deterministic, float* latents,
                                float* hiddens, float* actions, float* mus, float* sigmas, const Tape& tp, ImWs& w,
-                               bool split_gru, bool zg, hipStream_t s) {
+                               bool split_gru, bool zg, hipStream_t s, bool prepared) {
   const int L = latent(d), Hd = d->hidden, A = d->action, a1 = d->actor_h1, a2 = d->actor_h2;
   const long long ldH = (long long)(H + 1) * Hd, ldL = (long long)(H + 1) * L, ldA = (long long)H * A;
   const long long lda1 = (long long)H * a1, lda2 = (long long)H * a2;
-  const bool planes = split_gru && H > 1 && Hd % 8 == 0;
+  const bool planes = chain_planes(d, B, H);
   const bool a16 = planes && d->precision == DR_PREC_BF16;
-  if (planes) {
+  if (planes && !prepared) {
     DR_TRY(split_planes(d->prior_h1, Hd, wm->prior.l0.w, Hd, w.s3p0, s));
     if (zg) DR_TRY(split_planes(a1, Hd, ac->l0.w, Hd + L, w.s3a0, s));
     DR_TRY(split_planes(3 * Hd, Hd, wm->w_hh, Hd, w.s3whh, s));
@@ -515,7 +894,7 @@
     g.a_out = tp.x1a; g.ld_aout = lda1;
     DR_TRY(run(G_NT, AM_LNSILU, g, s));
   }
-  DR_TRY(stack_heads(ac, A, a2, w.wst, w.bst, s));
+  if (!prepared) DR_TRY(stack_heads(ac, A, a2, w.wst, w.bst, s));
   {
     GemmArgs h = lin_ln(B, 2 * A, a2, tp.pre2a, lda2, ac->n4, w.wst, w.bst, nullptr, 0);
     h.a_out = tp.x2a; h.ld_aout = lda2;
@@ -603,6 +982,28 @@
   const int L = latent(d), Hd = d->hidden, A = d->action, a1 = d->actor_h1, a2 = d->actor_h2;
   const long long ldH = (long long)(H + 1) * Hd, ldL = (long long)(H + 1) * L, ldA = (long long)H * A;
   const long long lda1 = (long long)H * a1, lda2 = (long long)H * a2;
+  const bool zg = actor_zgather(d);
+  const bool prepared = d->prepared != nullptr;
+  if (prepared) {
+    Prep P;
+    DR_TRY(prep_get(d, __func__, B, -1, H, wm, ac, P));
+    w.wt = P.wt;
+    w.tl0f = P.tl0;
+    w.wst = P.wst;
+    w.bst = P.bst;
+    if (chain_planes(d, B, H)) {
+      PREP_NEED(P.s3p0 && P.s3whh && (!zg || P.s3a0));
+      w.s3p0 = P.s3p0;
+      w.s3a0 = P.s3a0;
+      w.s3whh = P.s3whh;
+    }
+    const int M1 = B * (H + 1);
+    if (s3_first_layer(d, M1, d->rew_h1, hiddens, Hd, latents, L) &&
+        s3_first_layer(d, M1, d->cont_h1, hiddens, Hd, latents, L))
+      PREP_NEED(P.s3r && P.s3c);
+    w.s3r = P.s3r;
+    w.s3c = P.s3c;
+  }
   {
     const Copy2dJob cj[2] = {{latents, ldL, z0, L, L, B}, {hiddens, ldH, h0, Hd, Hd, B}};
     DR_TRY(op_copy2d_multi(cj, 2, s));
@@ -610,8 +1011,7 @@
   dr_noise nq = noise;
   nq.stream += 65536;
   const bool split_gru = B >= 128;
-  const bool zg = d->rows <= 32 && a1 % 4 == 0;
-  {
+  if (!prepared) {
     TransposeJob tj[2] = {{3 * Hd, L + A, 3 * Hd, wm->w_ih, w.wt}, {a1, Hd + L, a1, ac->l0.w, w.tl0f}};
     DR_TRY(op_transpose_multi(tj, zg ? 2 : 1, s));
   }
@@ -627,20 +1027,25 @@
     unrolled = rc == DR_OK;
   }
   if (!unrolled) DR_TRY(imagine_launch_form(d, wm, ac, B, H, noise, nq, deterministic, latents, hiddens, actions, mus,
-                                            sigmas, tp, w, split_gru, zg, s));
-  return imagine_heads(d, wm, B, H, latents, hiddens, rewards, continues, w, s);
+                                            sigmas, tp, w, split_gru, zg, s, prepared));
+  return imagine_heads(d, wm, B, H, latents, hiddens, rewards, continues, w, s, false, prepared);
 }
 
 static int imagine_heads(const dr_dims* d, const dr_world_model* wm, int B, int H, const float* latents,
-                         const float* hiddens, float* rewards, float* continues, ImWs& w, hipStream_t s, bool keep0) {
+                         const float* hiddens, float* rewards, float* continues, ImWs& w, hipStream_t s, bool keep0,
+                         bool prepared) {
   const int L = latent(d), Hd = d->hidden;
   {
     const int M1 = B * (H + 1);
     GemmArgs p[2];
     if (s3_first_layer(d, M1, d->rew_h1, hiddens, Hd, latents, L) &&
         s3_first_layer(d, M1, d->cont_h1, hiddens, Hd, latents, L)) {
-      DR_TRY(op_nt_repack_split3(d->rew_h1, Hd + L, wm->reward.l0.w, Hd + L, w.s3r, s));
-      DR_TRY(op_nt_repack_split3(d->cont_h1, Hd + L, wm->cont.l0.w, Hd + L, w.s3c, s));
+      if (prepared) {
+        PREP_NEED(w.s3r && w.s3c);
+      } else {
+        DR_TRY(op_nt_repack_split3(d->rew_h1, Hd + L, wm->reward.l0.w, Hd + L, w.s3r, s));
+        DR_TRY(op_nt_repack_split3(d->cont_h1, Hd + L, wm->cont.l0.w, Hd + L, w.s3c, s));
+      }
       DR_TRY(op_gemm_nt_split3_sk(M1, d->rew_h1, Hd + L, hiddens, Hd, latents, L, Hd, w.s3r, wm->reward.l0.b, 0,
                                   w.p1r, d->rew_h1, w.s3part, w.s3part_n, s));
       DR_TRY(op_gemm_nt_split3_sk(M1, d->cont_h1, Hd + L, hiddens, Hd, latents, L, Hd, w.s3c, wm->cont.l0.b, 0,
@@ -842,6 +1247,19 @@
   const long long lda1 = (long long)H * a1, lda2 = (long long)H * a2;
   const int BH = B * H;
   const bool upstream_state = g_latents || g_hiddens;
+  const bool prepared = d->prepared != nullptr;
+  if (prepared) {
+    Prep P;
+    DR_TRY(prep_get(d, __func__, B, -1, H, wm, ac, P));
+    w.tl6p = P.tl6p; w.tl3p = P.tl3p; w.tl0p = P.tl0p; w.wt = P.wt; w.twhh = P.twhh;
+    w.thead = P.thead; w.tl3a = P.tl3a; w.tl0a = P.tl0;
+    if (bwd_planes(d, B)) {
+      PREP_NEED(P.s3wt && P.s3twhh && (d->actor_h1 % 8 != 0 || P.s3tl0a));
+      w.s3wt = P.s3wt;
+      w.s3twhh = P.s3twhh;
+      w.s3tl0a = P.s3tl0a;
+    }
+  }
   if (do_prep) {
   if (!g_hiddens && !g_latents && !g_actions) {
     DR_TRY(zero(w.gH, (long long)((w.gA + (long long)BH * A) - w.gH), s));
@@ -853,7 +1271,7 @@
     if (g_actions) DR_TRY(copy2d(w.gA, A, g_actions, A, A, (long long)BH, s));
     else DR_TRY(zero(w.gA, (long long)BH * A, s));
   }
-  {
+  if (!prepared) {
     const int h1 = d->prior_h1, h2 = d->prior_h2;
     TransposeJob tj[9] = {
         {L, h2, L, wm->prior.l6.w, w.tl6p},
@@ -867,14 +1285,14 @@
         {a1, Hd + L, a1, ac->l0.w, w.tl0a},
     };
     DR_TRY(op_transpose_multi(tj, 9, s));
-    if (B >= 128 && (3 * Hd) % 8 == 0) {
+    if (bwd_planes(d, B)) {
       DR_TRY(split_planes(L + A, 3 * Hd, w.wt, 3 * Hd, w.s3wt, s));
       DR_TRY(split_planes(Hd, 3 * Hd, w.twhh, 3 * Hd, w.s3twhh, s));
       if (d->actor_h1 % 8 == 0) DR_TRY(split_planes(Hd + L, d->actor_h1, w.tl0a, d->actor_h1, w.s3tl0a, s));
     }
   }
   }
-  const bool planes = B >= 128 && (3 * Hd) % 8 == 0;
+  const bool planes = bwd_planes(d, B);
   if (!do_main) return DR_OK;
 
   bool looped = false;
@@ -1028,6 +1446,12 @@
                              size_t ws_bytes, hipStream_t s) {
   DR_REQUIRE(d && cr && h && z && M > 0, "null argument or empty batch");
   GemmBf16Scope bf16_scope(d->precision == DR_PREC_BF16);
+  Prep P;
+  PrepNote note;
+  if (d->prepared) {
+    DR_TRY(prep_get(d, __func__, -1, -1, -1, nullptr, nullptr, P, &note));
+    DR_REQUIRE(M == note.B * (note.H + 1), "the block was prepared for another shape (B, H)");
+  }
   CTape t;
   float* sk = nullptr;
   long long skn = 0;
@@ -1062,7 +1486,14 @@
   DR_REQUIRE(tape || ws, "dr_critic_fwd needs a tape or a workspace");
   const int L = latent(d), Hd = d->hidden, c1 = d->critic_h1, c2 = d->critic_h2, nb = d->buckets;
   if (s3w && s3_first_layer(d, M, c1, h, ldh, z, ldz)) {
-    DR_TRY(op_nt_repack_split3(c1, Hd + L, cr->net.l0.w, Hd + L, s3w, s));
+    if (d->prepared) {
+      const void* id = cr->net.l0.w;
+      DR_REQUIRE(id == note.cr || id == note.tc, "the block holds no part prepared from this critic's weights");
+      s3w = P.s3v[id == note.cr ? 0 : 1];
+      PREP_NEED(s3w);
+    } else {
+      DR_TRY(op_nt_repack_split3(c1, Hd + L, cr->net.l0.w, Hd + L, s3w, s));
+    }
     DR_TRY(op_gemm_nt_split3_sk(M, c1, Hd + L, h, (int)ldh, z, (int)ldz, Hd, s3w, cr->net.l0.b, 0, t.pre1, c1,
                                 s3part, s3part_n, s));
   } else {
@@ -1130,6 +1561,14 @@
   CBws w;
   cbws_carve(c, d, B, H, w);
   WS_CHECK(c, ws_bytes);
+  if (d->prepared) {
+    Prep P;
+    PrepNote note;
+    DR_TRY(prep_get(d, __func__, B, -1, H, nullptr, nullptr, P, &note));
+    DR_REQUIRE((const void*)cr->net.l0.w == note.cr, "the block's critic part was not prepared from these weights");
+    w.tl6 = P.tl6;
+    w.tl3 = P.tl3;
+  }
   const int M = B * (H + 1);
   Carve ct((void*)tape);
   CTape t;
@@ -1137,7 +1576,7 @@
   const int L = latent(d), Hd = d->hidden, c1 = d->critic_h1, c2 = d->critic_h2, nb = d->buckets;
   DR_TRY(op_critic_ce(B, H, nb, t.logits, R, cr->buckets, scale, w.row_loss, w.glog, s));
   DR_TRY(op_mean(B * H, w.row_loss, loss_out, s));
-  {
+  if (!d->prepared) {
     TransposeJob tj[2] = {{nb, c2, nb, cr->net.l6.w, w.tl6}, {c2, c1, c2, cr->net.l3.w, w.tl3}};
     DR_TRY(op_transpose_multi(tj, 2, s));
   }
diff --git a/dreamer_amd/engine.py b/dreamer_amd/engine.py
--- a/dreamer_amd/engine.py
+++ b/dreamer_amd/engine.py
@@ -1,5 +1,6 @@
 import contextlib
 import gc
+import os
 
 import numpy as np
 
@@ -58,10 +59,42 @@
     def dims(self):
         return self.dr.world_model.dims(self.dr.agent)
 
+    def _set_dims(self):
+        self.d = self.dims()
+        self.d_prep = None
+        if self.prep is not None:
+            self.d_prep = L.dr_dims.from_buffer_copy(self.d)
+            self.d_prep.prepared = L.ptr(self.prep)
+            self.d_prep.prepared_bytes = self.prep.numel()
+
+    @contextlib.contextmanager
+    def _epoch_dims(self):
+        if self.d_prep is None:
+            yield
+            return
+        plain, self.d = self.d, self.d_prep
+        try:
+            yield
+        finally:
+            self.d = plain
+
+    def _prepare(self, wm=True, ac=True):
+        d, ag = self.d, self.dr.agent
+        if not d.prepared:
+            return
+        L.call("dr_prepare_weights", d, self.dr.world_model.packed() if wm else None,
+               ag.actor_struct() if ac else None, ag.critic_struct() if ac else None,
+               ag.critic_struct(target=True) if ac else None, self.B, self.T, self.H, d.prepared, d.prepared_bytes,
+               hip.stream())
+
     def _alloc(self):
+        self.prep = None
         d = self.dims()
-        self.d = d
         B, H, T = self.B, self.H, self.T
+        if os.environ.get("DREAMER_PREPARED", "1") != "0":
+            self.prep = torch.zeros(L.query("dr_prepared_bytes", d, B, T, H), dtype=torch.uint8, device=self.dev)
+        self._set_dims()
+        d = self.d
         L_ = d.rows * d.cols
         dev = self.dev
         f = lambda *s: torch.zeros(*s, device=dev)
@@ -215,6 +248,7 @@
 
     def _ph_encwarm(self):
         main = torch.cuda.current_stream(self.dev)
+        self._prepare()
         self.dr.buffer.gather_actions(self.starts, self.act_win)
         self.side.wait_stream(main)
         done = []
@@ -277,7 +311,7 @@
         ag.fault_slot().zero_()
         ag.fault_host()[0][0] = 0
         ag.persistent_ok = False
-        self.d = self.dims()
+        self._set_dims()
         self.graph, self.graph_key, self._pipe = None, None, None
         raise RuntimeError("dreamer_amd: a persistent kernel (posterior scan / imagination unroll / BPTT) timed out "
                            "waiting on another workgroup (not every workgroup was resident, e.g. other work held "
@@ -349,22 +383,23 @@
         self.epochs += 1
         ag = self.dr.agent
         key = (ag.params_key(), self.dr.world_model.params_key(), self.dr.buffer.device_key())
-        if self.use_graph and (self.graph is None or self.graph_key != key):
-            self._capture(key)
-        evs = [torch.cuda.Event(enable_timing=True)] if timing else None
-        if evs:
-            evs[0].record()
-        for k, (name, body, coll) in enumerate(self.phases()):
-            if self.use_graph:
-                self.graph[k].replay()
-            else:
-                body()
-            if coll is not None:
-                coll()
+        with self._epoch_dims():
+            if self.use_graph and (self.graph is None or self.graph_key != key):
+                self._capture(key)
+            evs = [torch.cuda.Event(enable_timing=True)] if timing else None
             if evs:
-                e = torch.cuda.Event(enable_timing=True)
-                e.record()
-                evs.append(e)
+                evs[0].record()
+            for k, (name, body, coll) in enumerate(self.phases()):
+                if self.use_graph:
+                    self.graph[k].replay()
+                else:
+                    body()
+                if coll is not None:
+                    coll()
+                if evs:
+                    e = torch.cuda.Event(enable_timing=True)
+                    e.record()
+                    evs.append(e)
         self.last_events = evs
         return ag.loss_slot(0), ag.loss_slot(1)
 
@@ -430,9 +465,14 @@
                     with torch.cuda.graph(g, stream=cs):
                         body()
                     graphs[(name, s)] = g
+
+            def optim():
+                self._ph_optim()
+                self._prepare(wm=False)
+
             for name, body in (("returns", self.returns), ("xfwd", self._x_critic_fwd_and_prep),
                                ("actor_loss", self._actor_loss), ("xbwd", self._x_critic_bwd),
-                               ("bptt", lambda: self._bptt(d=dw)), ("optim", self._ph_optim)):
+                               ("bptt", lambda: self._bptt(d=dw)), ("optim", optim)):
                 g = torch.cuda.CUDAGraph()
                 with torch.cuda.graph(g, stream=cs):
                     body()
@@ -445,7 +485,9 @@
         self.check_faults(wait=False)
         ag = self.dr.agent
         key = (ag.params_key(), self.dr.world_model.params_key(), self.dr.buffer.device_key())
-        P = self._pipe_capture(key)
+        with self._epoch_dims():
+            self._prepare()
+            P = self._pipe_capture(key)
         G = P["graphs"]
         outer = torch.cuda.current_stream(self.dev)
         import os
diff --git a/include/dreamer_hip.h b/include/dreamer_hip.h
--- a/include/dreamer_hip.h
+++ b/include/dreamer_hip.h
@@ -36,6 +36,8 @@
   int launch_form;
   float* fault;
   unsigned* fault_host;
+  void* prepared;
+  size_t prepared_bytes;
 } dr_dims;
 #define DR_MAX_DEPTH 5
 #define DR_PREC_FP32 0
@@ -85,6 +87,11 @@
 int dr_stream_destroy(hipStream_t s);
 int dr_device_cus(int* out);
 int dr_host_device_ptr(void* host, void** dev);
+
+size_t dr_prepared_bytes(const dr_dims* d, int B, int T, int H);
+int dr_prepare_weights(const dr_dims* d, const dr_world_model* wm, const dr_actor* ac, const dr_critic* critic,
+                       const dr_critic* target_critic, int B, int T, int H, void* out, size_t bytes,
+                       hipStream_t stream);
 
 size_t dr_encoder_workspace_bytes(const dr_dims* d, int n_frames);
 int dr_encoder_features(const dr_dims* d, const dr_world_model* wm, const dr_frames* src, int B, int T,
```

Result: no change. 617,500 imagined latent-steps/s, median of 6 (+0.7%).
